# lin-shuyu/ladder-latent-data-distribution-modelling

Measured on AMD Instinct MI355X. Metric: training images/sec (full 4-run LaDDer iteration, CelebA 128x128), higher is better.
Workload: dtype f32; 1 GPU; BASELINE configs[2]: celeba 128x128x3 nh=512 z=64 R=2 K=30 L=100 per-GPU batch=128, 4 runs/iteration (AE step, sigma step, prior step, inner-sigma step), fitted-GM regime; global_batch=128, parallelism=dp1

## Files before the change

### include/ladder_hip.h

```cpp
#ifndef LADDER_HIP_H
#define LADDER_HIP_H

#include <stddef.h>
#include <stdint.h>

#ifdef __cplusplus
extern "C" {
#endif

typedef struct ihipStream_t* ladder_stream_t;

enum { LADDER_OK = 0, LADDER_E_SHAPE = -1, LADDER_E_ALIGN = -2, LADDER_E_WORKSPACE = -3, LADDER_E_LAUNCH = -4 };
enum { LADDER_ACT_NONE = 0, LADDER_ACT_LEAKY = 1 , LADDER_ACT_RELU = 2, LADDER_ACT_TANH = 3 };

#define LADDER_ABI_VERSION 2
int ladder_abi_version(void);
int ladder_igemm_fwd_tile(long M, int Cin, int Cout);
int ladder_conv2d_fwd_kernel_id(int N, int H, int W, int Cin, int Ho, int Wo, int Cout, int KH, int KW, int stride, int ups,
                                int pad_t, int pad_l);
int ladder_dense_fwd_nt(const float* x, const float* wT, const float* bias, float* y, int M, int K, int N, int act, ladder_stream_t stream);
int ladder_dense_bwd_data_nt(const float* dy, const float* w, float* dx, int M, int K, int N, const float* gate_y, int gate_act, ladder_stream_t stream);
int ladder_dense_fwd_is_persistent(long M, int K, int N);
int ladder_dense_bwd_weight_is_persistent(long M, int K, int N);

// ... 31 lines not shown
int ladder_absmax_samples(const float* x, int n_samples, size_t per_sample, float* out, ladder_stream_t stream);
size_t ladder_filter_pack_split_bytes(int ntaps, int Cin, int Cout, int prec);
int ladder_filter_pack_split(const float* w, void* packed, int ntaps, int Cin, int Cout, int transpose_flip, int prec,
                             ladder_stream_t stream);
typedef struct ladder_pack_job_t {
  const float* w;
  void* packed;
  int ntaps, Cin, Cout, transpose_flip;
  int block_begin, reserved;
} ladder_pack_job_t;
int ladder_filter_pack_job_blocks(int ntaps, int Cin, int Cout);
size_t ladder_filter_pack_split_multi_scratch_bytes(int njobs);
int ladder_filter_pack_split_multi(const ladder_pack_job_t* jobs_dev, int njobs, int total_blocks, int prec, void* scratch,
                                   size_t scratch_bytes, ladder_stream_t stream);
int ladder_conv3x3_split_eligible(int N, int H, int W, int Cin, int Cout);
int ladder_conv3x3_f32_eligible(int N, int H, int W, int Cin, int Cout);
int ladder_conv3x3_split(const float* x, const float* x_absmax, const void* packed, const float* bias, float* y, float* y_absmax, int N,
                         int H, int W, int Cin, int Cout, int act, int prec, ladder_stream_t stream);

int ladder_conv3x3_split_proj(const float* x, const float* x_absmax, const void* packed, const float* bias, float* y, const float* proj_w,
                              const float* proj_b, float* proj_out, int proj_cout, int N, int H, int W, int Cin, int Cout, int act,
                              int prec, ladder_stream_t stream);

int ladder_conv3x3_s2_bwd_data_split_eligible(int N, int H, int W, int Cin, int Ho, int Wo, int Cout, int KH, int KW, int stride, int pad_t,
                                              int pad_l);
int ladder_conv3x3_s2_bwd_data_split(const float* dy, const float* dy_absmax, const void* packed_s2, float* dx, float* dx_absmax, int N, int H,
                                     int W, int Cin, int Ho, int Wo, int Cout, int prec, ladder_stream_t stream);
int ladder_conv3x3_s2_bwd_data_f32_eligible(int N, int H, int W, int Cin, int Ho, int Wo, int Cout);
int ladder_conv3x3_s2_fwd_f32_eligible(int N, int H, int W, int Cin, int Ho, int Wo, int Cout);
int ladder_conv3x3_s2_fwd_f32(const float* x, const void* bank_s2f, const float* bias, float* y, int N, int H, int W, int Cin, int Ho, int Wo,
                              int Cout, int act, ladder_stream_t stream);

int ladder_up2proj_eligible(int N, int H, int W, int Cin, int Cout);
int ladder_up2proj_fwd_combine(const float* z, const float* bias, float* y, const float* proj_w, const float* proj_b, float* proj_out, int proj_cout,
                               int N, int H, int W, int C, int act, ladder_stream_t stream);
int ladder_up2proj_bwd_combine(const float* dy, float* d, int N, int H, int W, int C, ladder_stream_t stream);
int ladder_up2proj_wgrad_unpack(const float* dwcat, const float* db9, float* dw, float* db, int Cin, int Cout, ladder_stream_t stream);
int ladder_upfproj_eligible(int factor, int N, int H, int W, int Cin, int Cout);
int ladder_upfproj_fwd_combine(const float* z, const float* bias, float* y, int factor, int N, int H, int W, int C, int act, ladder_stream_t stream);
int ladder_upfproj_bwd_combine(const float* dy, float* d, int factor, int N, int H, int W, int C, ladder_stream_t stream);
int ladder_up2proj_bwd_combine_walk(const float* dy, float* d, int N, int H, int W, int C, int rows_per_thread, ladder_stream_t stream);
int ladder_up2proj_bwd_combine_proj_eligible(int N, int H, int W, int C, int pco);
size_t ladder_up2proj_bwd_combine_proj_workspace_bytes(int N, int H, int W, int C, int pco);
int ladder_up2proj_bwd_combine_proj(const float* y, const float* dyp, const float* pw, float* d, float* dpw, float* dpb, int pco, int N, int H, int W, int C,
                                    int act, void* ws, size_t ws_bytes, ladder_stream_t stream);
int ladder_up2proj_fused_eligible(int N, int H, int W, int Cin, int Cout);
int ladder_up2proj_fused_preferred(int N, int H, int W, int Cin, int Cout);
int ladder_up2proj_fused_wide_tile(int N, int H, int W, int Cin, int Cout);
size_t ladder_up2proj_fused_workspace_bytes(int N, int H, int W, int Cout, int proj_cout);
int ladder_up2proj_fused_fwd(const float* x, const float* wcatT, const float* bias, float* y, const float* proj_w, const float* proj_b, float* proj_out,
                             int proj_cout, int N, int H, int W, int Cin, int Cout, int act, void* ws, size_t ws_bytes, ladder_stream_t stream);

int ladder_conv3x3_up2_split_eligible(int N, int H, int W, int Cin, int Cout, int prec);
int ladder_conv3x3_up2_split(const float* x, const float* x_absmax, const void* packed_up2, const float* bias, float* y, float* y_absmax,
                             int N, int H, int W, int Cin, int Cout, int act, int prec, int x_upsampled, ladder_stream_t stream);
int ladder_conv3x3_up2_split_proj(const float* x, const float* x_absmax, const void* packed_up2, const float* bias, float* y, const float* proj_w,
                                  const float* proj_b, float* proj_out, int proj_cout, int N, int H, int W, int Cin, int Cout, int act, int prec,
                                  int x_upsampled, ladder_stream_t stream);
int ladder_conv3x3_up2_bwd_data_split_eligible(int N, int H, int W, int C, int Cout, int prec);
int ladder_conv3x3_up2_bwd_data_split(const float* dy, const float* dy_absmax, const void* packed_up2t, float* dx, float* dx_absmax, int N, int H,
                                      int W, int C, int Cout, int prec, ladder_stream_t stream);
int ladder_conv3x3_up2_bwd_border(const float* d_up, float* dx, float* dx_absmax, int N, int H, int W, int C, int axis, int first,
                                  ladder_stream_t stream);
size_t ladder_conv3x3_up2_bwd_borders_workspace_bytes(int N, int H, int W, int C, int Cout);
int ladder_conv3x3_up2_bwd_borders(const float* dy, const float* w, float* dx, int N, int H, int W, int C, int Cout, void* ws, size_t ws_bytes,
                                   ladder_stream_t stream);
int ladder_conv3x3_up2_bwd_data_gated_f32_eligible(int N, int H, int W, int C, int Cout);
int ladder_conv3x3_up2_bwd_data_gated_f32(const float* dy, const void* bank_up2t, float* dx, const float* gate, int gate_act, int N, int H, int W, int C,
                                          int Cout, ladder_stream_t stream);
int ladder_conv3x3_up2_bwd_borders_gated(const float* dy, const float* w, float* dx, const float* gate, int gate_act, int N, int H, int W, int C, int Cout,
                                         void* ws, size_t ws_bytes, ladder_stream_t stream);
int ladder_conv3x3_up2_wgrad_eligible(int N, int H, int W, int Cin, int Cout);
size_t ladder_conv3x3_up2_wgrad_workspace_bytes(int N, int H, int W, int Cin, int Cout);
int ladder_conv3x3_up2_wgrad(const float* x, int x_upsampled, const float* dy, float* dw, float* db, int N, int H, int W, int Cin, int Cout,
                             void* ws, size_t ws_bytes, ladder_stream_t stream);
size_t ladder_conv3x3_up2_edges_workspace_bytes(int N, int H, int W, int Cin, int Cout);
int ladder_conv3x3_up2_edges(const float* x, const float* w, const float* bias, float* y, float* y_absmax, const float* proj_w, const float* proj_b,
                             float* proj_out, int proj_cout, int N, int H, int W, int Cin, int Cout, int act, int x_upsampled, void* ws,
                             size_t ws_bytes, ladder_stream_t stream);

size_t ladder_presplit_bytes(size_t n, int prec);
int ladder_presplit(const float* x, const float* x_absmax, void* planes, size_t n, int n_samples, int prec, ladder_stream_t stream);
int ladder_conv2d_fwd_split_eligible(int N, int H, int W, int Cin, int Ho, int Wo, int Cout, int KH, int KW, int stride, int pad_t,
                                     int pad_l);
size_t ladder_conv2d_fwd_split_workspace_bytes(int N, int H, int W, int Cin, int Ho, int Wo, int Cout, int KH, int KW, int stride,
                                               int pad_t, int pad_l);
int ladder_conv2d_fwd_split(const void* x_planes, const float* x_absmax, const void* packed, const float* bias, float* y, int N, int H, int W,
                            int Cin, int Ho, int Wo, int Cout, int KH, int KW, int stride, int pad_t, int pad_l, int act, int prec,
                            void* ws, size_t ws_bytes, ladder_stream_t stream);
size_t ladder_conv2d_fwd_split_bnstats_workspace_bytes(int N, int H, int W, int Cin, int Ho, int Wo, int Cout, int KH, int KW, int stride,
                                                       int pad_t, int pad_l);
int ladder_conv2d_fwd_split_bnstats(const void* x_planes, const float* x_absmax, const void* packed, const float* bias, float* y, int N,
                                    int H, int W, int Cin, int Ho, int Wo, int Cout, int KH, int KW, int stride, int pad_t, int pad_l,
                                    int act, int prec, float* sums4, void* stats_ws, size_t stats_ws_bytes, ladder_stream_t stream);
size_t ladder_conv2d_fwd_bnstats_workspace_bytes(int N, int H, int W, int Cin, int Ho, int Wo, int Cout, int KH, int KW, int stride, int pad_t,
                                                 int pad_l);
int ladder_conv2d_fwd_bnstats(const float* x, const float* w, const float* bias, float* y, int N, int H, int W, int Cin, int Ho, int Wo, int Cout,
                              int KH, int KW, int stride, int pad_t, int pad_l, int act, float* sums4, void* stats_ws, size_t stats_ws_bytes,
                              ladder_stream_t stream);
int ladder_conv2d_bwd_data_split_eligible(int N, int H, int W, int Cin, int Ho, int Wo, int Cout, int KH, int KW, int stride, int pad_t,
                                          int pad_l, int gated);
size_t ladder_conv2d_bwd_data_split_workspace_bytes(int N, int H, int W, int Cin, int Ho, int Wo, int Cout, int KH, int KW, int stride,
                                                    int pad_t, int pad_l);
int ladder_conv2d_bwd_data_split(const void* dy_planes, const float* dy_absmax, const void* packed_T, float* dx, int N, int H, int W, int Cin,
                                 int Ho, int Wo, int Cout, int KH, int KW, int stride, int pad_t, int pad_l, const float* gate_y,
                                 int gate_act, int prec, void* ws, size_t ws_bytes, ladder_stream_t stream);
int ladder_conv3x3_wgrad_split_eligible(int N, int H, int W, int Cin, int Cout, int prec);
size_t ladder_conv3x3_wgrad_split_workspace_bytes(int N, int H, int W, int Cin, int Cout);
int ladder_conv3x3_wgrad_split(const float* x, const float* x_absmax, const float* dy, const float* dy_absmax, float* dw, float* db,
                               int N, int H, int W, int Cin, int Cout, int prec, void* ws, size_t ws_bytes, ladder_stream_t stream);
int ladder_conv2d_bwd_filter_split_eligible(int N, int H, int W, int Cin, int Ho, int Wo, int Cout, int KH, int KW, int stride, int pad_t,
                                            int pad_l);
size_t ladder_conv2d_bwd_filter_split_workspace_bytes(int N, int H, int W, int Cin, int Ho, int Wo, int Cout, int KH, int KW);
int ladder_conv2d_bwd_filter_split(const void* x_planes, const float* x_absmax, const void* dy_planes, const float* dy_absmax, float* dw, float* db,
                                   int N, int H, int W, int Cin, int Ho, int Wo, int Cout, int KH, int KW, int stride, int pad_t, int pad_l,
                                   int prec, void* ws, size_t ws_bytes, ladder_stream_t stream);
int ladder_reduce_splits(const float* ws, float* out, int splits, size_t n, ladder_stream_t stream);

int ladder_dense_fwd(const float* x, const float* w, const float* bias, float* y,
                     int M, int K, int N, int act, void* ws, size_t ws_bytes, ladder_stream_t stream);
int ladder_dense_bwd_data(const float* dy, const float* wT, float* dx, int M, int K, int N,
                          const float* gate_y, int gate_act, void* ws, size_t ws_bytes, ladder_stream_t stream);
size_t ladder_dense_bwd_weight_workspace_bytes(int M, int K, int N);
int ladder_dense_bwd_weight(const float* x, const float* dy, float* dw, float* db,
                            int M, int K, int N, void* ws, size_t ws_bytes, ladder_stream_t stream);
int ladder_dense_small_eligible(int M, int K, int N);
int ladder_dense_fwd_small(const float* x, const float* w, const float* bias, float* y, int M, int K, int N, int act, ladder_stream_t stream);
int ladder_dense_bwd_data_small(const float* dy, const float* w, float* dx, int M, int K, int N, const float* gate_y, int gate_act,
                                ladder_stream_t stream);
int ladder_dense_bwd_weight_small(const float* x, const float* dy, float* dw, float* db, int M, int K, int N, ladder_stream_t stream);
int ladder_dense_bwd_small(const float* x, const float* dy, const float* w, float* dx, float* dw, float* db, int M, int K, int N,
                           const float* gate_y, int gate_act, ladder_stream_t stream);
int ladder_dense_fwd_small_f32(const float* x, const float* w, const float* bias, float* y, int M, int K, int N, int act, ladder_stream_t stream);
int ladder_dense_bwd_data_small_f32(const float* dy, const float* w, float* dx, int M, int K, int N, const float* gate_y, int gate_act,
                                    ladder_stream_t stream);
int ladder_dense_bwd_weight_small_f32(const float* x, const float* dy, float* dw, float* db, int M, int K, int N, ladder_stream_t stream);
int ladder_dense_bwd_small_f32(const float* x, const float* dy, const float* w, float* dx, float* dw, float* db, int M, int K, int N,
                               const float* gate_y, int gate_act, ladder_stream_t stream);


int ladder_conv_rgb_s2_eligible(int N, int H, int W, int Cin, int Cout, int KH, int KW, int stride, int pad_t, int pad_l);
int ladder_conv_rgb_s2_fwd(const float* x, const float* w, const float* bias, float* y, int N, int H, int W, int Cout, int act,
                           ladder_stream_t stream);
size_t ladder_conv_rgb_s2_fwd_bnstats_workspace_bytes(int N, int H, int W, int Cout);
int ladder_conv_rgb_s2_fwd_bnstats(const float* x, const float* w, const float* bias, float* y, int N, int H, int W, int Cout, int act,
                                   float* sums4 , void* ws, size_t ws_bytes,
                                   ladder_stream_t stream);
int ladder_conv_rgb_s2_fwd_f32(const float* x, const float* w, const float* bias, float* y, int N, int H, int W, int Cout, int act,
                               ladder_stream_t stream);
int ladder_conv_rgb_s2_fwd_bnstats_f32(const float* x, const float* w, const float* bias, float* y, int N, int H, int W, int Cout, int act,
                                       float* sums, void* ws, size_t ws_bytes, ladder_stream_t stream);
int ladder_conv_rgb_s2_bwd_filter_f32(const float* x, const float* dy, float* dw, float* db, int N, int H, int W, int Cout, void* ws,
                                      size_t ws_bytes, ladder_stream_t stream);
size_t ladder_conv_rgb_s2_bwd_filter_workspace_bytes(int N, int H, int W, int Cout);
int ladder_conv_rgb_s2_bwd_filter(const float* x, const float* x_absmax, const float* dy, const float* dy_absmax, float* dw, float* db,
                                  int N, int H, int W, int Cout, void* ws, size_t ws_bytes, ladder_stream_t stream);

int ladder_act_bwd(const float* dy, const float* y, float* dx, size_t n, int act, ladder_stream_t stream);

size_t ladder_bn_workspace_bytes(size_t rows, int C);
int ladder_bn_fwd_stats(const float* x, float* sums , size_t rows, int C,
                        void* ws, size_t ws_bytes, ladder_stream_t stream);
int ladder_bn_stats_from_partials(const float* partials, int nblk, float* sums , int C, ladder_stream_t stream);
int ladder_bn_fwd_stats_minmax(const float* x, float* sums4, size_t rows, int C, void* ws, size_t ws_bytes, ladder_stream_t stream);
int ladder_bn_stats_minmax_from_partials(const float* partials , int nblk, float* sums4, int C, ladder_stream_t stream);
int ladder_bn_fwd_apply_planes(const float* x, const float* sums4, double count, const float* gamma, const float* beta, float* y,
                               void* y_planes, float* mean_rstd, size_t rows, int C, float eps, int act, float* y_absmax,
                               ladder_stream_t stream);
int ladder_bn_fwd_apply(const float* x, const float* sums, double count,
                        const float* gamma, const float* beta, float* y, float* mean_rstd,
                        size_t rows, int C, float eps, int act, ladder_stream_t stream);
int ladder_bn_bwd_stats(const float* dy, const float* x, const float* mean_rstd, const float* gamma,
                        const float* beta, float* dsums , size_t rows, int C, int act,
                        void* ws, size_t ws_bytes, ladder_stream_t stream);
int ladder_bn_bwd_apply(const float* dy, const float* x, const float* mean_rstd, const float* gamma,
                        const float* beta, const float* dsums, double count, float* dx,
                        float* dgamma, float* dbeta, size_t rows, int C, int act, ladder_stream_t stream);
int ladder_bn_fwd_apply_absmax(const float* x, const float* sums, double count, const float* gamma, const float* beta, float* y,
                               float* mean_rstd, size_t rows, int C, float eps, int act, float* y_absmax, ladder_stream_t stream);
int ladder_bn_bwd_apply_absmax(const float* dy, const float* x, const float* mean_rstd, const float* gamma, const float* beta,
                               const float* dsums, double count, float* dx, float* dgamma, float* dbeta, size_t rows, int C, int act,
                               float* dx_absmax, ladder_stream_t stream);

size_t ladder_in_style_workspace_bytes(int N, int HW, int C);
int ladder_in_style_fwd(const float* x, const float* style, float* y, float* mean_rstd ,
                        int N, int HW, int C, float eps, int act, void* ws, size_t ws_bytes, ladder_stream_t stream);
int ladder_in_style_bwd(const float* dy, const float* x, const float* style, const float* mean_rstd,
                        float* dx, float* dstyle , int N, int HW, int C, int act,
                        void* ws, size_t ws_bytes, ladder_stream_t stream);
int ladder_in_style_fwd_absmax(const float* x, const float* style, float* y, float* mean_rstd, int N, int HW, int C, float eps, int act,
                               void* ws, size_t ws_bytes, float* y_absmax, ladder_stream_t stream);
int ladder_in_style_bwd_absmax(const float* dy, const float* x, const float* style, const float* mean_rstd, float* dx, float* dstyle,
                               int N, int HW, int C, int act, void* ws, size_t ws_bytes, float* dx_absmax, ladder_stream_t stream);
int ladder_in_style_fwd_resize2x(const float* x, const float* style, float* up, float* mean_rstd, int N, int H, int W, int C, float eps,
                                 int act, void* ws, size_t ws_bytes, float* up_absmax, ladder_stream_t stream);
int ladder_in_style_fwd_resize2x_keep(const float* x, const float* style, float* up, float* y, float* mean_rstd, int N, int H, int W, int C,
                                      float eps, int act, void* ws, size_t ws_bytes, float* up_absmax, ladder_stream_t stream);

int ladder_resize_bilinear_fwd(const float* x, float* y, int N, int H, int W, int C, int OH, int OW, ladder_stream_t stream);
int ladder_resize_bilinear_bwd(const float* dy, float* dx, int N, int H, int W, int C, int OH, int OW, ladder_stream_t stream);
int ladder_resize_bilinear_bwd_gated(const float* dy, float* dx, int N, int H, int W, int C, int OH, int OW, const float* gate_y,
                                     int gate_act, ladder_stream_t stream);

int ladder_depth_to_space(const float* x, float* y, int N, int H, int W, int C, int r, int inverse, ladder_stream_t stream);
int ladder_pad_symmetric(const float* x, float* y, int N, int H, int W, int C, int p, ladder_stream_t stream);
int ladder_pad_symmetric_bwd(const float* dy, float* dx, int N, int H, int W, int C, int p, ladder_stream_t stream);

int ladder_randn(float* out, size_t n, uint64_t seed, uint64_t offset, ladder_stream_t stream);

int ladder_gmm_packed_stride(int R);
int ladder_gmm_prepare(const float* weights, const float* means, const float* covs, int K, int R,
                       float* packed, ladder_stream_t stream);
size_t ladder_gmm_workspace_bytes(int L, int B);
int ladder_gmm_logprob_fwd_bwd(const float* mu, const float* sd, const float* eps, const float* packed,
                               int L, int B, int R, int K, float* sum_logp, float* dmu, float* dsd,
                               void* ws, size_t ws_bytes, ladder_stream_t stream);

int ladder_gmm_logprob_rows(const float* t, const float* packed, int n, int R, int K, float* logp, ladder_stream_t stream);

enum { LADDER_P_PIX_ABS = 0, LADDER_P_PIX_SQ = 1, LADDER_P_LOG_SDZ = 2, LADDER_P_MU2SD2_Z = 3, LADDER_P_CODE_ERR = 4,
       LADDER_P_CODE_SQRT = 5, LADDER_P_CODE_ABS = 6, LADDER_P_LOG_SDT = 7, LADDER_P_MU2SD2_T = 8, LADDER_P_LOGP = 9,
       LADDER_P_FIXED = 16 };
enum { LADDER_S_SIGMA = 0, LADDER_S_MPE = 1, LADDER_S_ENTROPY_Z = 2, LADDER_S_XENT_SG = 3, LADDER_S_XENT_PRIOR = 4,
       LADDER_S_L1 = 5, LADDER_S_L2 = 6, LADDER_S_RECON_LL = 7, LADDER_S_SIGMA_REG = 8, LADDER_S_ELBO = 9,
       LADDER_S_LOSS_AE = 10, LADDER_S_INNER_SIGMA = 11, LADDER_S_MEAN_CODE_ERROR = 12, LADDER_S_CODE_LL = 13,
       LADDER_S_CODE_L1 = 14, LADDER_S_REP_REG = 15, LADDER_S_ENTROPY_T = 16, LADDER_S_XENT_T = 17,
       LADDER_S_ELBO_PRIOR = 18, LADDER_S_LOSS_PRIOR = 19,
       LADDER_S_G_PIX = 20,
       LADDER_S_G_SIGMA_VAR = 21,
       LADDER_S_G_CODE = 22,
       LADDER_S_G_INNER_SIGMA_VAR = 23,
       LADDER_S_INV_B = 24, LADDER_S_INV_LB = 25, LADDER_S_COUNT = 32 };
typedef struct {
  int B_global, D, Z, R, L;
  int sigma_uses_mpe;
  int has_inner;
  int use_sg;
  int clamp_inner_sigma;
  float inner_sigma_lb, inner_sigma_ub;
  int hierarchical;
  int prior_gmm;
} LadderElboCfg;

size_t ladder_pixel_partials_workspace_bytes(size_t n);
int ladder_pixel_partials(const float* x, const float* xhat, size_t n, float* out ,
                          void* ws, size_t ws_bytes, ladder_stream_t stream);
int ladder_pixel_grad(const float* x, const float* xhat, const float* coef, float* dxhat, size_t n, ladder_stream_t stream);
int ladder_latent_fwd(const float* mu, const float* sd_raw, const float* eps, float lvp, float* z, float* sd,
                      float* p_log, float* p_mu2sd2, float* p_sdsum, int B, int Z, ladder_stream_t stream);
int ladder_code_partials(const float* z, const float* zhat, const float* sd_z, int use_mask,
                         float* out , int B, int Z, ladder_stream_t stream);
int ladder_elbo_finalize(const float* partials, const float* sigma_var, const float* inner_sigma_var,
                         LadderElboCfg cfg, float* scalars, ladder_stream_t stream);
int ladder_code_grad(const float* z, const float* zhat, const float* sd_z, int use_mask, const float* scalars,
                     float* dz_accum, float* dzhat, int B, int Z, ladder_stream_t stream);
int ladder_latent_bwd(const float* g_sample, const float* mu, const float* sd, const float* sd_raw, const float* eps,
                      const float* extra_mu, const float* extra_sd, float extra_sign, const float* scalars, int mode,
                      float* dmu, float* dsd_raw, int B, int Z, ladder_stream_t stream);

int ladder_adam_clip(float* theta, const float* g, float* m, float* v, size_t n,
                     float lr_t, float beta1, float beta2, float eps, float clip, ladder_stream_t stream);

int ladder_adam_clip_dev(float* theta, const float* g, float* m, float* v, size_t n, float* state,
                         float beta1, float beta2, float eps, float clip, ladder_stream_t stream);
int ladder_randn_dev(float* out, size_t n, uint64_t seed, const uint64_t* offset_base, uint64_t offset_add, ladder_stream_t stream);
int ladder_u64_add(uint64_t* p, uint64_t inc, ladder_stream_t stream);

size_t ladder_gmm_dense_param_floats(int K, int R);
int ladder_gmm_prepare_dense(const float* weights, const float* means, const float* covs, int K, int R, float* params,
                             ladder_stream_t stream);
size_t ladder_gmm_dense_workspace_bytes(int L, int B, int R, int K);
int ladder_gmm_dense_logprob_fwd_bwd(const float* mu, const float* sd, const float* eps, const float* params, int L, int B, int R,
                                     int K, float* sum_logp, float* dmu, float* dsd, void* ws, size_t ws_bytes,
                                     ladder_stream_t stream);

int ladder_gmm_dense_logprob_rows(const float* t, const float* params, int n, int R, int K, float* logp, void* ws, size_t ws_bytes,
                                  ladder_stream_t stream);

size_t ladder_diag_mixture_workspace_bytes(int B, int Z, int K);
int ladder_diag_mixture_fwd_bwd(const float* mu, const float* sd, const float* eps, const float* comp_mean, const float* comp_sd,
                                int L, int B, int Z, int K, float* sum_logp, float* dmu, float* dsd, float* dcomp_mean,
                                float* dcomp_sd, void* ws, size_t ws_bytes, ladder_stream_t stream);

int ladder_gather_rows(const void* src, int src_is_u8, const int64_t* idx, float* out, int B, int64_t D, float scale,
                       ladder_stream_t stream);

size_t ladder_vbgmm_state_doubles(int K, int R);
size_t ladder_vbgmm_workspace_bytes(int N, int K);
int ladder_vbgmm_fit(const float* X, int N, int K, int R, const int* labels, double* state, int prior_type, double wc_prior,
                     double mean_prec_prior, double reg_covar, double tol, int max_iter, float* weights, float* means,
                     float* covs, void* ws, size_t ws_bytes, ladder_stream_t stream);

size_t ladder_vbgmm_shard_stats_doubles(int K, int R);
size_t ladder_vbgmm_shard_workspace_bytes(int N, int K, int R);
size_t ladder_vbgmm_shard_moments_doubles(int R);
int ladder_vbgmm_shard_moments(const float* X, int N, int R, double* moments, ladder_stream_t stream);
int ladder_vbgmm_shard_estep(const float* X, int N, int K, int R, const int* labels, const double* state, int prior_type, double* stats,
                             void* ws, size_t ws_bytes, ladder_stream_t stream);
int ladder_vbgmm_shard_mstep(const double* stats, const double* moments, int K, int R, double* state, int prior_type, double wc_prior,
                             double mean_prec_prior, double reg_covar, double tol, int max_iter, int it, float* weights, float* means,
                             float* covs, ladder_stream_t stream);

size_t ladder_mixture_sample_param_bytes(int K, int R);
int ladder_mixture_sample_prepare(const float* weights, const float* means, const float* covs, int K, int R, void* params,
                                  ladder_stream_t stream);
int ladder_mixture_sample_prepare_diag(const float* comp_mean, const float* comp_sd, int K, int R, void* params, ladder_stream_t stream);
int ladder_mixture_sample(const void* params, int K, int R, int n, int64_t first, const float* u, const float* eps, uint64_t seed,
                          uint64_t offset, float* out, int* comp, ladder_stream_t stream);
int ladder_images_to_u8(const float* x, uint8_t* out, size_t n, ladder_stream_t stream);

uint32_t ladder_crc32c_extend(uint32_t crc, const void* data, size_t n);
int ladder_axpy(const float* in, float* out, size_t n, float scale, int accumulate, ladder_stream_t stream);

#ifdef __cplusplus
}
#endif
#endif
```

### ladder_latent_data_distribution_modelling_amd/_lib.py

```python
import ctypes as C
import os

_HERE = os.path.dirname(os.path.abspath(__file__))
LIB_PATH = os.path.join(_HERE, "csrc", "libladder_hip.so")

ERRORS = {-1: "LADDER_E_SHAPE", -2: "LADDER_E_ALIGN", -3: "LADDER_E_WORKSPACE", -4: "LADDER_E_LAUNCH"}
ACT = {None: 0, "none": 0, "leaky_relu": 1, "relu": 2, "tanh": 3}

P_PIX_ABS, P_PIX_SQ, P_LOG_SDZ, P_MU2SD2_Z, P_CODE_ERR, P_CODE_SQRT, P_CODE_ABS, P_LOG_SDT, P_MU2SD2_T, P_LOGP = range(10)
P_FIXED = 16
S_NAMES = ["sigma", "mean_pixel_error", "entropy_z", "crossEntropy_prior_sg", "crossEntropy_prior",
           "l1_reconstruction_error", "l2_reconstruction_error", "reconstruction_likelihood", "sigma_regularisor",
           "elbo", "loss_ae", "inner_sigma", "mean_code_error", "code_reconstruction_likelihood",
           "code_l1_reconstruction_error", "representation_regularisor", "entropy_t",
           "crossEntropy_representation", "elbo_prior", "loss_prior",
           "_g_pix", "_g_sigma_var", "_g_code", "_g_inner_sigma_var", "_inv_B", "_inv_LB"]
S_INDEX = {n: i for i, n in enumerate(S_NAMES)}
S_COUNT = 32
ABSMAX_FLOATS = 512
ABI_VERSION = 2


class LadderElboCfg(C.Structure):
    _fields_ = [("B_global", C.c_int), ("D", C.c_int), ("Z", C.c_int), ("R", C.c_int), ("L", C.c_int),
                ("sigma_uses_mpe", C.c_int), ("has_inner", C.c_int), ("use_sg", C.c_int),
                ("clamp_inner_sigma", C.c_int), ("inner_sigma_lb", C.c_float), ("inner_sigma_ub", C.c_float),
                ("hierarchical", C.c_int), ("prior_gmm", C.c_int)]


_p, _i, _f, _d, _z, _u64 = C.c_void_p, C.c_int, C.c_float, C.c_double, C.c_size_t, C.c_uint64

PROTOTYPES = {
    "ladder_abi_version": (_i, []),
    "ladder_igemm_fwd_tile": (_i, [C.c_long, _i, _i]),
    "ladder_dense_fwd_is_persistent": (_i, [C.c_long, _i, _i]),
    "ladder_dense_fwd_nt": (_i, [_p, _p, _p, _p, _i, _i, _i, _i, _p]),
    "ladder_dense_bwd_data_nt": (_i, [_p, _p, _p, _i, _i, _i, _p, _i, _p]),
    "ladder_dense_bwd_weight_is_persistent": (_i, [C.c_long, _i, _i]),
    "ladder_igemm_fwd_splits": (_i, [C.c_long, _i, _i]),
    "ladder_conv2d_fwd_kernel_id": (_i, [_i] * 13),
    "ladder_conv2d_bwd_filter_kernel_id": (_i, [_i] * 12),
    "ladder_conv2d_fwd": (_i, [_p, _p, _p, _p] + [_i] * 13 + [_p, _z, _p]),
    "ladder_igemm_fwd_workspace_bytes": (_z, [C.c_long, _i, _i]),
    "ladder_filter_flip_transpose": (_i, [_p, _p, _i, _i, _i, _i, _p]),
    "ladder_conv2d_bwd_data": (_i, [_p, _p, _p] + [_i] * 12 + [_p, _i, _p, _z, _p]),
    "ladder_conv2d_bwd_filter_workspace_bytes": (_z, [_i] * 9),
    "ladder_conv2d_bwd_filter": (_i, [_p, _p, _p, _p] + [_i] * 12 + [_p, _z, _p]),
    "ladder_dense_fwd": (_i, [_p, _p, _p, _p, _i, _i, _i, _i, _p, _z, _p]),
    "ladder_dense_bwd_data": (_i, [_p, _p, _p, _i, _i, _i, _p, _i, _p, _z, _p]),
    "ladder_dense_bwd_weight_workspace_bytes": (_z, [_i, _i, _i]),
    "ladder_dense_bwd_weight": (_i, [_p, _p, _p, _p, _i, _i, _i, _p, _z, _p]),
    "ladder_act_bwd": (_i, [_p, _p, _p, _z, _i, _p]),
    "ladder_bn_workspace_bytes": (_z, [_z, _i]),
    "ladder_bn_fwd_stats": (_i, [_p, _p, _z, _i, _p, _z, _p]),
    "ladder_bn_fwd_apply": (_i, [_p, _p, _d, _p, _p, _p, _p, _z, _i, _f, _i, _p]),
    "ladder_bn_bwd_stats": (_i, [_p, _p, _p, _p, _p, _p, _z, _i, _i, _p, _z, _p]),
    "ladder_bn_bwd_apply": (_i, [_p, _p, _p, _p, _p, _p, _d, _p, _p, _p, _z, _i, _i, _p]),
    "ladder_in_style_workspace_bytes": (_z, [_i, _i, _i]),
    "ladder_in_style_fwd": (_i, [_p, _p, _p, _p, _i, _i, _i, _f, _i, _p, _z, _p]),
    "ladder_in_style_bwd": (_i, [_p, _p, _p, _p, _p, _p, _i, _i, _i, _i, _p, _z, _p]),
    "ladder_resize_bilinear_fwd": (_i, [_p, _p] + [_i] * 6 + [_p]),
    "ladder_resize_bilinear_bwd": (_i, [_p, _p] + [_i] * 6 + [_p]),
    "ladder_resize_bilinear_bwd_gated": (_i, [_p, _p, _i, _i, _i, _i, _i, _i, _p, _i, _p]),
    "ladder_depth_to_space": (_i, [_p, _p] + [_i] * 6 + [_p]),
    "ladder_pad_symmetric": (_i, [_p, _p] + [_i] * 5 + [_p]),
    "ladder_randn": (_i, [_p, _z, _u64, _u64, _p]),
    "ladder_gmm_packed_stride": (_i, [_i]),
    "ladder_gmm_prepare": (_i, [_p, _p, _p, _i, _i, _p, _p]),
    "ladder_gmm_workspace_bytes": (_z, [_i, _i]),
    "ladder_gmm_logprob_fwd_bwd": (_i, [_p, _p, _p, _p, _i, _i, _i, _i, _p, _p, _p, _p, _z, _p]),
    "ladder_gmm_logprob_rows": (_i, [_p, _p, _i, _i, _i, _p, _p]),
    "ladder_gmm_dense_logprob_rows": (_i, [_p, _p, _i, _i, _i, _p, _p, _z, _p]),
    "ladder_pixel_partials_workspace_bytes": (_z, [_z]),
    "ladder_pixel_partials": (_i, [_p, _p, _z, _p, _p, _z, _p]),
    "ladder_pixel_grad": (_i, [_p, _p, _p, _p, _z, _p]),
    "ladder_latent_fwd": (_i, [_p, _p, _p, _f, _p, _p, _p, _p, _p, _i, _i, _p]),
    "ladder_code_partials": (_i, [_p, _p, _p, _i, _p, _i, _i, _p]),
    "ladder_elbo_finalize": (_i, [_p, _p, _p, LadderElboCfg, _p, _p]),
    "ladder_code_grad": (_i, [_p, _p, _p, _i, _p, _p, _p, _i, _i, _p]),
    "ladder_latent_bwd": (_i, [_p, _p, _p, _p, _p, _p, _p, _f, _p, _i, _p, _p, _i, _i, _p]),
    "ladder_adam_clip": (_i, [_p, _p, _p, _p, _z, _f, _f, _f, _f, _f, _p]),
    "ladder_adam_clip_dev": (_i, [_p, _p, _p, _p, _z, _p, _f, _f, _f, _f, _p]),
    "ladder_randn_dev": (_i, [_p, _z, _u64, _p, _u64, _p]),
    "ladder_u64_add": (_i, [_p, _u64, _p]),
    "ladder_crc32c_extend": (C.c_uint32, [C.c_uint32, _p, _z]),
    "ladder_gmm_dense_param_floats": (_z, [_i, _i]),
    "ladder_gmm_prepare_dense": (_i, [_p, _p, _p, _i, _i, _p, _p]),
    "ladder_gmm_dense_workspace_bytes": (_z, [_i, _i, _i, _i]),
    "ladder_gmm_dense_logprob_fwd_bwd": (_i, [_p, _p, _p, _p, _i, _i, _i, _i, _p, _p, _p, _p, _z, _p]),
    "ladder_diag_mixture_workspace_bytes": (_z, [_i, _i, _i]),
    "ladder_diag_mixture_fwd_bwd": (_i, [_p, _p, _p, _p, _p, _i, _i, _i, _i, _p, _p, _p, _p, _p, _p, _z, _p]),
    "ladder_pad_symmetric_bwd": (_i, [_p, _p, _i, _i, _i, _i, _i, _p]),
    "ladder_conv1x1_smallcout_eligible": (_i, [C.c_long, _i, _i]),
    "ladder_conv1x1_smallcout_bwd_workspace_bytes": (_z, [C.c_long, _i, _i]),
    "ladder_conv1x1_smallcout_bwd": (_i, [_p, _p, _p, _p, _p, _p, C.c_long, _i, _i, _i, _p, _z, _p]),
    "ladder_gather_rows": (_i, [_p, _i, _p, _p, _i, C.c_int64, _f, _p]),
    "ladder_vbgmm_state_doubles": (_z, [_i, _i]),
    "ladder_vbgmm_workspace_bytes": (_z, [_i, _i]),
    "ladder_vbgmm_fit": (_i, [_p, _i, _i, _i, _p, _p, _i, _d, _d, _d, _d, _i, _p, _p, _p, _p, _z, _p]),
    "ladder_vbgmm_shard_stats_doubles": (_z, [_i, _i]),
    "ladder_vbgmm_shard_workspace_bytes": (_z, [_i, _i, _i]),
    "ladder_vbgmm_shard_moments_doubles": (_z, [_i]),
    "ladder_vbgmm_shard_moments": (_i, [_p, _i, _i, _p, _p]),
    "ladder_vbgmm_shard_estep": (_i, [_p, _i, _i, _i, _p, _p, _i, _p, _p, _z, _p]),
    "ladder_vbgmm_shard_mstep": (_i, [_p, _p, _i, _i, _p, _i, _d, _d, _d, _d, _i, _i, _p, _p, _p, _p]),
    "ladder_axpy": (_i, [_p, _p, _z, _f, _i, _p]),
    "ladder_filter_pack_split_bytes": (_z, [_i, _i, _i, _i]),
    "ladder_filter_pack_split": (_i, [_p, _p, _i, _i, _i, _i, _i, _p]),
    "ladder_filter_pack_job_blocks": (_i, [_i, _i, _i]),
    "ladder_filter_pack_split_multi_scratch_bytes": (_z, [_i]),
    "ladder_filter_pack_split_multi": (_i, [_p, _i, _i, _i, _p, _z, _p]),
    "ladder_conv2d_fwd_split_eligible": (_i, [_i] * 12),
    "ladder_conv2d_fwd_split_workspace_bytes": (_z, [_i] * 12),
    "ladder_conv2d_fwd_split": (_i, [_p, _p, _p, _p, _p] + [_i] * 14 + [_p, _z, _p]),
    "ladder_conv2d_fwd_split_bnstats_workspace_bytes": (_z, [_i] * 12),
    "ladder_conv2d_fwd_split_bnstats": (_i, [_p] * 5 + [_i] * 14 + [_p, _p, _z, _p]),
    "ladder_conv2d_fwd_bnstats_workspace_bytes": (_z, [_i] * 12),
    "ladder_conv2d_fwd_bnstats": (_i, [_p, _p, _p, _p] + [_i] * 13 + [_p, _p, _z, _p]),
    "ladder_conv2d_bwd_data_split_eligible": (_i, [_i] * 13),
    "ladder_conv2d_bwd_data_split_workspace_bytes": (_z, [_i] * 12),
    "ladder_conv2d_bwd_data_split": (_i, [_p, _p, _p, _p] + [_i] * 12 + [_p, _i, _i, _p, _z, _p]),
    "ladder_conv3x3_split_eligible": (_i, [_i] * 5),
    "ladder_conv3x3_split": (_i, [_p, _p, _p, _p, _p, _p] + [_i] * 7 + [_p]),
    "ladder_conv3x3_s2_bwd_data_split_eligible": (_i, [_i] * 12),
    "ladder_conv3x3_up2_split_eligible": (_i, [_i] * 6),
    "ladder_conv3x3_up2_split": (_i, [_p, _p, _p, _p, _p, _p] + [_i] * 8 + [_p]),
    "ladder_conv3x3_up2_split_proj": (_i, [_p] * 8 + [_i] * 9 + [_p]),
    "ladder_conv3x3_up2_bwd_data_split_eligible": (_i, [_i] * 6),
    "ladder_conv3x3_up2_bwd_data_split": (_i, [_p] * 5 + [_i] * 6 + [_p]),
    "ladder_conv3x3_up2_bwd_border": (_i, [_p, _p, _p] + [_i] * 6 + [_p]),
    "ladder_conv3x3_up2_bwd_borders_workspace_bytes": (_z, [_i] * 5),
    "ladder_conv3x3_up2_bwd_borders": (_i, [_p, _p, _p] + [_i] * 5 + [_p, _z, _p]),
    "ladder_conv3x3_up2_wgrad_eligible": (_i, [_i] * 5),
    "ladder_conv3x3_up2_wgrad_workspace_bytes": (_z, [_i] * 5),
    "ladder_conv3x3_up2_wgrad": (_i, [_p, _i, _p, _p, _p] + [_i] * 5 + [_p, _z, _p]),
    "ladder_conv3x3_up2_edges_workspace_bytes": (_z, [_i] * 5),
    "ladder_conv3x3_up2_edges": (_i, [_p] * 8 + [_i] * 8 + [_p, _z, _p]),
    "ladder_conv3x3_s2_bwd_data_split": (_i, [_p, _p, _p, _p, _p] + [_i] * 8 + [_p]),
    "ladder_conv3x3_f32_eligible": (_i, [_i] * 5),
    "ladder_conv3x3_up2_bwd_data_gated_f32_eligible": (_i, [_i] * 5),
    "ladder_conv3x3_up2_bwd_data_gated_f32": (_i, [_p, _p, _p, _p] + [_i] * 6 + [_p]),
    "ladder_conv3x3_up2_bwd_borders_gated": (_i, [_p, _p, _p, _p] + [_i] * 6 + [_p, _z, _p]),
    "ladder_conv3x3_s2_bwd_data_f32_eligible": (_i, [_i] * 7),
    "ladder_conv3x3_s2_fwd_f32_eligible": (_i, [_i] * 7),
    "ladder_conv3x3_s2_fwd_f32": (_i, [_p, _p, _p, _p] + [_i] * 8 + [_p]),
    "ladder_up2proj_eligible": (_i, [_i] * 5),
    "ladder_up2proj_fwd_combine": (_i, [_p] * 6 + [_i] * 6 + [_p]),
    "ladder_up2proj_bwd_combine": (_i, [_p, _p] + [_i] * 4 + [_p]),
    "ladder_up2proj_wgrad_unpack": (_i, [_p] * 4 + [_i, _i, _p]),
    "ladder_upfproj_eligible": (_i, [_i] * 6),
    "ladder_upfproj_fwd_combine": (_i, [_p] * 3 + [_i] * 6 + [_p]),
    "ladder_upfproj_bwd_combine": (_i, [_p, _p] + [_i] * 5 + [_p]),
    "ladder_up2proj_bwd_combine_walk": (_i, [_p, _p] + [_i] * 5 + [_p]),
    "ladder_up2proj_bwd_combine_proj_eligible": (_i, [_i] * 5),
    "ladder_up2proj_bwd_combine_proj_workspace_bytes": (_z, [_i] * 5),
    "ladder_up2proj_bwd_combine_proj": (_i, [_p] * 6 + [_i] * 6 + [_p, _z, _p]),
    "ladder_up2proj_fused_eligible": (_i, [_i] * 5),
    "ladder_up2proj_fused_preferred": (_i, [_i] * 5),
    "ladder_up2proj_fused_wide_tile": (_i, [_i] * 5),
    "ladder_up2proj_fused_workspace_bytes": (_z, [_i] * 5),
    "ladder_up2proj_fused_fwd": (_i, [_p] * 7 + [_i] * 7 + [_p, _z, _p]),
    "ladder_dense_small_eligible": (_i, [_i, _i, _i]),
    "ladder_dense_fwd_small": (_i, [_p, _p, _p, _p, _i, _i, _i, _i, _p]),
    "ladder_dense_bwd_data_small": (_i, [_p, _p, _p, _i, _i, _i, _p, _i, _p]),
    "ladder_dense_bwd_weight_small": (_i, [_p, _p, _p, _p, _i, _i, _i, _p]),
    "ladder_dense_bwd_small": (_i, [_p, _p, _p, _p, _p, _p, _i, _i, _i, _p, _i, _p]),
    "ladder_dense_fwd_small_f32": (_i, [_p, _p, _p, _p, _i, _i, _i, _i, _p]),
    "ladder_dense_bwd_data_small_f32": (_i, [_p, _p, _p, _i, _i, _i, _p, _i, _p]),
    "ladder_dense_bwd_weight_small_f32": (_i, [_p, _p, _p, _p, _i, _i, _i, _p]),
    "ladder_dense_bwd_small_f32": (_i, [_p, _p, _p, _p, _p, _p, _i, _i, _i, _p, _i, _p]),
    "ladder_presplit_bytes": (_z, [_z, _i]),
    "ladder_presplit": (_i, [_p, _p, _p, _z, _i, _i, _p]),
    "ladder_absmax_samples": (_i, [_p, _i, _z, _p, _p]),
    "ladder_conv3x3_split_proj": (_i, [_p, _p, _p, _p, _p, _p, _p, _p] + [_i] * 8 + [_p]),
    "ladder_conv_rgb_s2_eligible": (_i, [_i] * 10),
    "ladder_conv_rgb_s2_fwd": (_i, [_p, _p, _p, _p, _i, _i, _i, _i, _i, _p]),
    "ladder_conv_rgb_s2_fwd_bnstats_workspace_bytes": (_z, [_i] * 4),
    "ladder_conv_rgb_s2_fwd_bnstats": (_i, [_p, _p, _p, _p, _i, _i, _i, _i, _i, _p, _p, _z, _p]),
    "ladder_conv_rgb_s2_fwd_f32": (_i, [_p, _p, _p, _p, _i, _i, _i, _i, _i, _p]),
    "ladder_conv_rgb_s2_fwd_bnstats_f32": (_i, [_p, _p, _p, _p, _i, _i, _i, _i, _i, _p, _p, _z, _p]),
    "ladder_bn_stats_from_partials": (_i, [_p, _i, _p, _i, _p]),
    "ladder_bn_stats_minmax_from_partials": (_i, [_p, _i, _p, _i, _p]),
    "ladder_bn_fwd_stats_minmax": (_i, [_p, _p, _z, _i, _p, _z, _p]),
    "ladder_bn_fwd_apply_planes": (_i, [_p, _p, _d, _p, _p, _p, _p, _p, _z, _i, _f, _i, _p, _p]),
    "ladder_conv_rgb_s2_bwd_filter_workspace_bytes": (_z, [_i] * 4),
    "ladder_conv_rgb_s2_bwd_filter": (_i, [_p] * 6 + [_i] * 4 + [_p, _z, _p]),
    "ladder_conv_rgb_s2_bwd_filter_f32": (_i, [_p] * 4 + [_i] * 4 + [_p, _z, _p]),
    "ladder_bn_fwd_apply_absmax": (_i, [_p, _p, _d, _p, _p, _p, _p, _z, _i, _f, _i, _p, _p]),
    "ladder_bn_bwd_apply_absmax": (_i, [_p, _p, _p, _p, _p, _p, _d, _p, _p, _p, _z, _i, _i, _p, _p]),
    "ladder_in_style_fwd_absmax": (_i, [_p, _p, _p, _p, _i, _i, _i, _f, _i, _p, _z, _p, _p]),
    "ladder_in_style_fwd_resize2x": (_i, [_p, _p, _p, _p, _i, _i, _i, _i, _f, _i, _p, _z, _p, _p]),
    "ladder_in_style_fwd_resize2x_keep": (_i, [_p, _p, _p, _p, _p, _i, _i, _i, _i, _f, _i, _p, _z, _p, _p]),
    "ladder_in_style_bwd_absmax": (_i, [_p, _p, _p, _p, _p, _p, _i, _i, _i, _i, _p, _z, _p, _p]),
    "ladder_conv1x1_smallcout_bwd_absmax": (_i, [_p, _p, _p, _p, _p, _p, C.c_long, _i, _i, _i, _p, _z, _p, C.c_long, _p]),
    "ladder_absmax": (_i, [_p, _z, _p, _p]),
    "ladder_conv3x3_wgrad_split_eligible": (_i, [_i] * 6),
    "ladder_conv3x3_wgrad_split_workspace_bytes": (_z, [_i] * 5),
    "ladder_conv3x3_wgrad_split": (_i, [_p, _p, _p, _p, _p, _p] + [_i] * 6 + [_p, _z, _p]),
    "ladder_reduce_splits": (_i, [_p, _p, _i, _z, _p]),
    "ladder_conv2d_bwd_filter_split_eligible": (_i, [_i] * 12),
    "ladder_conv2d_bwd_filter_split_workspace_bytes": (_z, [_i] * 9),
    "ladder_conv2d_bwd_filter_split": (_i, [_p, _p, _p, _p, _p, _p] + [_i] * 13 + [_p, _z, _p]),
    "ladder_mixture_sample_param_bytes": (_z, [_i, _i]),
    "ladder_mixture_sample_prepare": (_i, [_p, _p, _p, _i, _i, _p, _p]),
    "ladder_mixture_sample_prepare_diag": (_i, [_p, _p, _i, _i, _p, _p]),
    "ladder_mixture_sample": (_i, [_p, _i, _i, _i, C.c_int64, _p, _p, _u64, _u64, _p, _p, _p]),
    "ladder_images_to_u8": (_i, [_p, _p, _z, _p]),
}

_lib = None


class LadderHipError(RuntimeError):
    pass


def load(path=None):
    global _lib
    if _lib is not None:
        return _lib
    path = path or os.environ.get("LADDER_HIP_LIB", LIB_PATH)
    import torch
    if not os.path.exists(path):
        raise LadderHipError(
            "libladder_hip.so not found at %s: build it with `python -m "
            "ladder_latent_data_distribution_modelling_amd.csrc.build` (there is no CPU fallback)" % path)
    lib = C.CDLL(path)
    for name, (res, args) in PROTOTYPES.items():
        fn = getattr(lib, name)
        fn.restype = res
        fn.argtypes = args
    got = lib.ladder_abi_version()
    if got != ABI_VERSION:
        raise LadderHipError("%s reports ABI version %d, this binding needs %d (stale build? re-run `python -m "
                             "ladder_latent_data_distribution_modelling_amd.csrc.build`)" % (path, got, ABI_VERSION))
    _lib = lib
    return lib


def call(name, *args):
    rc = getattr(load(), name)(*args)
    if rc != 0:
        raise LadderHipError("%s failed: %s (%d)" % (name, ERRORS.get(rc, "?"), rc))


def query(name, *args):
    return getattr(load(), name)(*args)
```

### ladder_latent_data_distribution_modelling_amd/csrc/convrgb.hip

```cpp
#include "split16.h"

namespace {

constexpr int RGB_TH = 8, RGB_TW = 32, RGB_PIX = RGB_TH * RGB_TW;
constexpr int RGB_PH = 2 * RGB_TH + 1, RGB_PW = 2 * RGB_TW + 1;
constexpr int RGB_PATCH = RGB_PH * RGB_PW * 3;
constexpr int RGB_THREADS = 512;
constexpr int RGB_A_PLANE = 2 * 2 * RGB_PIX * 16;
constexpr int RGB_B_PLANE = 2 * 2 * 128 * 16;

__device__ __forceinline__ float block_max_512(float m, float* red) {
  m = wave_max(m);
  __syncthreads();
  if ((threadIdx.x & 63) == 0) red[threadIdx.x >> 6] = m;
  __syncthreads();
  float b = red[0];
#pragma unroll
  for (int w = 1; w < 8; ++w) b = fmaxf(b, red[w]);
  return b;
}

__device__ __forceinline__ float rgb_tap(const float* __restrict__ patch, int pr, int pc, int k) {
  const int tap = k / 3, ci = k - tap * 3, r = tap / 3, s = tap - r * 3;
  return patch[((2 * pr + r) * RGB_PW + 2 * pc + s) * 3 + ci];
// ... 162 lines not shown
    __syncthreads();
#pragma unroll
    for (int ni = 0; ni < 2; ++ni) {
      const float a0 = st0[ni] + __shfl_xor(st0[ni], 32, 64), a1 = st1[ni] + __shfl_xor(st1[ni], 32, 64);
      const float a2 = fminf(smn[ni], __shfl_xor(smn[ni], 32, 64)), a3 = fmaxf(smx[ni], __shfl_xor(smx[ni], 32, 64));
      if (lh == 0) {
        const int cc = wn * 64 + ni * 32 + l31;
        sred[(0 * 4 + wm) * 128 + cc] = a0;
        sred[(1 * 4 + wm) * 128 + cc] = a1;
        sred[(2 * 4 + wm) * 128 + cc] = a2;
        sred[(3 * 4 + wm) * 128 + cc] = a3;
      }
    }
    __syncthreads();
    {
      const int which = tid >> 7, c = tid & 127;
      const float v0 = sred[(which * 4 + 0) * 128 + c], v1 = sred[(which * 4 + 1) * 128 + c], v2 = sred[(which * 4 + 2) * 128 + c],
                  v3 = sred[(which * 4 + 3) * 128 + c];
      const float t = which < 2 ? (v0 + v1) + (v2 + v3) : (which == 2 ? fminf(fminf(v0, v1), fminf(v2, v3)) : fmaxf(fmaxf(v0, v1), fmaxf(v2, v3)));
      if (n0 + c < Cout) stats_part[((size_t)mt * 4 + which) * Cout + n0 + c] = t;
    }
  }
}

constexpr int RW_PH = 2, RW_PW = 32, RW_PIX = RW_PH * RW_PW;
constexpr int RW_XH = 2 * RW_PH + 1, RW_XW = 2 * RW_PW + 1, RW_PATCH = RW_XH * RW_XW * 3;
constexpr int RW_THREADS = 256;
constexpr int RW_ABLK = RW_PIX * 64 + 64, RW_DBLK = RW_PIX * 64 + 64;
constexpr int RW_APLANE = RW_ABLK, RW_DPLANE = 4 * RW_DBLK;
constexpr int RW_XU = (RW_PATCH + RW_THREADS - 1) / RW_THREADS;
constexpr int RW_DU = RW_PIX * 32 / RW_THREADS;

typedef short rgb_s16x4 __attribute__((ext_vector_type(4)));
__device__ __forceinline__ uint4 rgb_tr_frag(const unsigned char* p) {
  const rgb_s16x4 lo = __builtin_amdgcn_ds_read_tr16_b64_v4i16((__attribute__((address_space(3))) rgb_s16x4*)(p));
  const rgb_s16x4 hi = __builtin_amdgcn_ds_read_tr16_b64_v4i16((__attribute__((address_space(3))) rgb_s16x4*)(p + 4 * 64));
  const uint2 a = __builtin_bit_cast(uint2, lo), b = __builtin_bit_cast(uint2, hi);
  return make_uint4(a.x, a.y, b.x, b.y);
}
__device__ __forceinline__ float rgb_frag_sum(const uint4 f) {
  const uint32_t w[4] = {f.x, f.y, f.z, f.w};
  float s = 0.f;
#pragma unroll
  for (int i = 0; i < 4; ++i) {
    const f32x2 v = __builtin_convertvector(__builtin_bit_cast(f16x2, w[i]), f32x2);
    s += v.x + v.y;
  }
  return s;
}

__global__ __launch_bounds__(RW_THREADS, 3) void conv_rgb_s2_wgrad_kernel(const float* __restrict__ x, const float* __restrict__ dy,
                                                                         float* __restrict__ part, float* __restrict__ bias_part,
                                                                         const int N, const int H, const int W, const int Cout,
                                                                         const int tiles_co, const int patches_per_split,
                                                                         const float* __restrict__ xamax, const float* __restrict__ damax) {
  __shared__ __attribute__((aligned(16))) unsigned char lds[2 * RW_APLANE + 2 * RW_DPLANE];
  __shared__ __attribute__((aligned(16))) float patch[RW_PATCH + 1];
  unsigned char* const Ab = lds;
  unsigned char* const Db = lds + 2 * RW_APLANE;

  const int tid = threadIdx.x, lane = tid & 63, wv = tid >> 6;
  const int l31 = lane & 31, lh = lane >> 5, l15 = lane & 15;
  const int split = blockIdx.x / tiles_co, co0 = (blockIdx.x - split * tiles_co) * 128;
  const int Ho = H / 2, Wo = W / 2, WP = Wo / RW_PW, HP = Ho / RW_PH;
  const int q_total = N * HP * WP;
  const int q0 = split * patches_per_split, q1 = min(q_total, q0 + patches_per_split);
  const float cx = scale_from_absmax(amax_load(xamax)), cd = scale_from_absmax(amax_load(damax));
  const int frag_lane = (8 * lh + (l15 >> 2)) * 64 + (16 * ((lane >> 4) & 1) + 4 * (l15 & 3)) * 2;

  f32x16 acc;
#pragma unroll
  for (int e = 0; e < 16; ++e) acc[e] = 0.f;
  float bsum = 0.f;

  float xr[RW_XU];
  float4 d0, d1, d2, d3, d4, d5, d6, d7;
  auto load_patch = [&](int q) {
    const int img = q / (HP * WP), rem = q - img * (HP * WP), hp = rem / WP;
    const int h0 = hp * RW_PH, w0 = (rem - hp * WP) * RW_PW;
#pragma unroll
    for (int i = 0; i < RW_XU; ++i) {
      const int v = tid + i * RW_THREADS;
      const int r = v / (RW_XW * 3), c3 = v - r * (RW_XW * 3);
      const int hi = 2 * h0 + r, wi3 = 2 * w0 * 3 + c3;
      xr[i] = (v < RW_PATCH && hi < H && wi3 < W * 3) ? x[((long)img * H + hi) * W * 3 + wi3] : 0.f;
    }
    const float* dbase = dy + (((long)img * Ho + h0) * Wo + w0) * Cout + co0;
#define RW_DSRC(i_) [&]() -> float4 {                                                                                       \
      const int u = tid + (i_) * RW_THREADS, px = u >> 5, q4 = u & 31;                                                        \
      if (co0 + q4 * 4 >= Cout) return make_float4(0.f, 0.f, 0.f, 0.f);                                                       \
      return *reinterpret_cast<const float4*>(dbase + ((long)(px >> 5) * Wo + (px & 31)) * Cout + q4 * 4); }()
    d0 = RW_DSRC(0); d1 = RW_DSRC(1); d2 = RW_DSRC(2); d3 = RW_DSRC(3); d4 = RW_DSRC(4); d5 = RW_DSRC(5); d6 = RW_DSRC(6); d7 = RW_DSRC(7);
#undef RW_DSRC
  };
  auto store_d = [&](int i, float4 v) {
    const int u = tid + i * RW_THREADS, px = u >> 5, q4 = u & 31;
    uint2 pl[2];
    split4<2, true>(make_float4(v.x * cd, v.y * cd, v.z * cd, v.w * cd), pl);
#pragma unroll
    for (int p = 0; p < 2; ++p) *reinterpret_cast<uint2*>(Db + p * RW_DPLANE + (q4 >> 3) * RW_DBLK + px * 64 + (q4 & 7) * 8) = pl[p];
  };

  if (q0 < q1) load_patch(q0);
  for (int q = q0; q < q1; ++q) {
#pragma unroll
    for (int i = 0; i < RW_XU; ++i)
      if (tid + i * RW_THREADS < RW_PATCH) patch[tid + i * RW_THREADS] = xr[i];
    store_d(0, d0); store_d(1, d1); store_d(2, d2); store_d(3, d3); store_d(4, d4); store_d(5, d5); store_d(6, d6); store_d(7, d7);
    __syncthreads();
    if (tid < 2 * RW_PIX) {
      const int p = tid & (RW_PIX - 1), kh = tid >> 6, pr = p >> 5, pc = p & 31;
      float av[16];
#pragma unroll
      for (int j = 0; j < 16; ++j) {
        const int k = kh * 16 + j;
        const int tap = k / 3, ci = k - tap * 3, r = tap / 3, s = tap - r * 3;
        av[j] = k < 27 ? patch[((2 * pr + r) * RW_XW + 2 * pc + s) * 3 + ci] * cx : 0.f;
      }
#pragma unroll
      for (int o = 0; o < 4; ++o) {
        uint2 pl[2];
        split4<2, true>(make_float4(av[4 * o], av[4 * o + 1], av[4 * o + 2], av[4 * o + 3]), pl);
#pragma unroll
        for (int pp = 0; pp < 2; ++pp) *reinterpret_cast<uint2*>(Ab + pp * RW_APLANE + p * 64 + kh * 32 + o * 8) = pl[pp];
      }
    }
    __syncthreads();
    if (q + 1 < q1) load_patch(q + 1);
#pragma unroll
    for (int ks = 0; ks < RW_PIX / 16; ++ks) {
      const int pb = ks * 16;
      const uint4 a0 = rgb_tr_frag(Ab + pb * 64 + frag_lane), a1 = rgb_tr_frag(Ab + RW_APLANE + pb * 64 + frag_lane);
      const uint4 b0 = rgb_tr_frag(Db + wv * RW_DBLK + pb * 64 + frag_lane), b1 = rgb_tr_frag(Db + RW_DPLANE + wv * RW_DBLK + pb * 64 + frag_lane);
      acc = mfma16<true>(a1, b0, acc);
      acc = mfma16<true>(a0, b1, acc);
      acc = mfma16<true>(a0, b0, acc);
      bsum += rgb_frag_sum(b1) + rgb_frag_sum(b0);
    }
    __syncthreads();
  }

  const float unscale = 1.f / (cx * cd);
  float* o = part + (size_t)split * 27 * Cout;
  const int n = co0 + wv * 32 + l31;
#pragma unroll
  for (int e = 0; e < 16; ++e) {
    const int k = (e & 3) + 8 * (e >> 2) + 4 * lh;
    if (k < 27 && n < Cout) o[(size_t)k * Cout + n] = acc[e] * unscale;
  }
  bsum += __shfl_down(bsum, 32, 64);
  if (bias_part != nullptr && lh == 0 && n < Cout) bias_part[(size_t)split * Cout + n] = bsum * (1.f / cd);
}

constexpr int RW_LDA32 = 33;
__global__ __launch_bounds__(RW_THREADS, 4) void conv_rgb_s2_wgrad_f32_kernel(const float* __restrict__ x, const float* __restrict__ dy,
                                                                             float* __restrict__ part, float* __restrict__ bias_part,
                                                                             const int N, const int H, const int W, const int Cout,
                                                                             const int tiles_co, const int patches_per_split) {
  __shared__ float A32[RW_PIX * RW_LDA32];
  __shared__ float patch[RW_PATCH + 1];
  const int tid = threadIdx.x, lane = tid & 63, wv = tid >> 6;
  const int l31 = lane & 31, lh = lane >> 5;
  const int split = blockIdx.x / tiles_co, co0 = (blockIdx.x - split * tiles_co) * 128;
  const int Ho = H / 2, Wo = W / 2, WP = Wo / RW_PW, HP = Ho / RW_PH;
  const int q_total = N * HP * WP;
  const int q0 = split * patches_per_split, q1 = min(q_total, q0 + patches_per_split);
  const int co = co0 + wv * 32 + l31;
  const bool co_ok = co < Cout;

  f32x16 acc;
#pragma unroll
  for (int e = 0; e < 16; ++e) acc[e] = 0.f;
  float bsum = 0.f;
  float xr[RW_XU];
  auto decode = [&](int q, int& img, int& h0, int& w0) {
    img = q / (HP * WP);
    const int rem = q - img * (HP * WP), hp = rem / WP;
    h0 = hp * RW_PH;
    w0 = (rem - hp * WP) * RW_PW;
  };
  auto load_x = [&](int q) {
    int img, h0, w0;
    decode(q, img, h0, w0);
#pragma unroll
    for (int i = 0; i < RW_XU; ++i) {
      const int v = tid + i * RW_THREADS;
      const int r = v / (RW_XW * 3), c3 = v - r * (RW_XW * 3);
      const int hi = 2 * h0 + r, wi3 = 2 * w0 * 3 + c3;
      xr[i] = (v < RW_PATCH && hi < H && wi3 < W * 3) ? x[((long)img * H + hi) * W * 3 + wi3] : 0.f;
    }
  };

  if (q0 < q1) load_x(q0);
  for (int q = q0; q < q1; ++q) {
    float b[RW_PIX / 2];
    {
      int img, h0, w0;
      decode(q, img, h0, w0);
      const float* du = dy + (((long)img * Ho + h0) * Wo + w0) * Cout;
      const unsigned loff = (unsigned)(co + lh * Cout);
#pragma unroll
      for (int ks = 0; ks < RW_PIX / 2; ++ks) {
        const float* pk = du + ((long)(ks >> 4) * Wo + 2 * (ks & 15)) * Cout;
        b[ks] = co_ok ? pk[loff] : 0.f;
      }
    }
#pragma unroll
    for (int i = 0; i < RW_XU; ++i)
      if (tid + i * RW_THREADS < RW_PATCH) patch[tid + i * RW_THREADS] = xr[i];
    __syncthreads();
    if (q + 1 < q1) load_x(q + 1);
    {
      const int p = tid & (RW_PIX - 1), kq = tid >> 6, pr = p >> 5, pc = p & 31;
#pragma unroll
      for (int j = 0; j < 8; ++j) {
        const int k = kq * 8 + j;
        const int tap = k / 3, ci = k - tap * 3, r = tap / 3, sx = tap - r * 3;
        A32[p * RW_LDA32 + k] = k < 27 ? patch[((2 * pr + r) * RW_XW + 2 * pc + sx) * 3 + ci] : 0.f;
      }
    }
    __syncthreads();
#pragma unroll
    for (int ks = 0; ks < RW_PIX / 2; ++ks) {
      const float a = A32[(2 * ks + lh) * RW_LDA32 + l31];
      acc = __builtin_amdgcn_mfma_f32_32x32x2f32(a, b[ks], acc, 0, 0, 0);
      bsum += b[ks];
    }
    __syncthreads();
  }

  float* o = part + (size_t)split * 27 * Cout;
#pragma unroll
  for (int e = 0; e < 16; ++e) {
    const int k = (e & 3) + 8 * (e >> 2) + 4 * lh;
    if (k < 27 && co_ok) o[(size_t)k * Cout + co] = acc[e];
  }
  if (bias_part != nullptr) {
    const float v = bsum + __shfl_down(bsum, 32, 64);
    if (lh == 0 && co_ok) bias_part[(size_t)split * Cout + co] = v;
  }
}

struct RgbWgradPlan { int tiles_co, splits, pps; };
RgbWgradPlan plan_rgb_wgrad(int N, int H, int W, int Cout) {
  RgbWgradPlan p;
  p.tiles_co = (Cout + 127) / 128;
  const long q_total = (long)N * (H / 2 / RW_PH) * (W / 2 / RW_PW);
  long s = (3 * 256L) / p.tiles_co;
  if (s > q_total / 4) s = q_total / 4;
  if (s < 1) s = 1;
  p.pps = (int)((q_total + s - 1) / s);
  p.splits = (int)((q_total + p.pps - 1) / p.pps);
  return p;
}

bool rgb_s2_ok(int N, int H, int W, int Cin, int Cout, int KH, int KW, int stride, int pad_t, int pad_l) {
  return N > 0 && Cin == 3 && KH == 3 && KW == 3 && stride == 2 && pad_t == 0 && pad_l == 0 && (H % 2) == 0 && (W % 2) == 0 &&
         ((H / 2) % RGB_TH) == 0 && ((W / 2) % RGB_TW) == 0 && Cout >= 32 && (Cout % 4) == 0;
}

}

extern "C" {

int ladder_conv_rgb_s2_eligible(int N, int H, int W, int Cin, int Cout, int KH, int KW, int stride, int pad_t, int pad_l) {
  return rgb_s2_ok(N, H, W, Cin, Cout, KH, KW, stride, pad_t, pad_l) ? 1 : 0;
}

static int rgb_fwd_launch(const float* x, const float* w, const float* bias, float* y, int N, int H, int W, int Cout, int act, float* stats_part,
                          ladder_stream_t stream, bool f32 = false) {
  if (!rgb_s2_ok(N, H, W, 3, Cout, 3, 3, 2, 0, 0)) return LADDER_E_SHAPE;
  if (!ladder_aligned16(y) || (bias != nullptr && !ladder_aligned16(bias))) return LADDER_E_ALIGN;
  const int tiles_n = (Cout + 127) / 128;
  const long tiles = (long)N * (H / 2 / RGB_TH) * (W / 2 / RGB_TW) * tiles_n;
  if (tiles >= (1L << 31)) return LADDER_E_SHAPE;
  if (f32)
    hipLaunchKernelGGL(conv_rgb_s2_fwd_kernel<true>, dim3((unsigned)tiles), dim3(RGB_THREADS), 0, stream, x, w, bias, y, N, H, W, Cout, act, tiles_n,
                       stats_part);
  else
    hipLaunchKernelGGL(conv_rgb_s2_fwd_kernel<false>, dim3((unsigned)tiles), dim3(RGB_THREADS), 0, stream, x, w, bias, y, N, H, W, Cout, act, tiles_n,
                       stats_part);
  LADDER_CHECK_LAUNCH();
  return LADDER_OK;
}

int ladder_conv_rgb_s2_fwd(const float* x, const float* w, const float* bias, float* y, int N, int H, int W, int Cout, int act,
                           ladder_stream_t stream) {
  return rgb_fwd_launch(x, w, bias, y, N, H, W, Cout, act, nullptr, stream);
}

size_t ladder_conv_rgb_s2_fwd_bnstats_workspace_bytes(int N, int H, int W, int Cout) {
  if (!rgb_s2_ok(N, H, W, 3, Cout, 3, 3, 2, 0, 0)) return 0;
  return (size_t)N * (H / 2 / RGB_TH) * (W / 2 / RGB_TW) * 4 * Cout * sizeof(float);
}

int ladder_conv_rgb_s2_fwd_bnstats(const float* x, const float* w, const float* bias, float* y, int N, int H, int W, int Cout, int act,
                                   float* sums, void* ws, size_t ws_bytes, ladder_stream_t stream) {
  const size_t need = ladder_conv_rgb_s2_fwd_bnstats_workspace_bytes(N, H, W, Cout);
  if (need == 0 || sums == nullptr) return LADDER_E_SHAPE;
  if (ws == nullptr || ws_bytes < need) return LADDER_E_WORKSPACE;
  const int rc = rgb_fwd_launch(x, w, bias, y, N, H, W, Cout, act, (float*)ws, stream);
  if (rc != LADDER_OK) return rc;
  return ladder_bn_stats_minmax_from_partials((const float*)ws, N * (H / 2 / RGB_TH) * (W / 2 / RGB_TW), sums, Cout, stream);
}

int ladder_conv_rgb_s2_fwd_f32(const float* x, const float* w, const float* bias, float* y, int N, int H, int W, int Cout, int act,
                               ladder_stream_t stream) {
  return rgb_fwd_launch(x, w, bias, y, N, H, W, Cout, act, nullptr, stream, true);
}

int ladder_conv_rgb_s2_fwd_bnstats_f32(const float* x, const float* w, const float* bias, float* y, int N, int H, int W, int Cout, int act,
                                       float* sums, void* ws, size_t ws_bytes, ladder_stream_t stream) {
  const size_t need = ladder_conv_rgb_s2_fwd_bnstats_workspace_bytes(N, H, W, Cout);
  if (need == 0 || sums == nullptr) return LADDER_E_SHAPE;
  if (ws == nullptr || ws_bytes < need) return LADDER_E_WORKSPACE;
  const int rc = rgb_fwd_launch(x, w, bias, y, N, H, W, Cout, act, (float*)ws, stream, true);
  if (rc != LADDER_OK) return rc;
  return ladder_bn_stats_minmax_from_partials((const float*)ws, N * (H / 2 / RGB_TH) * (W / 2 / RGB_TW), sums, Cout, stream);
}

int ladder_conv_rgb_s2_bwd_filter_f32(const float* x, const float* dy, float* dw, float* db, int N, int H, int W, int Cout, void* ws,
                                      size_t ws_bytes, ladder_stream_t stream) {
  if (!rgb_s2_ok(N, H, W, 3, Cout, 3, 3, 2, 0, 0)) return LADDER_E_SHAPE;
  if (!ladder_aligned16(dw)) return LADDER_E_ALIGN;
  const RgbWgradPlan p = plan_rgb_wgrad(N, H, W, Cout);
  if (ws == nullptr || ws_bytes < (size_t)p.splits * (27 * (size_t)Cout + Cout) * sizeof(float)) return LADDER_E_WORKSPACE;
  float* part = (float*)ws;
  float* bias_part = db != nullptr ? part + (size_t)p.splits * 27 * Cout : nullptr;
  hipLaunchKernelGGL(conv_rgb_s2_wgrad_f32_kernel, dim3(p.tiles_co * p.splits), dim3(RW_THREADS), 0, stream, x, dy, part, bias_part, N, H, W, Cout,
                     p.tiles_co, p.pps);
  LADDER_CHECK_LAUNCH();
  int rc = ladder_reduce_splits(part, dw, p.splits, (size_t)27 * Cout, stream);
  if (rc != LADDER_OK) return rc;
  if (db != nullptr) rc = ladder_reduce_splits(bias_part, db, p.splits, (size_t)Cout, stream);
  return rc;
}

size_t ladder_conv_rgb_s2_bwd_filter_workspace_bytes(int N, int H, int W, int Cout) {
  if (!rgb_s2_ok(N, H, W, 3, Cout, 3, 3, 2, 0, 0)) return 0;
  const RgbWgradPlan p = plan_rgb_wgrad(N, H, W, Cout);
  return (size_t)p.splits * (27 * (size_t)Cout + Cout) * sizeof(float);
}

int ladder_conv_rgb_s2_bwd_filter(const float* x, const float* x_absmax, const float* dy, const float* dy_absmax, float* dw, float* db, int N,
                                  int H, int W, int Cout, void* ws, size_t ws_bytes, ladder_stream_t stream) {
  if (!rgb_s2_ok(N, H, W, 3, Cout, 3, 3, 2, 0, 0) || x_absmax == nullptr || dy_absmax == nullptr) return LADDER_E_SHAPE;
  if (!ladder_aligned16(dy) || !ladder_aligned16(dw)) return LADDER_E_ALIGN;
  if (ws == nullptr || ws_bytes < ladder_conv_rgb_s2_bwd_filter_workspace_bytes(N, H, W, Cout)) return LADDER_E_WORKSPACE;
  const RgbWgradPlan p = plan_rgb_wgrad(N, H, W, Cout);
  float* part = (float*)ws;
  float* bias_part = db != nullptr ? part + (size_t)p.splits * 27 * Cout : nullptr;
  hipLaunchKernelGGL(conv_rgb_s2_wgrad_kernel, dim3(p.tiles_co * p.splits), dim3(RW_THREADS), 0, stream, x, dy, part, bias_part, N, H, W, Cout,
                     p.tiles_co, p.pps, x_absmax, dy_absmax);
  LADDER_CHECK_LAUNCH();
  int rc = ladder_reduce_splits(part, dw, p.splits, (size_t)27 * Cout, stream);
  if (rc != LADDER_OK) return rc;
  if (db != nullptr) rc = ladder_reduce_splits(bias_part, db, p.splits, (size_t)Cout, stream);
  return rc;
}

}
```

### ladder_latent_data_distribution_modelling_amd/csrc/norm.hip

```cpp
#include "split16.h"

namespace {

template <int MODE>
__global__ __launch_bounds__(256) void colstats_stage1(const float* __restrict__ a, const float* __restrict__ b,
                                                       const float* __restrict__ mean_rstd, const float* __restrict__ gamma,
                                                       const float* __restrict__ beta, float* __restrict__ ws, size_t rows,
                                                       int C, size_t rows_per_blk, int act) {
  const int cl = threadIdx.x & 63, rl = threadIdx.x >> 6;
  const int c = blockIdx.x * 64 + cl;
  const size_t r0 = (size_t)blockIdx.y * rows_per_blk, r1 = min(rows, r0 + rows_per_blk);
  float s0 = 0.f, s1 = 0.f;
  if (c < C) {
    if (MODE == 1) {
      for (size_t r = r0 + rl; r < r1; r += 4) {
        const float v = a[r * C + c];
        s0 += v;
        s1 += v * v;
      }
    } else {
      const float mu = mean_rstd[c], rs = mean_rstd[C + c], g = gamma[c], be = beta[c];
      for (size_t r = r0 + rl; r < r1; r += 4) {
        const float xh = (b[r * C + c] - mu) * rs;
        const float dp = a[r * C + c] * ladder_act_grad_from_out(g * xh + be, act);
// ... 593 lines not shown
  __syncthreads();
  if (rl < 2 && c < C) {
    float4 t = make_float4(0.f, 0.f, 0.f, 0.f);
#pragma unroll
    for (int k = 0; k < 16; ++k) t = f4add(t, sm[rl][k][cq]);
    *reinterpret_cast<float4*>(part + (((size_t)n * split + sp) * 2 + rl) * C + c) = t;
  }
}

__global__ void in_finalize_kernel(const float* __restrict__ x, const float* __restrict__ part, float* __restrict__ mean_rstd,
                                   int N, int HW, int C, int split, float eps, float* __restrict__ clear_rec) {
  amax_clear_by_block0(clear_rec);
  const int i = blockIdx.x * blockDim.x + threadIdx.x;
  if (i >= N * C) return;
  const int n = i / C, c = i - n * C;
  double s0 = 0.0, s1 = 0.0;
  for (int sp = 0; sp < split; ++sp) {
    s0 += (double)part[(((size_t)n * split + sp) * 2 + 0) * C + c];
    s1 += (double)part[(((size_t)n * split + sp) * 2 + 1) * C + c];
  }
  const double pv = (double)in_pivot(x + (size_t)n * HW * C, HW, C, c);
  const double md = s0 / HW;
  double var = s1 / HW - md * md;
  if (var < 0.0) var = 0.0;
  mean_rstd[(size_t)n * 2 * C + c] = (float)(pv + md);
  mean_rstd[(size_t)n * 2 * C + C + c] = (float)(1.0 / sqrt(var + (double)eps));
}

__global__ __launch_bounds__(256) void in_apply_kernel(const float* __restrict__ x, const float* __restrict__ style,
                                                       const float* __restrict__ mean_rstd, float* __restrict__ y, int HW, int C,
                                                       int act, int split, float* __restrict__ yamax) {
  const int cq = threadIdx.x & 15, rl = threadIdx.x >> 4;
  const int n = blockIdx.y, sp = blockIdx.z;
  int c = blockIdx.x * 64 + cq * 4;
  const bool live = c < C;
  if (!live) {
    if (yamax == nullptr) return;
    c = 0;
  }
  float ymax = 0.f;
  const size_t base = (size_t)n * HW * C;
  const int per = (HW + split - 1) / split, r0 = sp * per, r1 = live ? min(HW, r0 + per) : r0;
  const float4 mu = *reinterpret_cast<const float4*>(mean_rstd + (size_t)n * 2 * C + c);
  const float4 rs = *reinterpret_cast<const float4*>(mean_rstd + (size_t)n * 2 * C + C + c);
  float4 s0 = *reinterpret_cast<const float4*>(style + (size_t)n * 2 * C + c);
  const float4 s1 = *reinterpret_cast<const float4*>(style + (size_t)n * 2 * C + C + c);
  s0.x += 1.f; s0.y += 1.f; s0.z += 1.f; s0.w += 1.f;
  for (int r = r0 + rl; r < r1; r += 16) {
    const size_t i = base + (size_t)r * C + c;
    const float4 v = *reinterpret_cast<const float4*>(x + i);
    float4 o;
    o.x = ladder_act_fn((v.x - mu.x) * rs.x * s0.x + s1.x, act);
    o.y = ladder_act_fn((v.y - mu.y) * rs.y * s0.y + s1.y, act);
    o.z = ladder_act_fn((v.z - mu.z) * rs.z * s0.z + s1.z, act);
    o.w = ladder_act_fn((v.w - mu.w) * rs.w * s0.w + s1.w, act);
    *reinterpret_cast<float4*>(y + i) = o;
    ymax = fmaxf(fmaxf(ymax, fmaxf(fabsf(o.x), fabsf(o.y))), fmaxf(fabsf(o.z), fabsf(o.w)));
  }
  if (yamax != nullptr) amax_commit_block_sample(ymax, yamax, n);
}

__global__ __launch_bounds__(256) void in_bwd_stats_kernel(const float* __restrict__ dy, const float* __restrict__ x,
                                                           const float* __restrict__ style, const float* __restrict__ mean_rstd,
                                                           float* __restrict__ part, int HW, int C, int act, int split) {
  const int cq = threadIdx.x & 15, rl = threadIdx.x >> 4;
  const int n = blockIdx.y, c = blockIdx.x * 64 + cq * 4, sp = blockIdx.z;
  const size_t base = (size_t)n * HW * C;
  const int per = (HW + split - 1) / split, r0 = sp * per, r1 = min(HW, r0 + per);
  float4 a0 = make_float4(0.f, 0.f, 0.f, 0.f), a1 = a0;
  if (c < C) {
    const float4 mu = *reinterpret_cast<const float4*>(mean_rstd + (size_t)n * 2 * C + c);
    const float4 rs = *reinterpret_cast<const float4*>(mean_rstd + (size_t)n * 2 * C + C + c);
    float4 s0 = *reinterpret_cast<const float4*>(style + (size_t)n * 2 * C + c);
    const float4 s1 = *reinterpret_cast<const float4*>(style + (size_t)n * 2 * C + C + c);
    s0.x += 1.f; s0.y += 1.f; s0.z += 1.f; s0.w += 1.f;
    for (int r = r0 + rl; r < r1; r += 16) {
      const size_t i = base + (size_t)r * C + c;
      const float4 xv = *reinterpret_cast<const float4*>(x + i), dv = *reinterpret_cast<const float4*>(dy + i);
      float xh, dp;
      xh = (xv.x - mu.x) * rs.x; dp = dv.x * ladder_act_grad_from_out(xh * s0.x + s1.x, act); a0.x += dp * xh; a1.x += dp;
      xh = (xv.y - mu.y) * rs.y; dp = dv.y * ladder_act_grad_from_out(xh * s0.y + s1.y, act); a0.y += dp * xh; a1.y += dp;
      xh = (xv.z - mu.z) * rs.z; dp = dv.z * ladder_act_grad_from_out(xh * s0.z + s1.z, act); a0.z += dp * xh; a1.z += dp;
      xh = (xv.w - mu.w) * rs.w; dp = dv.w * ladder_act_grad_from_out(xh * s0.w + s1.w, act); a0.w += dp * xh; a1.w += dp;
    }
  }
  __shared__ float4 sm[2][16][16];
  sm[0][rl][cq] = a0;
  sm[1][rl][cq] = a1;
  __syncthreads();
  if (rl < 2 && c < C) {
    float4 t = make_float4(0.f, 0.f, 0.f, 0.f);
#pragma unroll
    for (int k = 0; k < 16; ++k) t = f4add(t, sm[rl][k][cq]);
    *reinterpret_cast<float4*>(part + (((size_t)n * split + sp) * 2 + rl) * C + c) = t;
  }
}
__global__ void in_bwd_finalize_kernel(const float* __restrict__ part, float* __restrict__ dstyle, int N, int C, int split,
                                       float* __restrict__ clear_rec) {
  amax_clear_by_block0(clear_rec);
  const int i = blockIdx.x * blockDim.x + threadIdx.x;
  if (i >= N * C) return;
  const int n = i / C, c = i - n * C;
  double s0 = 0.0, s1 = 0.0;
  for (int sp = 0; sp < split; ++sp) {
    s0 += (double)part[(((size_t)n * split + sp) * 2 + 0) * C + c];
    s1 += (double)part[(((size_t)n * split + sp) * 2 + 1) * C + c];
  }
  dstyle[(size_t)n * 2 * C + c] = (float)s0;
  dstyle[(size_t)n * 2 * C + C + c] = (float)s1;
}
__global__ __launch_bounds__(256) void in_bwd_apply_kernel(const float* __restrict__ dy, const float* __restrict__ x,
                                                           const float* __restrict__ style, const float* __restrict__ mean_rstd,
                                                           const float* __restrict__ dstyle, float* __restrict__ dx, int HW, int C,
                                                           int act, int split, float* __restrict__ dxamax) {
  const int cq = threadIdx.x & 15, rl = threadIdx.x >> 4;
  const int n = blockIdx.y, sp = blockIdx.z;
  int c = blockIdx.x * 64 + cq * 4;
  const bool live = c < C;
  if (!live) {
    if (dxamax == nullptr) return;
    c = 0;
  }
  float omax = 0.f;
  const size_t base = (size_t)n * HW * C;
  const int per = (HW + split - 1) / split, r0 = sp * per, r1 = live ? min(HW, r0 + per) : r0;
  const float inv = 1.f / (float)HW;
  float mu[4], rs[4], s0[4], s1[4], d0[4], d1[4];
#pragma unroll
  for (int j = 0; j < 4; ++j) {
    mu[j] = mean_rstd[(size_t)n * 2 * C + c + j];
    rs[j] = mean_rstd[(size_t)n * 2 * C + C + c + j];
    s0[j] = style[(size_t)n * 2 * C + c + j] + 1.f;
    s1[j] = style[(size_t)n * 2 * C + C + c + j];
    d0[j] = dstyle[(size_t)n * 2 * C + c + j] * inv;
    d1[j] = dstyle[(size_t)n * 2 * C + C + c + j] * inv;
  }
  for (int r = r0 + rl; r < r1; r += 16) {
    const size_t i = base + (size_t)r * C + c;
    const float4 xv = *reinterpret_cast<const float4*>(x + i), dv = *reinterpret_cast<const float4*>(dy + i);
    const float xs[4] = {xv.x, xv.y, xv.z, xv.w}, ds[4] = {dv.x, dv.y, dv.z, dv.w};
    float o[4];
#pragma unroll
    for (int j = 0; j < 4; ++j) {
      const float xh = (xs[j] - mu[j]) * rs[j];
      const float dp = ds[j] * ladder_act_grad_from_out(xh * s0[j] + s1[j], act);
      o[j] = rs[j] * s0[j] * (dp - d1[j] - xh * d0[j]);
    }
    *reinterpret_cast<float4*>(dx + i) = make_float4(o[0], o[1], o[2], o[3]);
    omax = fmaxf(fmaxf(omax, fmaxf(fabsf(o[0]), fabsf(o[1]))), fmaxf(fabsf(o[2]), fabsf(o[3])));
  }
  if (dxamax != nullptr) amax_commit_block_sample(omax, dxamax, n);
}

inline int in_split(int N, int HW, int C) {
  const long groups = (long)N * ((C + 63) / 64);
  int sp = (int)((2048 + groups - 1) / groups);
  const int max_sp = (HW + 63) / 64;
  if (sp > max_sp) sp = max_sp;
  if (sp < 1) sp = 1;
  return sp;
}

template <int V> struct ResizeVec;
template <> struct ResizeVec<4> { using T = float4; };
template <> struct ResizeVec<1> { using T = float; };
__device__ __forceinline__ float4 rz_lerp(const float4& a, const float4& b, float t) {
  return make_float4(a.x + (b.x - a.x) * t, a.y + (b.y - a.y) * t, a.z + (b.z - a.z) * t, a.w + (b.w - a.w) * t);
}
__device__ __forceinline__ float rz_lerp(float a, float b, float t) { return a + (b - a) * t; }
__device__ __forceinline__ void rz_fma(float4& acc, float w, const float4& q) {
  acc.x += w * q.x; acc.y += w * q.y; acc.z += w * q.z; acc.w += w * q.w;
}
__device__ __forceinline__ void rz_fma(float& acc, float w, float q) { acc += w * q; }
__device__ __forceinline__ void rz_zero(float4& a) { a = make_float4(0.f, 0.f, 0.f, 0.f); }
__device__ __forceinline__ void rz_zero(float& a) { a = 0.f; }
__device__ __forceinline__ void rz_gate(float4& a, const float4& y, int act) {
  a.x *= ladder_act_grad_from_out(y.x, act); a.y *= ladder_act_grad_from_out(y.y, act);
  a.z *= ladder_act_grad_from_out(y.z, act); a.w *= ladder_act_grad_from_out(y.w, act);
}
__device__ __forceinline__ void rz_gate(float& a, float y, int act) { a *= ladder_act_grad_from_out(y, act); }

template <int V>
__global__ __launch_bounds__(256) void resize_fwd_kernel(const float* __restrict__ x, float* __restrict__ y, int H, int W, int CV,
                                                         int fy, int fx, int bpr) {
  using T = typename ResizeVec<V>::T;
  const int row = blockIdx.x / bpr;
  const int j = (blockIdx.x - row * bpr) * blockDim.x + threadIdx.x;
  if (j >= W * CV) return;
  const int n = row / H, iy = row - n * H;
  const int ix = j / CV, cv = j - ix * CV;
  const int yhi = min(iy + 1, H - 1), xhi = min(ix + 1, W - 1);
  const T* r0 = reinterpret_cast<const T*>(x) + (size_t)row * W * CV;
  const T* r1 = reinterpret_cast<const T*>(x) + ((size_t)n * H + yhi) * W * CV;
  const T tl = r0[ix * CV + cv], tr = r0[xhi * CV + cv], bl = r1[ix * CV + cv], br = r1[xhi * CV + cv];
  const int OW = W * fx;
  T* out = reinterpret_cast<T*>(y) + (((size_t)row * fy) * OW + (size_t)ix * fx) * CV + cv;
  for (int dy = 0; dy < fy; ++dy) {
    const float yl = (float)dy / (float)fy;
    for (int dx = 0; dx < fx; ++dx) {
      const float xl = (float)dx / (float)fx;
      const T top = rz_lerp(tl, tr, xl), bot = rz_lerp(bl, br, xl);
      out[((size_t)dy * OW + dx) * CV] = rz_lerp(top, bot, yl);
    }
  }
}

__global__ __launch_bounds__(256) void in_apply_resize2x_kernel(const float* __restrict__ x, const float* __restrict__ style,
                                                                const float* __restrict__ mean_rstd, float* __restrict__ up, int H, int W,
                                                                int C, int act, float* __restrict__ yamax, float* __restrict__ lo) {
  const int CV = C >> 2;
  const int n = blockIdx.y;
  const long j = (long)blockIdx.x * blockDim.x + threadIdx.x;
  float ymax = 0.f;
  if (j < (long)H * W * CV) {
    const int cv = (int)(j % CV);
    const int pix = (int)(j / CV), iy = pix / W, ix = pix - iy * W;
    const int c = cv * 4;
    const float4 mu = *reinterpret_cast<const float4*>(mean_rstd + (size_t)n * 2 * C + c);
    const float4 rs = *reinterpret_cast<const float4*>(mean_rstd + (size_t)n * 2 * C + C + c);
    float4 s0 = *reinterpret_cast<const float4*>(style + (size_t)n * 2 * C + c);
    const float4 s1 = *reinterpret_cast<const float4*>(style + (size_t)n * 2 * C + C + c);
    s0.x += 1.f; s0.y += 1.f; s0.z += 1.f; s0.w += 1.f;
    const int yh = min(iy + 1, H - 1), xh = min(ix + 1, W - 1);
    const float* xb = x + (size_t)n * H * W * C + c;
    auto norm = [&](int r, int q) -> float4 {
      const float4 v = *reinterpret_cast<const float4*>(xb + ((size_t)r * W + q) * C);
      float4 o;
      o.x = ladder_act_fn((v.x - mu.x) * rs.x * s0.x + s1.x, act);
      o.y = ladder_act_fn((v.y - mu.y) * rs.y * s0.y + s1.y, act);
      o.z = ladder_act_fn((v.z - mu.z) * rs.z * s0.z + s1.z, act);
      o.w = ladder_act_fn((v.w - mu.w) * rs.w * s0.w + s1.w, act);
      return o;
    };
    const float4 tl = norm(iy, ix), tr = norm(iy, xh), bl = norm(yh, ix), br = norm(yh, xh);
    ymax = fmaxf(fmaxf(fabsf(tl.x), fabsf(tl.y)), fmaxf(fabsf(tl.z), fabsf(tl.w)));
    const float4 top = rz_lerp(tl, tr, 0.5f), bot = rz_lerp(bl, br, 0.5f);
    const int OW = 2 * W;
    float* o = up + (((size_t)n * 2 * H + 2 * iy) * OW + 2 * ix) * C + c;
    *reinterpret_cast<float4*>(o) = tl;
    if (lo != nullptr) *reinterpret_cast<float4*>(lo + (((size_t)n * H + iy) * W + ix) * C + c) = tl;
    *reinterpret_cast<float4*>(o + C) = top;
    *reinterpret_cast<float4*>(o + (size_t)OW * C) = rz_lerp(tl, bl, 0.5f);
    *reinterpret_cast<float4*>(o + (size_t)OW * C + C) = rz_lerp(top, bot, 0.5f);
  }
  if (yamax != nullptr) amax_commit_block_sample(ymax, yamax, n);
}

template <int V>
__global__ __launch_bounds__(256) void resize_bwd_kernel(const float* __restrict__ dy, float* __restrict__ dx, int H, int W, int CV,
                                                         int fy, int fx, int bpr) {
  using T = typename ResizeVec<V>::T;
  const int row = blockIdx.x / bpr;
  const int j = (blockIdx.x - row * bpr) * blockDim.x + threadIdx.x;
  if (j >= W * CV) return;
  const int n = row / H, iy = row - n * H;
  const int ix = j / CV, cv = j - ix * CV;
  const int OH = H * fy, OW = W * fx;
  T acc;
  rz_zero(acc);
  const int oy0 = max(0, (iy - 1) * fy), oy1 = min(OH, (iy + 1) * fy);
  const int ox0 = max(0, (ix - 1) * fx), ox1 = min(OW, (ix + 1) * fx);
  const T* base = reinterpret_cast<const T*>(dy) + (size_t)n * OH * OW * CV + cv;
  for (int oy = oy0; oy < oy1; ++oy) {
    const int ylo = oy / fy, yhi = min(ylo + 1, H - 1);
    const float yl = (float)(oy - ylo * fy) / (float)fy;
    const float wy = (ylo == iy ? 1.f - yl : 0.f) + (yhi == iy ? yl : 0.f);
    if (wy == 0.f) continue;
    for (int ox = ox0; ox < ox1; ++ox) {
      const int xlo = ox / fx, xhi = min(xlo + 1, W - 1);
      const float xl = (float)(ox - xlo * fx) / (float)fx;
      const float wx = (xlo == ix ? 1.f - xl : 0.f) + (xhi == ix ? xl : 0.f);
      if (wx == 0.f) continue;
      rz_fma(acc, wy * wx, base[((size_t)oy * OW + ox) * CV]);
    }
  }
  reinterpret_cast<T*>(dx)[((size_t)row * W + ix) * CV + cv] = acc;
}

template <int V>
__global__ __launch_bounds__(256) void resize_bwd_x2_kernel(const float* __restrict__ dy, float* __restrict__ dx, int H, int W, int CV,
                                                            int bpr, const float* __restrict__ gate_y, int gate_act) {
  using T = typename ResizeVec<V>::T;
  const int row = blockIdx.x / bpr;
  const int j = (blockIdx.x - row * bpr) * blockDim.x + threadIdx.x;
  if (j >= W * CV) return;
  const int n = row / H, iy = row - n * H;
  const int ix = j / CV, cv = j - ix * CV;
  const int OW = 2 * W;
  const T* base = reinterpret_cast<const T*>(dy) + (size_t)n * (2 * H) * OW * CV + cv;
  const float wy[3] = {iy > 0 ? 0.5f : 0.f, 1.f, iy == H - 1 ? 1.f : 0.5f};
  const float wx[3] = {ix > 0 ? 0.5f : 0.f, 1.f, ix == W - 1 ? 1.f : 0.5f};
  T v[3][3];
#pragma unroll
  for (int a = 0; a < 3; ++a)
#pragma unroll
    for (int b = 0; b < 3; ++b) {
      const int oy = max(2 * iy - 1 + a, 0), ox = max(2 * ix - 1 + b, 0);
      v[a][b] = base[((size_t)oy * OW + ox) * CV];
    }
  T acc;
  rz_zero(acc);
#pragma unroll
  for (int a = 0; a < 3; ++a)
#pragma unroll
    for (int b = 0; b < 3; ++b)
      if (wy[a] != 0.f && wx[b] != 0.f) rz_fma(acc, wy[a] * wx[b], v[a][b]);
  const size_t o = ((size_t)row * W + ix) * CV + cv;
  if (gate_y != nullptr) rz_gate(acc, reinterpret_cast<const T*>(gate_y)[o], gate_act);
  reinterpret_cast<T*>(dx)[o] = acc;
}

__global__ __launch_bounds__(256) void gather_rows_u8_kernel(const unsigned char* __restrict__ src, const long long* __restrict__ idx,
                                                             float* __restrict__ out, int B, long long D, float scale) {
// ... 105 lines not shown
    out[i] = accumulate == 2 ? scale : (accumulate ? out[i] + scale * in[i] : scale * in[i]);
}

inline unsigned ew_grid(size_t work_items) {
  size_t g = (work_items + 255) / 256;
  if (g > 256 * 8) g = 256 * 8;
  if (g < 1) g = 1;
  return (unsigned)g;
}

}

extern "C" {

int ladder_bn_fwd_stats(const float* x, float* sums, size_t rows, int C, void* ws, size_t ws_bytes, ladder_stream_t stream) {
  if (rows == 0 || C <= 0) return LADDER_E_SHAPE;
  const size_t nblk = stats_nblk(rows);
  if (ws_bytes < nblk * 2 * (size_t)C * sizeof(double)) return LADDER_E_WORKSPACE;
  if ((reinterpret_cast<uintptr_t>(sums) & 7u) != 0 || (reinterpret_cast<uintptr_t>(ws) & 7u) != 0) return LADDER_E_ALIGN;
  const size_t rpb = (rows + nblk - 1) / nblk;
  if (C % 4 == 0 && ladder_aligned16(x))
    hipLaunchKernelGGL(colstats64_stage1_v4<false>, dim3((C + 63) / 64, (unsigned)nblk), dim3(256), 0, stream, x, (double*)ws, (float*)nullptr, rows, C, rpb);
  else
    hipLaunchKernelGGL(colstats64_stage1, dim3((C + 63) / 64, (unsigned)nblk), dim3(256), 0, stream, x, (double*)ws, rows, C, rpb);
  hipLaunchKernelGGL(colstats64_stage2, dim3((2 * C + 63) / 64), dim3(1024), 0, stream, (const double*)ws, (const float*)nullptr, sums, (int)nblk, C);
  LADDER_CHECK_LAUNCH();
  return LADDER_OK;
}

int ladder_bn_stats_from_partials(const float* partials, int nblk, float* sums, int C, ladder_stream_t stream) {
  if (nblk <= 0 || C <= 0) return LADDER_E_SHAPE;
  hipLaunchKernelGGL(colstats_stage2_wide, dim3((2 * C + 15) / 16), dim3(256), 0, stream, partials, sums, nblk, C);
  LADDER_CHECK_LAUNCH();
  return LADDER_OK;
}

int ladder_bn_fwd_apply(const float* x, const float* sums, double count, const float* gamma, const float* beta, float* y,
                        float* mean_rstd, size_t rows, int C, float eps, int act, ladder_stream_t stream) {
  return ladder_bn_fwd_apply_absmax(x, sums, count, gamma, beta, y, mean_rstd, rows, C, eps, act, nullptr, stream);
}

int ladder_bn_fwd_apply_absmax(const float* x, const float* sums, double count, const float* gamma, const float* beta, float* y,
                               float* mean_rstd, size_t rows, int C, float eps, int act, float* y_absmax, ladder_stream_t stream) {
  if (rows == 0 || C <= 0 || count <= 0) return LADDER_E_SHAPE;
  if (y_absmax != nullptr) {
    if (!(C % 4 == 0 && ladder_aligned16(x) && ladder_aligned16(y))) return LADDER_E_SHAPE;
  }
  const size_t n = rows * (size_t)C;
  static const bool fold = getenv("LADDER_DISABLE_BN_FOLD") == nullptr;
  if (fold && y_absmax == nullptr && C % 4 == 0 && ladder_aligned16(x) && ladder_aligned16(y) && ladder_aligned16(gamma) && ladder_aligned16(beta) &&
      ((size_t)ew_grid(n / 4) * 256 * 4) % (size_t)C == 0) {
    hipLaunchKernelGGL(bn_apply_fin_kernel, dim3(ew_grid(n / 4)), dim3(256), 0, stream, x, sums, count, eps, mean_rstd, gamma, beta, y, n, C, act);
    LADDER_CHECK_LAUNCH();
    return LADDER_OK;
  }
  hipLaunchKernelGGL(bn_finalize_kernel, dim3((C + 255) / 256), dim3(256), 0, stream, sums, count, eps, mean_rstd, C, y_absmax);
  if (C % 4 == 0 && ladder_aligned16(x) && ladder_aligned16(y))
    hipLaunchKernelGGL(bn_apply_kernel, dim3(ew_grid(n / 4)), dim3(256), 0, stream, x, mean_rstd, gamma, beta, y, n, C, act, y_absmax);
  else
    hipLaunchKernelGGL(bn_apply_scalar_kernel, dim3(ew_grid(n)), dim3(256), 0, stream, x, mean_rstd, gamma, beta, y, n, C, act);
  LADDER_CHECK_LAUNCH();
  return LADDER_OK;
}

int ladder_bn_fwd_stats_minmax(const float* x, float* sums4, size_t rows, int C, void* ws, size_t ws_bytes, ladder_stream_t stream) {
  if (rows == 0 || C <= 0 || (C % 4) != 0) return LADDER_E_SHAPE;
  if (!ladder_aligned16(x)) return LADDER_E_ALIGN;
  const size_t nblk = stats_nblk(rows);
  if (ws_bytes < nblk * (2 * (size_t)C * sizeof(double) + 2 * (size_t)C * sizeof(float))) return LADDER_E_WORKSPACE;
  if ((reinterpret_cast<uintptr_t>(sums4) & 7u) != 0 || (reinterpret_cast<uintptr_t>(ws) & 7u) != 0) return LADDER_E_ALIGN;
  const size_t rpb = (rows + nblk - 1) / nblk;
  float* wsmm = reinterpret_cast<float*>(reinterpret_cast<double*>(ws) + nblk * 2 * (size_t)C);
  hipLaunchKernelGGL(colstats64_stage1_v4<true>, dim3((C + 63) / 64, (unsigned)nblk), dim3(256), 0, stream, x, (double*)ws, wsmm, rows, C, rpb);
  hipLaunchKernelGGL(colstats64_stage2, dim3((4 * C + 63) / 64), dim3(1024), 0, stream, (const double*)ws, (const float*)wsmm, sums4, (int)nblk, C);
  LADDER_CHECK_LAUNCH();
  return LADDER_OK;
}

int ladder_bn_stats_minmax_from_partials(const float* partials, int nblk, float* sums4, int C, ladder_stream_t stream) {
  if (nblk <= 0 || C <= 0) return LADDER_E_SHAPE;
  hipLaunchKernelGGL(colstats_minmax_stage2, dim3((4 * C + 15) / 16), dim3(1024), 0, stream, partials, sums4, nblk, C);
  LADDER_CHECK_LAUNCH();
  return LADDER_OK;
}

int ladder_bn_fwd_apply_planes(const float* x, const float* sums4, double count, const float* gamma, const float* beta, float* y, void* y_planes,
                               float* mean_rstd, size_t rows, int C, float eps, int act, float* y_absmax, ladder_stream_t stream) {
  if (rows == 0 || C <= 0 || count <= 0 || (C % 4) != 0 || y_planes == nullptr || y_absmax == nullptr) return LADDER_E_SHAPE;
  const size_t n = rows * (size_t)C;
  if ((n % 8) != 0) return LADDER_E_SHAPE;
  if (!ladder_aligned16(x) || !ladder_aligned16(y_planes) || (y != nullptr && !ladder_aligned16(y))) return LADDER_E_ALIGN;
  hipLaunchKernelGGL(bn_finalize_minmax_kernel, dim3(1), dim3(256), 0, stream, sums4, count, eps, mean_rstd, gamma, beta, C, act, y_absmax);
  hipLaunchKernelGGL(bn_apply_planes_kernel, dim3(ew_grid(n / 4)), dim3(256), 0, stream, x, (const float*)mean_rstd, gamma, beta, y,
                     (uint16_t*)y_planes, n, C, act, (const float*)y_absmax);
  LADDER_CHECK_LAUNCH();
  return LADDER_OK;
}

int ladder_bn_bwd_stats(const float* dy, const float* x, const float* mean_rstd, const float* gamma, const float* beta,
                        float* dsums, size_t rows, int C, int act, void* ws, size_t ws_bytes, ladder_stream_t stream) {
  if (rows == 0 || C <= 0) return LADDER_E_SHAPE;
  const size_t nblk = stats_nblk(rows);
  if (ws_bytes < nblk * 2 * (size_t)C * sizeof(float)) return LADDER_E_WORKSPACE;
  const size_t rpb = (rows + nblk - 1) / nblk;
  if (C % 4 == 0 && ladder_aligned16(x) && ladder_aligned16(dy))
    hipLaunchKernelGGL(colstats_stage1_v4<2>, dim3((C + 63) / 64, (unsigned)nblk), dim3(256), 0, stream, dy, x, mean_rstd, gamma, beta,
                       (float*)ws, rows, C, rpb, act);
  else
    hipLaunchKernelGGL(colstats_stage1<2>, dim3((C + 63) / 64, (unsigned)nblk), dim3(256), 0, stream, dy, x, mean_rstd, gamma, beta,
                       (float*)ws, rows, C, rpb, act);
  hipLaunchKernelGGL(colstats_stage2, dim3((2 * C + 63) / 64), dim3(1024), 0, stream, (const float*)ws, dsums, (int)nblk, C);
  LADDER_CHECK_LAUNCH();
  return LADDER_OK;
}

int ladder_bn_bwd_apply(const float* dy, const float* x, const float* mean_rstd, const float* gamma, const float* beta,
                        const float* dsums, double count, float* dx, float* dgamma, float* dbeta, size_t rows, int C, int act,
                        ladder_stream_t stream) {
  return ladder_bn_bwd_apply_absmax(dy, x, mean_rstd, gamma, beta, dsums, count, dx, dgamma, dbeta, rows, C, act, nullptr, stream);
}

int ladder_bn_bwd_apply_absmax(const float* dy, const float* x, const float* mean_rstd, const float* gamma, const float* beta,
                               const float* dsums, double count, float* dx, float* dgamma, float* dbeta, size_t rows, int C, int act,
                               float* dx_absmax, ladder_stream_t stream) {
  if (rows == 0 || C <= 0 || count <= 0) return LADDER_E_SHAPE;
  const size_t n = rows * (size_t)C;
  if (dx_absmax != nullptr) {
    if (!(dx != nullptr && C % 4 == 0 && ladder_aligned16(x) && ladder_aligned16(dy) && ladder_aligned16(dx))) return LADDER_E_SHAPE;
  }
  const bool pgrad = dgamma != nullptr && dbeta != nullptr;
  const bool v4 = dx != nullptr && C % 4 == 0 && ladder_aligned16(x) && ladder_aligned16(dy) && ladder_aligned16(dx);
  static const bool fold = getenv("LADDER_DISABLE_BN_FOLD") == nullptr;
  const bool pgrad_rides = fold && pgrad && v4 && dx_absmax == nullptr;
  if (pgrad && !pgrad_rides)
    hipLaunchKernelGGL(bn_param_grad_kernel, dim3((C + 255) / 256), dim3(256), 0, stream, dsums, dgamma, dbeta, C, dx_absmax);
  else if (!pgrad && dx_absmax != nullptr && hipMemsetAsync(dx_absmax, 0, LADDER_ABSMAX_FLOATS * sizeof(float), stream) != hipSuccess)
    return LADDER_E_LAUNCH;
  if (dx != nullptr) {
    if (v4)
      hipLaunchKernelGGL(bn_bwd_apply_v4_kernel, dim3(ew_grid(n / 4)), dim3(256), 0, stream, dy, x, mean_rstd, gamma, beta, dsums,
                         (float)(1.0 / count), dx, n, C, act, dx_absmax, pgrad_rides ? dgamma : (float*)nullptr, pgrad_rides ? dbeta : (float*)nullptr);
    else
      hipLaunchKernelGGL(bn_bwd_apply_kernel, dim3(ew_grid(n)), dim3(256), 0, stream, dy, x, mean_rstd, gamma, beta, dsums,
                         (float)(1.0 / count), dx, n, C, act);
  }
  LADDER_CHECK_LAUNCH();
  return LADDER_OK;
}

size_t ladder_bn_workspace_bytes(size_t rows, int C) { return stats_nblk(rows) * 2 * (size_t)C * sizeof(double); }

size_t ladder_in_style_workspace_bytes(int N, int HW, int C) { return (size_t)N * in_split(N, HW, C) * 2 * C * sizeof(float); }

int ladder_in_style_fwd(const float* x, const float* style, float* y, float* mean_rstd, int N, int HW, int C, float eps, int act,
                        void* ws, size_t ws_bytes, ladder_stream_t stream) {
  return ladder_in_style_fwd_absmax(x, style, y, mean_rstd, N, HW, C, eps, act, ws, ws_bytes, nullptr, stream);
}

int ladder_in_style_fwd_absmax(const float* x, const float* style, float* y, float* mean_rstd, int N, int HW, int C, float eps, int act,
                               void* ws, size_t ws_bytes, float* y_absmax, ladder_stream_t stream) {
  if (N <= 0 || HW <= 0 || C <= 0) return LADDER_E_SHAPE;
  if (y_absmax != nullptr) {
    if (!(C % 4 == 0 && ws != nullptr && ws_bytes >= ladder_in_style_workspace_bytes(N, HW, C) && ladder_aligned16(x) && ladder_aligned16(y)))
      return LADDER_E_SHAPE;
  }
  if (C % 4 == 0 && ws != nullptr && ws_bytes >= ladder_in_style_workspace_bytes(N, HW, C) && ladder_aligned16(x) && ladder_aligned16(y)) {
    const int sp = in_split(N, HW, C);
    dim3 grid((C + 63) / 64, N, sp);
    hipLaunchKernelGGL(in_stats_kernel, grid, dim3(256), 0, stream, x, (float*)ws, HW, C, sp);
    hipLaunchKernelGGL(in_finalize_kernel, dim3((N * C + 255) / 256), dim3(256), 0, stream, x, (const float*)ws, mean_rstd, N, HW, C, sp, eps, y_absmax);
    hipLaunchKernelGGL(in_apply_kernel, grid, dim3(256), 0, stream, x, style, (const float*)mean_rstd, y, HW, C, act, sp, y_absmax);
    LADDER_CHECK_LAUNCH();
    return LADDER_OK;
  }
  hipLaunchKernelGGL(in_style_fwd_kernel, dim3((C + 63) / 64, N), dim3(256), 0, stream, x, style, y, mean_rstd, HW, C, eps, act);
  LADDER_CHECK_LAUNCH();
  return LADDER_OK;
}

int ladder_in_style_fwd_resize2x(const float* x, const float* style, float* up, float* mean_rstd, int N, int H, int W, int C, float eps,
                                 int act, void* ws, size_t ws_bytes, float* up_absmax, ladder_stream_t stream) {
  return ladder_in_style_fwd_resize2x_keep(x, style, up, nullptr, mean_rstd, N, H, W, C, eps, act, ws, ws_bytes, up_absmax, stream);
}

int ladder_in_style_fwd_resize2x_keep(const float* x, const float* style, float* up, float* y, float* mean_rstd, int N, int H, int W, int C,
                                      float eps, int act, void* ws, size_t ws_bytes, float* up_absmax, ladder_stream_t stream) {
  if (N <= 0 || H <= 0 || W <= 0 || C <= 0) return LADDER_E_SHAPE;
  if (y != nullptr && !ladder_aligned16(y)) return LADDER_E_ALIGN;
  const int HW = H * W;
  if (!(C % 4 == 0 && ws != nullptr && ws_bytes >= ladder_in_style_workspace_bytes(N, HW, C) && ladder_aligned16(x) && ladder_aligned16(up)))
    return LADDER_E_SHAPE;
  const int sp = in_split(N, HW, C);
  dim3 grid((C + 63) / 64, N, sp);
  hipLaunchKernelGGL(in_stats_kernel, grid, dim3(256), 0, stream, x, (float*)ws, HW, C, sp);
  hipLaunchKernelGGL(in_finalize_kernel, dim3((N * C + 255) / 256), dim3(256), 0, stream, x, (const float*)ws, mean_rstd, N, HW, C, sp, eps, up_absmax);
  const long units = (long)HW * (C / 4);
  hipLaunchKernelGGL(in_apply_resize2x_kernel, dim3((unsigned)((units + 255) / 256), N), dim3(256), 0, stream, x, style,
                     (const float*)mean_rstd, up, H, W, C, act, up_absmax, y);
  LADDER_CHECK_LAUNCH();
  return LADDER_OK;
}

int ladder_in_style_bwd(const float* dy, const float* x, const float* style, const float* mean_rstd, float* dx, float* dstyle,
                        int N, int HW, int C, int act, void* ws, size_t ws_bytes, ladder_stream_t stream) {
  return ladder_in_style_bwd_absmax(dy, x, style, mean_rstd, dx, dstyle, N, HW, C, act, ws, ws_bytes, nullptr, stream);
}

int ladder_in_style_bwd_absmax(const float* dy, const float* x, const float* style, const float* mean_rstd, float* dx, float* dstyle,
                               int N, int HW, int C, int act, void* ws, size_t ws_bytes, float* dx_absmax, ladder_stream_t stream) {
  if (N <= 0 || HW <= 0 || C <= 0) return LADDER_E_SHAPE;
  if (dx_absmax != nullptr) {
    if (!(C % 4 == 0 && ws != nullptr && ws_bytes >= ladder_in_style_workspace_bytes(N, HW, C) && ladder_aligned16(x) && ladder_aligned16(dy) &&
          ladder_aligned16(dx)))
      return LADDER_E_SHAPE;
  }
  if (C % 4 == 0 && ws != nullptr && ws_bytes >= ladder_in_style_workspace_bytes(N, HW, C) && ladder_aligned16(x) && ladder_aligned16(dy) &&
      ladder_aligned16(dx)) {
    const int sp = in_split(N, HW, C);
    dim3 grid((C + 63) / 64, N, sp);
    hipLaunchKernelGGL(in_bwd_stats_kernel, grid, dim3(256), 0, stream, dy, x, style, mean_rstd, (float*)ws, HW, C, act, sp);
    hipLaunchKernelGGL(in_bwd_finalize_kernel, dim3((N * C + 255) / 256), dim3(256), 0, stream, (const float*)ws, dstyle, N, C, sp, dx_absmax);
    hipLaunchKernelGGL(in_bwd_apply_kernel, grid, dim3(256), 0, stream, dy, x, style, mean_rstd, (const float*)dstyle, dx, HW, C, act, sp, dx_absmax);
    LADDER_CHECK_LAUNCH();
    return LADDER_OK;
  }
  hipLaunchKernelGGL(in_style_bwd_kernel, dim3((C + 63) / 64, N), dim3(256), 0, stream, dy, x, style, mean_rstd, dx, dstyle, HW, C, act);
  LADDER_CHECK_LAUNCH();
  return LADDER_OK;
}

static int resize_launch(bool fwd, const float* a, float* b, int N, int H, int W, int C, int OH, int OW, hipStream_t stream,
                         const float* gate_y = nullptr, int gate_act = 0) {
  if (N <= 0 || H <= 0 || W <= 0 || C <= 0 || OH < H || OW < W || OH % H || OW % W) return LADDER_E_SHAPE;
  if (gate_y != nullptr && (fwd || OH != 2 * H || OW != 2 * W)) return LADDER_E_SHAPE;
  const bool v4 = (C % 4 == 0) && ladder_aligned16(a) && ladder_aligned16(b) && (gate_y == nullptr || ladder_aligned16(gate_y));
  const int CV = v4 ? C / 4 : C;
  const long bprl = ((long)W * CV + 255) / 256;
  if (bprl * N * H >= (1L << 31)) return LADDER_E_SHAPE;
  const int bpr = (int)bprl;
  const dim3 grid((unsigned)(bprl * N * H)), block(256);
  const int fy = OH / H, fx = OW / W;
  if (fwd) {
    if (v4) hipLaunchKernelGGL(resize_fwd_kernel<4>, grid, block, 0, stream, a, b, H, W, CV, fy, fx, bpr);
    else hipLaunchKernelGGL(resize_fwd_kernel<1>, grid, block, 0, stream, a, b, H, W, CV, fy, fx, bpr);
  } else {
    if (fy == 2 && fx == 2) {
      if (v4) hipLaunchKernelGGL(resize_bwd_x2_kernel<4>, grid, block, 0, stream, a, b, H, W, CV, bpr, gate_y, gate_act);
      else hipLaunchKernelGGL(resize_bwd_x2_kernel<1>, grid, block, 0, stream, a, b, H, W, CV, bpr, gate_y, gate_act);
    } else if (v4) hipLaunchKernelGGL(resize_bwd_kernel<4>, grid, block, 0, stream, a, b, H, W, CV, fy, fx, bpr);
    else hipLaunchKernelGGL(resize_bwd_kernel<1>, grid, block, 0, stream, a, b, H, W, CV, fy, fx, bpr);
  }
  LADDER_CHECK_LAUNCH();
  return LADDER_OK;
}

int ladder_resize_bilinear_fwd(const float* x, float* y, int N, int H, int W, int C, int OH, int OW, ladder_stream_t stream) {
  return resize_launch(true, x, y, N, H, W, C, OH, OW, stream);
}

int ladder_resize_bilinear_bwd(const float* dy, float* dx, int N, int H, int W, int C, int OH, int OW, ladder_stream_t stream) {
  return resize_launch(false, dy, dx, N, H, W, C, OH, OW, stream);
}

int ladder_resize_bilinear_bwd_gated(const float* dy, float* dx, int N, int H, int W, int C, int OH, int OW, const float* gate_y, int gate_act,
                                     ladder_stream_t stream) {
  if (gate_y == nullptr) return LADDER_E_SHAPE;
  return resize_launch(false, dy, dx, N, H, W, C, OH, OW, stream, gate_y, gate_act);
}

int ladder_gather_rows(const void* src, int src_is_u8, const int64_t* idx, float* out, int B, int64_t D, float scale,
                       ladder_stream_t stream) {
  if (B <= 0 || D <= 0) return LADDER_E_SHAPE;
  const long long total = (long long)B * D;
  if (src_is_u8 && (D % 16) == 0 && ladder_aligned16(src) && ladder_aligned16(out)) {
    hipLaunchKernelGGL(gather_rows_u8_kernel, dim3(ew_grid((size_t)(total / 16))), dim3(256), 0, stream, (const unsigned char*)src,
                       (const long long*)idx, out, B, (long long)D, scale);
  } else if (src_is_u8) {
    hipLaunchKernelGGL(gather_rows_scalar_kernel<unsigned char>, dim3(ew_grid((size_t)total)), dim3(256), 0, stream,
                       (const unsigned char*)src, (const long long*)idx, out, B, (long long)D, scale);
  } else {
    hipLaunchKernelGGL(gather_rows_scalar_kernel<float>, dim3(ew_grid((size_t)total)), dim3(256), 0, stream, (const float*)src,
                       (const long long*)idx, out, B, (long long)D, scale);
  }
  LADDER_CHECK_LAUNCH();
  return LADDER_OK;
}

int ladder_depth_to_space(const float* x, float* y, int N, int H, int W, int C, int r, int inverse, ladder_stream_t stream) {
  if (N <= 0 || H <= 0 || W <= 0 || C <= 0 || r <= 0 || C % (r * r)) return LADDER_E_SHAPE;
  const int seg = C / r;
  const bool v4 = (seg % 4 == 0) && ladder_aligned16(x) && ladder_aligned16(y);
  const long per_row = (long)W * seg / (v4 ? 4 : 1);
  const long bpr = (per_row + 255) / 256, rows = (long)N * H * r;
  if (bpr * rows >= (1L << 31) || (long)W * seg >= (1L << 31)) return LADDER_E_SHAPE;
  if (v4) hipLaunchKernelGGL(d2s_kernel<4>, dim3((unsigned)(bpr * rows)), dim3(256), 0, stream, x, y, H, W, C, r, inverse, (int)bpr);
  else hipLaunchKernelGGL(d2s_kernel<1>, dim3((unsigned)(bpr * rows)), dim3(256), 0, stream, x, y, H, W, C, r, inverse, (int)bpr);
  LADDER_CHECK_LAUNCH();
  return LADDER_OK;
}

int ladder_pad_symmetric(const float* x, float* y, int N, int H, int W, int C, int p, ladder_stream_t stream) {
  if (N <= 0 || H <= 0 || W <= 0 || C <= 0 || p < 0 || p > H || p > W) return LADDER_E_SHAPE;
  hipLaunchKernelGGL(pad_sym_kernel, dim3(ew_grid((size_t)N * (H + 2 * p) * (W + 2 * p) * C)), dim3(256), 0, stream, x, y, N, H, W, C, p);
  LADDER_CHECK_LAUNCH();
  return LADDER_OK;
}

int ladder_pad_symmetric_bwd(const float* dy, float* dx, int N, int H, int W, int C, int p, ladder_stream_t stream) {
  if (N <= 0 || H <= 0 || W <= 0 || C <= 0 || p < 0 || p > H || p > W) return LADDER_E_SHAPE;
  hipLaunchKernelGGL(pad_sym_bwd_kernel, dim3(ew_grid((size_t)N * H * W * C)), dim3(256), 0, stream, dy, dx, N, H, W, C, p);
  LADDER_CHECK_LAUNCH();
  return LADDER_OK;
}

int ladder_act_bwd(const float* dy, const float* y, float* dx, size_t n, int act, ladder_stream_t stream) {
  if (n == 0) return LADDER_OK;
  hipLaunchKernelGGL(act_bwd_kernel, dim3(ew_grid(n / 4 + 1)), dim3(256), 0, stream, dy, y, dx, n, act);
  LADDER_CHECK_LAUNCH();
  return LADDER_OK;
}

int ladder_axpy(const float* in, float* out, size_t n, float scale, int accumulate, ladder_stream_t stream) {
  if (n == 0) return LADDER_OK;
  hipLaunchKernelGGL(axpy_kernel, dim3(ew_grid(n)), dim3(256), 0, stream, in, out, n, scale, accumulate);
  LADDER_CHECK_LAUNCH();
  return LADDER_OK;
}

}
```

### ladder_latent_data_distribution_modelling_amd/engine.py

```python
import os

import numpy as np
import torch

from . import _lib as L
from . import arch
from . import layers as _layers
from .comm import Comm, VirtualComm, VirtualGroup, run_virtual_ranks, _NoComm, _DoneWork, _TracedWork
from .layers import (ADAM_B1, ADAM_B2, ADAM_EPS, BN_EPS, DEFAULT_PRECISION, IN_EPS, PRECISION_NOTES, PRECISIONS, BatchNormAct, Conv2D, Ctx, Dense,
                     DepthToSpace, InstanceNormStyleAct, ParamStore, PlanesOnly, Resize, _p, _timed, add_, pad_symmetric, plan_decoder)
from .profiler import KernelProfiler


def set_profiler(prof):
    _layers.PROF = prof


class Encoder:
    def __init__(self, ctx, ps, cfg):
        self.ctx, self.cfg = ctx, cfg
        self.exp = cfg["exp_name"]
        self.convs, self.bns = [], []
        for i, (cin, cout, k, s, pad, act, bn) in enumerate(arch.encoder_convs(cfg)):
            self.convs.append(Conv2D(ctx, ps, "encoder/" + arch.tfname("conv2d", i), k, cin, cout, s, pad, act, bias_grad=not bn, want_bn_sums=bool(bn)))
            self.bns.append(BatchNormAct(ctx, ps, "encoder/" + arch.tfname("batch_normalization", i), cout, "leaky_relu") if bn else None)
        feat, hid = arch.encoder_flat_dim(cfg), arch.encoder_hidden(cfg)
        self.hidden = Dense(ctx, ps, "encoder/dense", feat, hid, "leaky_relu") if hid is not None else None
        feat = hid if hid is not None else feat
        Z = int(cfg["code_size"])
        self.head_mu = Dense(ctx, ps, "encoder/code_mean", feat, Z, None)
        self.head_sd = Dense(ctx, ps, "encoder/code_std_dev", feat, Z, "relu")

    def forward(self, x):
        h = pad_symmetric(self.ctx, x, 2) if self.exp != "celeba" else x
        for i, (conv, bn) in enumerate(zip(self.convs, self.bns)):
            h = conv.forward(h)
            if bn is not None:
                nxt = self.convs[i + 1] if i + 1 < len(self.convs) else None
                h = bn.forward(h, sums=conv.bn_sums, planes=nxt.planes_demand(h.shape) if nxt is not None else (False, True))
            conv.bn_sums = None
        self.conv_shape = h.shape
        h = h.reshape(h.shape[0], -1)
        if self.hidden is not None:
            h = self.hidden.forward(h)
        return self.head_mu.forward(h), self.head_sd.forward(h)

    def backward(self, dmu, dsd_raw, wgrad=True, need_input_dx=False):
        dh = self.head_mu.backward(dmu, wgrad=wgrad)
        add_(self.ctx, dh, self.head_sd.backward(dsd_raw, wgrad=wgrad, act_done=True))
        if self.hidden is not None:
            dh = self.hidden.backward(dh, wgrad=wgrad)
        dh = dh.reshape(self.conv_shape)
        for i in range(len(self.convs) - 1, -1, -1):
            if self.bns[i] is not None:
                dh = self.bns[i].backward(dh, wgrad=wgrad)
            dh = self.convs[i].backward(dh, need_dx=(i > 0 or need_input_dx), wgrad=wgrad)
        if need_input_dx and self.exp != "celeba":
            N, Hp, Wp, C = dh.shape
            dx = self.ctx.empty(N, Hp - 4, Wp - 4, C)
            L.call("ladder_pad_symmetric_bwd", _p(dh), _p(dx), N, Hp - 4, Wp - 4, C, 2, self.ctx.stream)
            dh = dx
        return dh if need_input_dx else None


class MnistDecoder:
    def __init__(self, ctx, ps, cfg):
        self.ctx = ctx
        width, r0, convs = arch.mnist_decoder_convs(cfg)
        self.dense = Dense(ctx, ps, "decoder/dense", int(cfg["code_size"]), width, "leaky_relu")
        self.d2s0 = DepthToSpace(ctx, r0)
        self.convs, self.d2s = [], []
        for i, (k, ci, co, pad, act, d) in enumerate(convs):
            self.convs.append(Conv2D(ctx, ps, "decoder/" + arch.tfname("conv2d", i), k, ci, co, 1, pad, act))
            self.d2s.append(DepthToSpace(ctx, d) if d else None)

    def forward(self, z):
        h = self.dense.forward(z)
        h = self.d2s0.forward(h.view(h.shape[0], 1, 1, -1))
        for conv, d in zip(self.convs, self.d2s):
            h = conv.forward(h)
            if d is not None:
                h = d.forward(h)
        return h

    def backward(self, dxhat, need_dz=True):
        dh = dxhat
        for conv, d in zip(reversed(self.convs), reversed(self.d2s)):
            if d is not None:
                dh = d.backward(dh)
            dh = conv.backward(dh)
        dh = self.d2s0.backward(dh)
        return self.dense.backward(dh.reshape(dh.shape[0], -1), need_dx=need_dz)


class CelebADecoder:

    def __init__(self, ctx, ps, cfg):
        self.ctx = ctx
        nh, Z = int(cfg["num_hidden_units"]), int(cfg["code_size"])
        self.nh = nh
        self.dense0 = Dense(ctx, ps, "decoder/dense", Z, nh, "leaky_relu")
        self.mapping = [Dense(ctx, ps, "decoder/dense_%d" % i, nh, nh, "leaky_relu") for i in range(1, 9)]
        self.conv0 = Conv2D(ctx, ps, "decoder/conv2d", 1, nh, nh, 1, "same", None)
        self.up0 = Resize(ctx, 2, 2)
        self.blocks = []
        si = 0
        for i, (k, ci, co, styled, act, rs) in enumerate(arch.celeba_decoder_convs(cfg)):
            conv = Conv2D(ctx, ps, "decoder/conv2d_%d" % (i + 1), k, ci, co, 1, "same", act, bias_grad=not styled)
            sty = norm = None
            if styled:
                sty = Dense(ctx, ps, "decoder/StyleMod_%d/dense" % si, nh, 2 * co, None)
                norm = InstanceNormStyleAct(ctx, co, "leaky_relu")
                si += 1
            self.blocks.append((conv, sty, norm, Resize(ctx, rs, rs) if rs else None))
        self.conv_out = Conv2D(ctx, ps, "decoder/conv2d_8", 1, nh // 4, int(cfg["dim_input_channel"]), 1, "same", None)
        self._plans, self.plan = {}, None

    def forward(self, z):
        B = z.shape[0]
        encoded = self.dense0.forward(z)
        d = encoded
        for lyr in self.mapping:
            d = lyr.forward(d)
        dlatent = d
        keep = self.ctx.keep_activations
        h = self.conv0.forward(encoded.view(B, 1, 1, self.nh))
        plan = plan_decoder(self._plans, self.ctx, self.up0, self.blocks, self.conv_out, tuple(h.shape[:3]))
        if keep:
            self.plan = plan
        h, lo = (None, h) if plan[0].resize in ("virtual", "fold_forward_only") else (self.up0.forward(h), None)
        for e, (conv, sty, norm, rs) in zip(plan, self.blocks):
            proj = self.conv_out if e.proj else None
            if e.form != "plain":
                h = conv.forward_up2(lo, e, proj, keep_y=keep, upsampled=h)
            elif proj is not None:
                h = conv.forward_fused_proj(h, proj, keep_y=keep)
            else:
                h = conv.forward(h)
            if proj is not None:
                return h
            lo = None
            if norm is not None:
                style = sty.forward(dlatent)
                h, lo = (norm.forward(h, style), None) if e.norm_out == "lowres" else norm.forward_resized(h, style, rs, e.norm_out == "both")
            if e.behind in ("virtual", "fold_forward_only"):
                h, lo = None, h
            elif e.behind is not None and e.norm_out in (None, "lowres"):
                h, lo = rs.forward(h), (h if e.behind == "keep_both" else None)
        return self.conv_out.forward(h)

    def backward(self, dxhat, need_dz=True):
        ctx, plan = self.ctx, self.plan
        last = plan[-1]
        dh = None if last.proj_grad else self.conv_out.backward(dxhat, gate_prev=self.blocks[-1][0].act if last.fuse_last else None)
        ddlat = None
        for i in range(len(self.blocks) - 1, -1, -1):
            e, (conv, sty, norm, rs) = plan[i], self.blocks[i]
            if e.gated:
                dh, _ = rs.backward(dh, gate=(conv.kept.y, conv.act))
            elif e.rs_bwd:
                dh = rs.backward(dh)
            if norm is not None:
                dh, dstyle = norm.backward(dh)
                g = sty.backward(dstyle)
                ddlat = g if ddlat is None else add_(ctx, ddlat, g)
            below = self.blocks[i - 1][0]
            dh = conv.backward(dh, act_done=e.fuse_last or e.gated or e.pre_gated, lowres_dx=e.lowres_dx,
                               lowres_gate=(below.kept.y, below.act) if e.lgate else None, proj_grad=(dxhat, self.conv_out) if e.proj_grad else None)
        dh = self.conv0.backward(dh if plan[0].lowres_dx else self.up0.backward(dh))
        denc = dh.reshape(dh.shape[0], self.nh)
        for i in range(len(self.mapping) - 1, -1, -1):
            ddlat = self.mapping[i].backward(ddlat, act_done=(i < len(self.mapping) - 1), gate_prev="leaky_relu" if i > 0 else None)
        add_(ctx, denc, ddlat)
        return self.dense0.backward(denc, need_dx=need_dz)


class InnerVAE:

    def __init__(self, ctx, ps, cfg):
        self.ctx = ctx
        Z, H = int(cfg["code_size"]), int(cfg["num_hidden_units_inner_VAE"])
        R, nl = int(cfg["representation_size"]), int(cfg["n_layers_inner_VAE"])
        a = cfg["inner_activation"]
        dims = [(Z, H)] + [(H, H)] * (nl - 1)
        self.enc = [Dense(ctx, ps, "prior/" + arch.tfname("dense", i), ci, co, a) for i, (ci, co) in enumerate(dims)]
        self.head_mu = Dense(ctx, ps, "prior/" + arch.tfname("dense", nl), H, R, None)
        self.head_sd = Dense(ctx, ps, "prior/" + arch.tfname("dense", nl + 1), H, R, "relu")
        dims = [(R, H)] + [(H, H)] * (nl - 1)
        self.dec = [Dense(ctx, ps, "prior/" + arch.tfname("dense", nl + 2 + i), ci, co, a) for i, (ci, co) in enumerate(dims)]
        self.dec_out = Dense(ctx, ps, "prior/" + arch.tfname("dense", 2 * nl + 2), H, Z, None)

    def encode(self, z):
        h = z
        for lyr in self.enc:
            h = lyr.forward(h)
        return self.head_mu.forward(h), self.head_sd.forward(h)

    def decode(self, t):
        h = t
        for lyr in self.dec:
            h = lyr.forward(h)
        return self.dec_out.forward(h)

    def decode_backward(self, dzhat, wgrad):
        a = self.dec[0].act
        dh = self.dec_out.backward(dzhat, wgrad=wgrad, gate_prev=a)
        for i in range(len(self.dec) - 1, -1, -1):
            dh = self.dec[i].backward(dh, wgrad=wgrad, act_done=True, gate_prev=a if i > 0 else None)
        return dh

    def encode_backward(self, dmu, dsd_raw, wgrad, need_dz):
        dh = self.head_mu.backward(dmu, wgrad=wgrad)
        add_(self.ctx, dh, self.head_sd.backward(dsd_raw, wgrad=wgrad, act_done=True))
        a = self.enc[0].act
        for i in range(len(self.enc) - 1, -1, -1):
            dh = self.enc[i].backward(dh, need_dx=(need_dz or i > 0), wgrad=wgrad, act_done=(i < len(self.enc) - 1),
                                      gate_prev=a if i > 0 else None)
        return dh


class _AsyncFetch:

    def __init__(self, host, event, names, pool, undefined=()):
        self._host, self._event, self._names, self._pool, self._val = host, event, names, pool, None
        self._undefined = frozenset(undefined)

    def ready(self):
        return self._val is not None or self._event.query()

    def get(self):
        if self._val is None:
            self._event.synchronize()
            s = self._host.numpy()
            self._val = {n: (float("nan") if n in self._undefined else float(s[L.S_INDEX[n]])) for n in self._names}
            self._pool.append(self._host)
            self._host = None
        return self._val


DEC_SCALARS = frozenset(("sigma", "mean_pixel_error", "l1_reconstruction_error", "l2_reconstruction_error", "reconstruction_likelihood",
                         "sigma_regularisor", "elbo", "loss_ae"))


PRIOR_METHODS = arch.PRIOR_METHODS


class PriorSampler:

    def __init__(self, eng, method, K, R, params, seed=0, offset=0):
        self.eng, self.method, self.K, self.R, self.params = eng, method, int(K), int(R), params
        self.seed, self.offset = int(seed), int(offset)
        self.to_code = method in ("ours", "hierarchical")

    def sample(self, n, first=0, noise=None, seed=None):
        eng, n = self.eng, int(n)
        ctx = eng.ctx
        latent = ctx.empty(n, self.R)
        comp = torch.empty(n, dtype=torch.int32, device=ctx.device)
        u = eps = None
        if noise is not None:
            u, eps = eng._dev(noise["u"]).reshape(-1), eng._dev(noise["eps"])
            if tuple(u.shape) != (n,) or tuple(eps.shape) != (n, self.R):
                raise ValueError("noise: u %s, eps %s; expected (%d,) and (%d, %d)" % (tuple(u.shape), tuple(eps.shape), n, n, self.R))
        L.call("ladder_mixture_sample", _p(self.params), self.K, self.R, n, int(first), _p(u), _p(eps),
               self.seed if seed is None else int(seed), self.offset, _p(latent), _p(comp), ctx.stream)
        code = eng.decode_representation(latent) if self.to_code else latent
        return code, latent, comp


class LadderEngine:

    def __init__(self, cfg, device="cuda:0", values=None, seed=1, comm=None, noise_seed=1234):
        self.cfg = cfg
        if comm is None and bool(int(cfg.get("deterministic_allreduce", 0))):
            comm = Comm(deterministic=True)
        self.ctx = Ctx(device, comm)
        prec = str(cfg.get("matmul_precision", DEFAULT_PRECISION))
        if prec not in PRECISIONS:
            raise ValueError("matmul_precision %r: expected one of %s" % (prec, sorted(PRECISIONS)))
        self.ctx.ns = PRECISIONS[prec]
        self.ctx.up2 = int(cfg.get("upsample_fused_convs", 4 if prec == "f32" else 2))
        self.ctx.fuse_fwd = int(cfg.get("fused_projected_forward", 2))
        self.ctx.fuse_bwd_proj = int(cfg.get("fused_projection_backward", 1))
        self.precision = prec
        if self.ctx.comm.rank == 0:
            print("Contraction precision (config key matmul_precision): {} -- {}".format(prec, PRECISION_NOTES[prec]))
        self.ps = ParamStore(cfg, self.ctx, values, seed)
        self.encoder = Encoder(self.ctx, self.ps, cfg)
        self.decoder = (CelebADecoder if cfg["exp_name"] == "celeba" else MnistDecoder)(self.ctx, self.ps, cfg)
        self.has_inner = cfg["prior"] in ("ours", "hierarchical")
        self.hier = cfg["prior"] == "hierarchical"
        self.gmm_z = cfg["prior"] == "GMM"
        self.vamp = cfg["prior"] == "vampPrior"
        if cfg["prior"] not in ("ours", "hierarchical", "GMM", "vampPrior", "standard_gaussian"):
            raise ValueError("unknown prior %r" % cfg["prior"])
        if self.vamp:
            self.encoder_p = Encoder(self.ctx.local(), self.ps, cfg)
            self._enc_range = self.ps.prefix_range("ae", "encoder/")
        self.inner = InnerVAE(self.ctx, self.ps, cfg) if self.has_inner else None
        self.Z = int(cfg["code_size"])
        self.R = int(cfg["code_size"]) if cfg["prior"] in ("GMM", "vampPrior") else int(cfg.get("representation_size", 1))
        self.K = int(cfg.get("n_mixtures", 1))
        self.Lmc = int(cfg.get("n_MC_samples", 1))
        self.D = int(cfg["dim_input_x"]) * int(cfg["dim_input_y"]) * int(cfg["dim_input_channel"])
        self.lvp = float(cfg["latent_variance_precision"])
        self.partials = self.ctx.zeros(L.P_FIXED + self.Z + self.R)
        self.scalars = self.ctx.zeros(L.S_COUNT)
        self.noise_seed = int(noise_seed) + 7919 * self.ctx.comm.rank
        self.rng_counter = torch.zeros(1, dtype=torch.int64, device=self.ctx.device)
        self._run_calls = 0
        self._gm_packed = None
        self.use_graphs = False
        if bool(int(cfg.get("overlap_filter_gradients", os.environ.get("LADDER_OVERLAP_FILTER_GRADIENTS", 0)))):
            self.ctx.side = torch.cuda.Stream(device=self.ctx.device)
        self._graphs, self._warm = {}, {}
        self._dec_range = self.ps.prefix_range("ae", "decoder/")
        self.ps.before_read = self._join_aux
        self._aux_on = False
        self._enc_event, self._aux_event = None, None
        self._main_calls, self._aux_calls = 0, 0
        self._on_aux = False
        self._fetch_src = None
        self._sigma_one = torch.ones(1, dtype=torch.float32, device=self.ctx.device)

    def enable_prior_overlap(self, on=True):
        on = bool(on) and not self.ctx.comm.on
        self._aux_on = on
        if on and self.ctx.aux is None:
            self.ctx.aux = torch.cuda.Stream(device=self.ctx.device, priority=int(os.environ.get("LADDER_AUX_PRIORITY", -1)))
            self.partials_aux, self.scalars_aux = torch.zeros_like(self.partials), torch.zeros_like(self.scalars)
            self.rng_counter_aux = torch.zeros_like(self.rng_counter)

    def _join_aux(self):
        if self._aux_event is not None:
            torch.cuda.current_stream(self.ctx.device).wait_event(self._aux_event)
            self._aux_event = None
            self._aux_calls = 0

    def _dev(self, a):
        if a is None:
            return None
        if isinstance(a, torch.Tensor):
            return a.to(device=self.ctx.device, dtype=torch.float32).contiguous()
        return torch.as_tensor(np.ascontiguousarray(a, dtype=np.float32)).to(self.ctx.device)

    @staticmethod
    def _batch_token(x):
        if isinstance(x, torch.Tensor):
            return ("t", x.data_ptr(), tuple(x.shape))
        a = np.asarray(x)
        return ("n", a.__array_interface__["data"][0], tuple(a.shape))

    def _randn(self, *shape):
        t = self.ctx.empty(*shape)
        if self._on_aux:
            L.call("ladder_randn_dev", _p(t), t.numel(), self.noise_seed, _p(self.rng_counter_aux),
                   self._main_calls + self._aux_calls + self._run_calls, self.ctx.stream)
        else:
            L.call("ladder_randn_dev", _p(t), t.numel(), self.noise_seed, _p(self.rng_counter), self._run_calls, self.ctx.stream)
        self._run_calls += 1
        return t

    def _noise(self, noise, key, shape):
        if noise is not None and noise.get(key) is not None:
            t = self._dev(noise[key])
            assert tuple(t.shape) == tuple(shape), (key, t.shape, shape)
            return t
        return self._randn(*shape)

    def set_mixture(self, weights, means, covs):
        K, R = self.K, self.R
        w, m, c = self._dev(weights), self._dev(means), self._dev(covs)
        assert tuple(w.shape) == (K,) and tuple(m.shape) == (K, R) and tuple(c.shape) == (K, R, R)
        self._gm_dense = R > 8
        if getattr(self, "_gm_buf", None) is None:
            self._gm_buf = self.ctx.empty(L.query("ladder_gmm_dense_param_floats", K, R) if self._gm_dense
                                          else K * L.query("ladder_gmm_packed_stride", R))
        L.call("ladder_gmm_prepare_dense" if self._gm_dense else "ladder_gmm_prepare", _p(w), _p(m), _p(c), K, R, _p(self._gm_buf),
               self.ctx.stream)
        torch.cuda.current_stream(self.ctx.device).synchronize()
        self._gm_packed = self._gm_buf

    def set_sg_mixture(self):
        K, R = self.K, self.R
        self.set_mixture(np.full(K, 1.0 / K), np.zeros((K, R)), np.tile(np.eye(R), (K, 1, 1)))

    def forward(self, x, noise=None, use_sg=True, use_mask=False, parts=("dec", "inner", "gmm"), reuse_encoder=False, keep_acts=True):
        ctx, st = self.ctx, self.ctx.stream
        if not self._on_aux:
            self._join_aux()
            self._fetch_src = (self.scalars, torch.cuda.current_stream(ctx.device))
        ctx.keep_activations = bool(keep_acts)
        Z, R = self.Z, self.R
        P = self.partials
        L.call("ladder_axpy", None, _p(P), P.numel(), 0.0, 2, st)
        self._run_calls = 0
        use_mask = bool(use_mask) and not self.hier
        tok = self.__dict__.pop("_x_token", None) or self._batch_token(x)
        cache = getattr(self, "_enc_cache", None)
        if (reuse_encoder and cache is not None and cache[0] == self.ps.step["ae"] and cache[4] == tok
                and not self._enc_needs_grad(parts)):
            _, x, mu, sd_raw, _ = cache
        else:
            x = self._dev(x)
            mu, sd_raw = self.encoder.forward(x)
            self._enc_cache = (self.ps.step["ae"], x, mu, sd_raw, tok)
        B = x.shape[0]
        self.x, self.B = x, B
        self.Bg = B * ctx.comm.world
        eps_z = self._noise(noise, "eps_z", (B, Z))
        z, sd = ctx.empty(B, Z), ctx.empty(B, Z)
        L.call("ladder_latent_fwd", _p(mu), _p(sd_raw), _p(eps_z), self.lvp, _p(z), _p(sd), _p(P[L.P_LOG_SDZ:]),
               _p(P[L.P_MU2SD2_Z:]), _p(P[L.P_FIXED:]), B, Z, st)
        self.lat_z = (mu, sd, sd_raw, eps_z, z)
        early_aux = "inner" not in parts and "gmm" not in parts
        if early_aux:
            self._mark_for_aux()
        self.xhat = None
        if "dec" in parts:
            xhat = self.decoder.forward(z)
            nb = L.query("ladder_pixel_partials_workspace_bytes", x.numel())
            wsp, wsn = ctx.ws(nb)
            L.call("ladder_pixel_partials", _p(x), _p(xhat), x.numel(), _p(P[L.P_PIX_ABS:]), wsp, wsn, st)
            self.xhat = xhat
        if self.gmm_z and "gmm" in parts:
            self.gmm_grads = self._mixture_term(mu, sd, noise, B, need_grad="gmm_grad" in parts)
        vamp_on = self.vamp and "gmm" in parts and not use_sg
        if vamp_on:
            self.gmm_grads = self._vamp_term(mu, sd, noise, B)
        inner_on = self.has_inner and "inner" in parts
        if inner_on:
            mu_t, sdraw_t = self.inner.encode(z)
            eps_t = self._noise(noise, "eps_t", (B, R))
            t, sd_t = ctx.empty(B, R), ctx.empty(B, R)
            L.call("ladder_latent_fwd", _p(mu_t), _p(sdraw_t), _p(eps_t), self.lvp, _p(t), _p(sd_t), _p(P[L.P_LOG_SDT:]),
                   _p(P[L.P_MU2SD2_T:]), _p(P[L.P_FIXED + Z:]), B, R, st)
# ... 443 lines not shown
```

### ladder_latent_data_distribution_modelling_amd/layers.py

```python
import functools
import os
from collections import namedtuple

import numpy as np
import torch

from . import _lib as L
from . import arch
from .comm import Comm, _NoComm

BN_EPS = 1e-3
IN_EPS = 1e-6
ADAM_B1, ADAM_B2, ADAM_EPS = 0.9, 0.95, 1e-8


def _p(t):
    return None if t is None else t.data_ptr()


PRECISIONS = {"f32": 0, "bf16x3": 2, "bf16x6": 3, "f16x3": 4}
DEFAULT_PRECISION = "f32"

PRECISION_NOTES = {
    "f32": "native fp32 MFMA (v_mfma_f32_32x32x2_f32), bit-exact fp32 FMA chains",
    "f16x3": "fp32-class EMULATION: fp32 operands as 2 scaled fp16 planes (22 significand bits, power-of-two scales per sample / "
             "per tensor, see DESIGN 4a), 3 fp16 MFMAs per product, fp32 accumulation; set \"matmul_precision\": \"f32\" for strict fp32",
    "bf16x6": "fp32-class EMULATION: 3 bf16 planes (24 bits), 6 bf16 MFMAs per product, fp32 accumulation",
    "bf16x3": "REDUCED precision: 2 bf16 planes (16 bits), 3 bf16 MFMAs per product (between TF32 and fp32)"}

PROF = None


def _igemm_plan(M, Cin, Cout, Kdim, conv=None):
    nb = L.query("ladder_igemm_fwd_workspace_bytes", M, Kdim, Cout)
    kid = L.query("ladder_conv2d_fwd_kernel_id", *conv) if conv else L.query("ladder_igemm_fwd_tile", M, Cin, Cout)
    if kid != 256128 and nb and L.query("ladder_igemm_fwd_splits", M, Kdim, Cout) > 1:
        kid = 0
    return nb or None, kid if kid in (256128, 128128) else 0


def _timed(kid, flops, name, args, executed=None):
    if PROF is None or not kid:
        L.call(name, *args)
        return
    s, e = torch.cuda.Event(enable_timing=True), torch.cuda.Event(enable_timing=True)
    s.record()
    L.call(name, *args)
    e.record()
    PROF.add(kid, s, e, flops, executed)


class PlanesOnly:

    def __init__(self, shape):
        self.shape = torch.Size(shape)

    def numel(self):
        n = 1
        for d in self.shape:
            n *= int(d)
        return n

    def data_ptr(self):
        raise RuntimeError("this activation exists only as fp16 planes (PlanesOnly): an fp32 kernel was routed to it")


class Ctx:

    def __init__(self, device, comm=None):
        self.device = torch.device(device)
        if self.device.type != "cuda":
            raise L.LadderHipError("the LaDDer HIP path needs a GPU device (got %s); there is no CPU fallback" % device)
        L.load()
        self.comm = comm or Comm()
        self._ws = torch.empty(1 << 20, dtype=torch.uint8, device=self.device)
        self._ws_retired, self.ws_generation = [], 0
        self._amax = {}
        self._planes = {}
        self.pack_banks, self._pack_table = [], None
        self.side, self._side_active, self._side_refs = None, False, []
        self._ws_side = torch.empty(1 << 20, dtype=torch.uint8, device=self.device)
        self._ws_side_retired = []
        self.aux = None
        self._ws_aux = None
        self.keep_activations = True
        self.ns = 0
        self.up2_used = {}
        self.up2_skipped = {}
        self.fuse_bwd_proj = 1
        self.fuse_fwd = 2
        self.up2 = True

    @property
    def sfx(self):
        return "" if self.ns else "_f32"

    @property
    def stream(self):
        return torch.cuda.current_stream(self.device).cuda_stream

    def fork_side(self, *keep):
        ev = torch.cuda.Event()
        ev.record()
        self.side.wait_event(ev)
        self._side_refs.extend(k for k in keep if k is not None)
        self._side_active = True
        return torch.cuda.stream(self.side)

    def side_or_main(self, *keep):
        if self.side is None or torch.cuda.is_current_stream_capturing():
            import contextlib
            return contextlib.nullcontext()
        return self.fork_side(*keep)

    def join_side(self):
        if self._side_active:
            torch.cuda.current_stream(self.device).wait_stream(self.side)
            self._side_active = False
            self._side_refs.clear()
            self._ws_side_retired.clear()

    def ws(self, nbytes):
        if nbytes is None:
            return None, 0
        if self.aux is not None and torch.cuda.current_stream(self.device) == self.aux:
            if self._ws_aux is None or self._ws_aux.numel() < nbytes:
                self._ws_aux = torch.empty(int(nbytes * 1.25) + 256, dtype=torch.uint8, device=self.device)
            return self._ws_aux.data_ptr(), self._ws_aux.numel()
        if self.side is not None and torch.cuda.current_stream(self.device) == self.side:
            if self._ws_side.numel() < nbytes:
                self._ws_side_retired.append(self._ws_side)
                self._ws_side = torch.empty(int(nbytes * 1.25) + 256, dtype=torch.uint8, device=self.device)
            return self._ws_side.data_ptr(), self._ws_side.numel()
        if self._ws.numel() < nbytes:
            self._ws_retired.append(self._ws)
            self._ws = torch.empty(int(nbytes * 1.25) + 256, dtype=torch.uint8, device=self.device)
            self.ws_generation += 1
        return self._ws.data_ptr(), self._ws.numel()

    def empty(self, *shape):
        return torch.empty(*shape, dtype=torch.float32, device=self.device)

    def new_amax(self):
        return torch.empty(L.ABSMAX_FLOATS, dtype=torch.float32, device=self.device)

    def set_amax(self, t, rec):
        if self.ns == 4 and rec is not None:
            import weakref
            k, reg = id(t), self._amax
            reg[k] = (weakref.ref(t, lambda _r, k=k, reg=reg: reg.pop(k, None)), rec)

    def known_amax(self, t):
        e = self._amax.get(id(t))
        return e[1] if e is not None and e[0]() is t else None

    def drop_amax(self, t):
        self._amax.pop(id(t), None)
        self._planes.pop(id(t), None)

    def absmax(self, t):
        if self.ns != 4:
            return None
        rec = self.known_amax(t)
        if rec is None:
            rec = self.new_amax()
            per = t.numel() // int(t.shape[0]) if t.dim() >= 2 else 0
            if per and per % 4 == 0 and int(t.shape[0]) > 1:
                L.call("ladder_absmax_samples", _p(t), int(t.shape[0]), per, _p(rec), self.stream)
            else:
                L.call("ladder_absmax", _p(t), t.numel(), _p(rec), self.stream)
            self.set_amax(t, rec)
        return rec

    def set_planes(self, t, buf):
        import weakref
        k, reg = id(t), self._planes
        reg[k] = (weakref.ref(t, lambda _r, k=k, reg=reg: reg.pop(k, None)), buf)

    def planes(self, t, per_sample=False):
        e = self._planes.get(id(t))
        if e is not None and e[0]() is t:
            return e[1]
        import weakref
        buf = torch.empty(L.query("ladder_presplit_bytes", t.numel(), self.ns), dtype=torch.uint8, device=self.device)
        ns = int(t.shape[0]) if (per_sample and t.dim() == 4 and (t.numel() // int(t.shape[0])) % 8 == 0) else 0
        L.call("ladder_presplit", _p(t), _p(self.absmax(t)), _p(buf), t.numel(), ns, self.ns, self.stream)
        k, reg = id(t), self._planes
        reg[k] = (weakref.ref(t, lambda _r, k=k, reg=reg: reg.pop(k, None)), buf)
        return buf

    def zeros(self, *shape):
        return torch.zeros(*shape, dtype=torch.float32, device=self.device)

    def local(self):
        import copy
        c = copy.copy(self)
        c.comm = _NoComm()
        return c


class ParamStore:

    ALIGN = 64

    def __init__(self, cfg, ctx, values=None, seed=1):
        self.cfg, self.ctx = cfg, ctx
        self.specs = arch.param_specs(cfg)
        values = values if values is not None else arch.init_values(cfg, seed)
        self.offsets, sizes = {}, {}
        for name, shp in self.specs.items():
            g = arch.group_of(name)
            off = sizes.get(g, 0)
            n = int(np.prod(shp)) if len(shp) else 1
            self.offsets[name] = (g, off, n)
            sizes[g] = off + (n + self.ALIGN - 1) // self.ALIGN * self.ALIGN
        self.theta = {g: ctx.zeros(n) for g, n in sizes.items()}
        self.grad = {g: ctx.zeros(n) for g, n in sizes.items()}
        self.m = {g: ctx.zeros(n) for g, n in sizes.items()}
        self.v = {g: ctx.zeros(n) for g, n in sizes.items()}
        self.step = {g: 0 for g in sizes}
        self.version = {g: 0 for g in sizes}
        self.adam_state = {g: ctx.zeros(4) for g in sizes}
        self._lr_host = {g: None for g in sizes}
        self.w, self.g = {}, {}
        for name, shp in self.specs.items():
            g, off, n = self.offsets[name]
            self.w[name] = self.theta[g][off:off + n].view(*shp) if len(shp) else self.theta[g][off:off + 1]
            self.g[name] = self.grad[g][off:off + n].view(*shp) if len(shp) else self.grad[g][off:off + 1]
        self.load_dict(values)

    def prefix_range(self, group, prefix):
        runs = [(off, off + (n + self.ALIGN - 1) // self.ALIGN * self.ALIGN, name.startswith(prefix))
                for name, (g, off, n) in self.offsets.items() if g == group]
        runs.sort()
        inside = [r for r in runs if r[2]]
        if not inside:
            return None
        lo, hi = inside[0][0], inside[-1][1]
        if any(lo <= r[0] < hi and not r[2] for r in runs):
            return None
        return lo, hi
# ... 337 lines not shown

    def _fwd_s2(self, r, x, y):
        _timed(r.fwd.kid, r.flops, r.fwd.fn, (_p(x), _p(self._packed_filter(BANK_S2_FWD)), self._wb()[1], _p(y), r.N, r.H, r.W, self.cin, r.Ho, r.Wo,
                                              self.cout, L.ACT[self.act], self.ctx.stream))

    def _fwd_gather(self, r, x, y):
        wsp, wsn = self.ctx.ws(r.fwd.ws)
        _timed(r.fwd.kid, r.flops, r.fwd.fn, (_p(x), *self._wb(), _p(y), *r.geo, L.ACT[self.act], *self._sums(r), wsp, wsn, self.ctx.stream))

    def _backward_proj(self, dy, need_dx, wgrad, gate, proj_grad=None):
        ctx, st = self.ctx, self.ctx.stream
        x, f = self.kept.x, self.kept.factor
        N, H, W, _ = x.shape
        M, n9 = N * H * W, 9 * self.cout
        flops = 2.0 * N * f * f * H * W * 9 * self.cin * self.cout
        executed = 2.0 * M * self.cin * n9
        d = ctx.empty(M, n9)
        if proj_grad is not None:
            dyp, proj = proj_grad
            wsp, wsn = ctx.ws(L.query("ladder_up2proj_bwd_combine_proj_workspace_bytes", N, H, W, self.cout, proj.cout))
            L.call("ladder_up2proj_bwd_combine_proj", _p(self.kept.y), _p(dyp), _p(proj.ps.w[proj.name + "/kernel"]), _p(d), _p(proj.ps.g[proj.name + "/kernel"]),
                   _p(proj.ps.g[proj.name + "/bias"]) if proj.bias_grad else None, proj.cout, N, H, W, self.cout, L.ACT[self.act] if self.act else 0,
                   wsp, wsn, st)
            proj.kept = None
        else:
            L.call("ladder_upfproj_bwd_combine", _p(dy), _p(d), f, N, H, W, self.cout, st)
        if wgrad:
            self._count_up2(":wgrad", 1.0 - 1.0 / (f * f))
            dwcat, db9 = ctx.empty(self.cin, n9), (ctx.empty(n9) if self.bias_grad else None)
            wsp, wsn = ctx.ws(L.query("ladder_dense_bwd_weight_workspace_bytes", M, self.cin, n9))
            _timed(9132 if L.query("ladder_dense_bwd_weight_is_persistent", M, self.cin, n9) else 9130, flops, "ladder_dense_bwd_weight",
                   (_p(x), _p(d), _p(dwcat), _p(db9), M, self.cin, n9, wsp, wsn, st), executed)
            L.call("ladder_up2proj_wgrad_unpack", _p(dwcat), _p(db9), _p(self.ps.g[self.name + "/kernel"]),
                   _p(self.ps.g[self.name + "/bias"]) if self.bias_grad else None, self.cin, self.cout, st)
        dx = None
        if need_dx:
            self._count_up2(":bwd", 1.0 - 1.0 / (f * f))
            dx = ctx.empty(N, H, W, self.cin)
            wsp, wsn = ctx.ws(L.query("ladder_igemm_fwd_workspace_bytes", M, n9, self.cin))
            gy, gact = gate if gate is not None else (None, None)
            if L.query("ladder_dense_fwd_is_persistent", M, n9, self.cin):
                _timed(128134, flops, "ladder_dense_bwd_data_nt",
                       (_p(d), _p(self._packed_filter(BANK_PROJ)), _p(dx), M, self.cin, n9, _p(gy), L.ACT[gact] if gact else 0, st), executed)
            else:
                _timed(abs(L.query("ladder_igemm_fwd_tile", M, n9, self.cin)), flops, "ladder_dense_bwd_data",
                       (_p(d), _p(self._packed_filter(BANK_PROJ_T)), _p(dx), M, self.cin, n9, _p(gy), L.ACT[gact] if gact else 0, wsp, wsn, st), executed)
        return dx

    def _dx_lowres(self, dy, dy_amax, kid, gate=None):
        ctx, st = self.ctx, self.ctx.stream
        N, OH, OW, _ = dy.shape
        H, W = OH // 2, OW // 2
        dx = ctx.empty(N, H, W, self.cin)
        dx_amax = ctx.new_amax() if ctx.ns == 4 else None
        flops = 2.0 * N * OH * OW * 9 * self.cin * self.cout
        self._count_up2(":bwd", 11.0 / 36.0)
        pk4 = self._packed_filter(BANK_UP2_BWD)
        if ctx.ns == 0:
            wsp, wsn = ctx.ws(L.query("ladder_conv3x3_up2_bwd_borders_workspace_bytes", N, H, W, self.cout, self.cin))
            if gate is not None:
                gy, gact = gate
                _timed(kid, flops, "ladder_conv3x3_up2_bwd_data_gated_f32",
                       (_p(dy), _p(pk4), _p(dx), _p(gy), L.ACT[gact], N, H, W, self.cout, self.cin, st), flops * 25.0 / 36.0)
                L.call("ladder_conv3x3_up2_bwd_borders_gated", _p(dy), _p(self.ps.w[self.name + "/kernel"]), _p(dx), _p(gy), L.ACT[gact], N, H, W, self.cout,
                       self.cin, wsp, wsn, st)
                return dx
            _timed(kid, flops, "ladder_conv3x3_up2_bwd_data_split",
                   (_p(dy), None, _p(pk4), _p(dx), None, N, H, W, self.cout, self.cin, 0, st), flops * 25.0 / 36.0)
            L.call("ladder_conv3x3_up2_bwd_borders", _p(dy), _p(self.ps.w[self.name + "/kernel"]), _p(dx), N, H, W, self.cout, self.cin, wsp, wsn, st)
            return dx
        pk = self._packed_filter(BANK_BWD)
        strips = []
        for axis, first in ((1, True), (1, False), (2, True), (2, False)):
            n_dy, n_up = (3, 2) if first else (4, 3)
            O_ = OH if axis == 1 else OW
            sl = slice(0, n_dy) if first else slice(O_ - n_dy, O_)
            pad = 1 if first else 2
            if axis == 1:
                geo = (N, n_up, OW, self.cin, n_dy, OW, self.cout, 3, 3, 1, pad, 1)
                view, s, dup = dy[:, sl], ctx.empty(N, n_dy, OW, self.cout), ctx.empty(N, n_up, OW, self.cin)
            else:
                geo = (N, OH, n_up, self.cin, OH, n_dy, self.cout, 3, 3, 1, 1, pad)
                view, s, dup = dy[:, :, sl], ctx.empty(N, OH, n_dy, self.cout), ctx.empty(N, OH, n_up, self.cin)
            strips.append((axis, first, geo, view, s, dup))
        _timed(256120 + ctx.ns, flops, "ladder_conv3x3_up2_bwd_data_split",
               (_p(dy), _p(dy_amax), _p(pk4), _p(dx), _p(dx_amax), N, H, W, self.cout, self.cin, ctx.ns, st), flops * 25.0 / 36.0)
        for axis, first, geo, view, s, dup in strips:
            s.copy_(view)
            ctx.set_amax(s, dy_amax)
            s_amax = ctx.absmax(s)
            wsp, wsn = ctx.ws(L.query("ladder_conv2d_bwd_data_split_workspace_bytes", *geo))
            L.call("ladder_conv2d_bwd_data_split", _p(ctx.planes(s, self._ps(geo[1], geo[2]))), _p(s_amax), _p(pk), _p(dup), *geo, None, 0, ctx.ns, wsp, wsn, st)
            L.call("ladder_conv3x3_up2_bwd_border", _p(dup), _p(dx), _p(dx_amax), N, H, W, self.cin, axis, 1 if first else 0, st)
        ctx.set_amax(dx, dx_amax)
        return dx

    def backward(self, dy, need_dx=True, wgrad=True, act_done=False, gate_prev=None, lowres_dx=False, lowres_gate=None, proj_grad=None):
        try:
            return self._backward(self.kept, dy, need_dx, wgrad, act_done, gate_prev, lowres_dx, lowres_gate, proj_grad)
        finally:
            self.kept = None

    def _backward(self, k, dy, need_dx, wgrad, act_done, gate_prev, lowres_dx, lowres_gate, proj_grad):
        r, x, x_amax, ctx = k.route, k.x, k.x_amax, self.ctx
        lo = k.x_kind == "lowres"
        if proj_grad is not None:
            if not (wgrad and lo and k.form == "projected" and k.factor == 2):
                raise RuntimeError("%s: the projection-gradient form of the backward combination does not apply" % self.name)
            return self._backward_proj(None, need_dx, wgrad, lowres_gate, proj_grad)
        if self.act is not None and not act_done:
            L.call("ladder_act_bwd", _p(dy), _p(k.y), _p(dy), dy.numel(), L.ACT[self.act], ctx.stream)
        if lo and k.form == "projected":
            return self._backward_proj(dy, need_dx, wgrad, lowres_gate)
        if wgrad and r.fused_bwd is not None:
            return r.fused_bwd.run(r, x, dy, need_dx, gate_prev)
        wg, dl = r.wgrad if wgrad else None, (r.dx_gated if gate_prev else r.dx) if need_dx else None
        halo_w, halo_d = bool(wg and wg.fn == "ladder_conv3x3_wgrad_split"), bool(dl and dl.fn == "ladder_conv3x3_split")
        if halo_w and x_amax is None:
            x_amax = ctx.absmax(x)
        dy_amax = ctx.absmax(dy) if (halo_w or halo_d) else None
        if wg is not None:
            wg.run(r, x, dy, x_amax, dy_amax, lo)
        if lowres_dx:
            if not halo_d:
                raise RuntimeError("%s: the low-resolution backward-data was requested for a call the split halo kernels do not take" % self.name)
            return self._dx_lowres(dy, dy_amax, r.up2_kids[1], lowres_gate)
        if dl is None:
            return None
        dx = ctx.empty(r.N, r.H, r.W, self.cin)
        dl.run(r, dl, x, dy, dx, dy_amax, gate_prev)
        return dx

    def _bwd_smallcout(self, r, x, dy, need_dx, gate):
        ctx, M = self.ctx, r.N * r.H * r.W
        wsp, wsn = ctx.ws(r.fused_bwd.ws)
        dx = ctx.empty(r.N, r.H, r.W, self.cin) if need_dx else None
        dx_amax = ctx.new_amax() if (need_dx and ctx.ns == 4) else None
        L.call(r.fused_bwd.fn, _p(x), _p(dy), self._wb()[0], _p(dx), *self._grads(), M, self.cin, self.cout, L.ACT[gate] if gate else 0, wsp, wsn,
               _p(dx_amax), r.H * r.W, ctx.stream)
        if dx is not None:
            ctx.set_amax(dx, dx_amax)
        return dx

    def _wg_dense(self, r, x, dy, x_amax, dy_amax, lo):
        L.call(r.wgrad.fn, _p(x), _p(dy), *self._grads(), r.N * r.H * r.W, self.cin, self.cout, self.ctx.stream)

    def _wg_rgb(self, r, x, dy, x_amax, dy_amax, lo):
        ctx = self.ctx
        xa, da = (ctx.absmax(x), ctx.absmax(dy)) if ctx.ns else (None, None)
        with ctx.side_or_main(x, dy, xa, da):
            wsp, wsn = ctx.ws(r.wgrad.ws)
            ops = (_p(x), _p(xa), _p(dy), _p(da)) if ctx.ns else (_p(x), _p(dy))
            L.call(r.wgrad.fn, *ops, *self._grads(), r.N, r.H, r.W, self.cout, wsp, wsn, ctx.stream)

    def _wg_halo_split(self, r, x, dy, x_amax, dy_amax, lo):
        ctx = self.ctx
        with ctx.side_or_main(x, dy, x_amax, dy_amax):
            wsp, wsn = ctx.ws(r.wgrad.ws)
            _timed(r.wgrad.kid, r.flops, r.wgrad.fn, (_p(x), _p(x_amax), _p(dy), _p(dy_amax), *self._grads(), r.N, r.H, r.W, self.cin, self.cout,
                                                            ctx.ns, wsp, wsn, ctx.stream))

    def _wg_gather_split(self, r, x, dy, x_amax, dy_amax, lo):
        ctx = self.ctx
        x_amax, dy_amax = ctx.absmax(x) if x_amax is None else x_amax, ctx.absmax(dy)
        ps_ = self._ps(r.Ho, r.Wo)
        xpl, dpl = ctx.planes(x, ps_), ctx.planes(dy, ps_)
        with ctx.side_or_main(x, dy, xpl, dpl, x_amax, dy_amax):
            wsp, wsn = ctx.ws(r.wgrad.ws)
            L.call(r.wgrad.fn, _p(xpl), _p(x_amax), _p(dpl), _p(dy_amax), *self._grads(), *r.geo, ctx.ns, wsp, wsn, ctx.stream)

    def _wg_up2(self, r, x, dy, x_amax, dy_amax, lo):
        ctx, fl = self.ctx, r.flops
        wsp, wsn = ctx.ws(r.wgrad.ws)
        self._count_up2(":wgrad", 11.0 / 36.0)
        _timed(r.wgrad.kid, fl, r.wgrad.fn, (_p(x), 0 if lo else 1, _p(dy), *self._grads(), r.N, r.H // 2, r.W // 2, self.cin, self.cout, wsp, wsn,
                                            ctx.stream), fl * 25.0 / 36.0)

    def _wg_gather(self, r, x, dy, x_amax, dy_amax, lo):
        assert not lo, "%s: virtual upsample without the low-resolution filter gradient" % self.name
        wsp, wsn = self.ctx.ws(r.wgrad.ws)
        _timed(r.wgrad.kid, r.flops, r.wgrad.fn, (_p(x), _p(dy), *self._grads(), *r.geo, wsp, wsn, self.ctx.stream))

    def _dx_dense(self, r, dl, x, dy, dx, dy_amax, gate):
        gate_args = (_p(x), L.ACT[gate]) if gate else (None, 0)
        L.call(dl.fn, _p(dy), self._wb()[0], _p(dx), r.N * r.H * r.W, self.cin, self.cout, *gate_args, self.ctx.stream)

    def _dx_halo(self, r, dl, x, dy, dx, dy_amax, gate):
        ctx = self.ctx
        dx_amax = ctx.new_amax() if ctx.ns == 4 else None
        ctx.set_amax(dx, dx_amax)
        _timed(dl.kid, r.flops, dl.fn,
               (_p(dy), _p(dy_amax), _p(self._packed_filter(BANK_BWD)), None, _p(dx), _p(dx_amax), r.N, r.H, r.W, self.cout, self.cin, 0, ctx.ns, ctx.stream))

    def _dx_s2(self, r, dl, x, dy, dx, dy_amax, gate):
        ctx = self.ctx
        dy_amax = ctx.absmax(dy)
        dx_amax = ctx.new_amax() if ctx.ns == 4 else None
        ctx.set_amax(dx, dx_amax)
        _timed(dl.kid, 2.0 * r.N * r.Ho * r.Wo * 9 * self.cin * self.cout, dl.fn,
               (_p(dy), _p(dy_amax), _p(self._packed_filter(BANK_S2_BWD)), _p(dx), _p(dx_amax), r.N, r.H, r.W, self.cin, r.Ho, r.Wo, self.cout, ctx.ns, ctx.stream))

    def _dx_gather_split(self, r, dl, x, dy, dx, dy_amax, gate):
        ctx = self.ctx
        dy_amax = ctx.absmax(dy)
        wsp, wsn = ctx.ws(dl.ws)
        L.call(dl.fn, _p(ctx.planes(dy, self._ps(r.Ho, r.Wo))), _p(dy_amax), _p(self._packed_filter(BANK_BWD)), _p(dx), *r.geo,
               _p(x) if gate else None, L.ACT[gate] if gate else 0, ctx.ns, wsp, wsn, ctx.stream)

    def _dx_gather(self, r, dl, x, dy, dx, dy_amax, gate):
        ctx = self.ctx
        wT = self._packed_filter(dl.bank) if dl.bank is not None else ctx.empty(self.k * self.k * self.cin * self.cout)
        if dl.bank is None:
            L.call("ladder_filter_flip_transpose", self._wb()[0], _p(wT), self.k, self.k, self.cin, self.cout, ctx.stream)
        wsp, wsn = ctx.ws(dl.ws)
        _timed(dl.kid, 2.0 * r.N * r.H * r.W * self.k * self.k * self.cin * self.cout, dl.fn,
               (_p(dy), _p(wT), _p(dx), *r.geo, _p(x) if gate else None, L.ACT[gate] if gate else 0, wsp, wsn, ctx.stream))


PairPlan = namedtuple("PairPlan", "resize factor form one_launch proj norm_out behind lowres_dx lgate pre_gated gated rs_bwd fuse_last proj_grad")


def plan_decoder(cache, ctx, up0, blocks, conv_out, shape):
    keep, ns, up2 = ctx.keep_activations, ctx.ns, ctx.up2
    halo_sw, gate_sw = halo_disabled(), switch("LADDER_ENABLE_LOWRES_GATE") == "1"
    key = (tuple(shape), keep, ns, up2, ctx.fuse_fwd, ctx.fuse_bwd_proj, halo_sw, gate_sw)
    if key in cache:
        return cache[key]
    N = shape[0]
    halo_off = ns == 0 and halo_sw

    def c3(c):
        return c.k == 3 and c.stride == 1 and c.padding == "same"

    def factor(rs, H, W):
        return next((f for f in (2, 4) if rs is not None and (rs.oh, rs.ow) == (f * H, f * W)), 0)

    def proj_ok(c, H, W, f):
        return bool(ns == 0 and up2 >= 4 and c3(c) and not halo_sw and 36 * N * H * W * c.cout <= PROJ_MAX_BYTES
                    and L.query("ladder_upfproj_eligible", f, N, H, W, c.cin, c.cout))

    def fold_ok(c, H, W, f):
        if proj_ok(c, H, W, f):
            return True
        return bool(f == 2 and not halo_off and up2 and ns in (0, 2, 4) and c3(c) and L.query("ladder_conv3x3_up2_split_eligible", N, H, W, c.cin, c.cout, ns))

    def tap_bwd_ok(c, H, W):
        if halo_off:
            return False
        if ns == 0 and H * W < UP2T_MIN_PIXELS:
            return False
        return bool(up2 >= 2 and ns in (0, 2, 4) and c3(c) and L.query("ladder_conv3x3_up2_bwd_data_split_eligible", N, H, W, c.cout, c.cin, ns)
                    and (ns == 0 or all(L.query("ladder_conv2d_bwd_data_split_eligible", *g, 0) for g in (
                        (N, 2, 2 * W, c.cin, 3, 2 * W, c.cout, 3, 3, 1, 1, 1), (N, 3, 2 * W, c.cin, 4, 2 * W, c.cout, 3, 3, 1, 2, 1),
                        (N, 2 * H, 2, c.cin, 2 * H, 3, c.cout, 3, 3, 1, 1, 1), (N, 2 * H, 3, c.cin, 2 * H, 4, c.cout, 3, 3, 1, 1, 2)))))

    def virtual_ok(c, H, W, f):
        if proj_ok(c, H, W, f):
            return True
        return bool(f == 2 and ns == 0 and up2 >= 3 and fold_ok(c, H, W, 2) and tap_bwd_ok(c, H, W) and H * W >= UP2W_MIN_PIXELS
                    and L.query("ladder_conv3x3_up2_wgrad_eligible", N, H, W, c.cin, c.cout))

    n, fwd, front, (h, w) = len(blocks), [], up0, shape[1:3]
    for i, (conv, _, norm, rs) in enumerate(blocks):
        f, resize = factor(front, h, w), None
        if front is not None and (front.oh, front.ow) != (h, w):
            if not (f and fold_ok(conv, h, w, f)):
                resize = "materialise"
            elif not keep:
                resize = "fold_forward_only"
            elif virtual_ok(conv, h, w, f):
                resize = "virtual"
            elif i and up2 >= 2 and f == 2 and (blocks[i - 1][2] is None or blocks[i - 1][0].cout % 4 == 0):
                resize = "keep_both"
            else:
                resize = "materialise"
        lo_hw, (h, w) = (h, w), ((front.oh, front.ow) if front is not None else (h, w))
        last = i == n - 1 and norm is None and (rs is None or (rs.oh, rs.ow) == (h, w))
        if resize in (None, "materialise"):
            form, one_launch = "plain", False
            proj = "rides" if (last and conv.cout <= 128 and conv._is_projection(conv_out) and conv.route((N, h, w, conv.cin)).halo) else None
        else:
            form = "projected" if proj_ok(conv, lo_hw[0], lo_hw[1], f) else "tapfold"
            one_launch = bool(form == "projected" and f == 2 and ctx.fuse_fwd and L.query(
                "ladder_up2proj_fused_eligible" if ctx.fuse_fwd >= 2 else "ladder_up2proj_fused_preferred", N, lo_hw[0], lo_hw[1], conv.cin, conv.cout))
            proj = None if not (last and f == 2) else "rides" if (conv.cout == 128 and conv._is_projection(conv_out)) else "follows"
        fwd.append((resize, f, form, one_launch, proj, lo_hw, (h, w), last))
        front = rs
    plan, above_lowres, above_lgate = [None] * n, False, False
    for i in range(n - 1, -1, -1):
        conv, _, norm, rs = blocks[i]
        resize, f, form, one_launch, proj, (lh, lw), (ho, wo), last = fwd[i]
        if i + 1 < n:
            behind, fb = fwd[i + 1][0], fwd[i + 1][1]
        else:
            behind, fb = ("materialise" if rs is not None and (rs.oh, rs.ow) != (ho, wo) else None), factor(rs, ho, wo)
        norm_out = None if norm is None else "both" if behind == "keep_both" else \
            "resized" if (behind == "materialise" and fb == 2 and conv.cout % 4 == 0) else "lowres"
        lowres_dx = bool(keep and (resize == "virtual" or (
            resize in ("materialise", "keep_both") and i and f == 2 and (i == n - 1 or up2 >= 3) and tap_bwd_ok(conv, lh, lw))))
        below = blocks[i - 1] if i else None
        lgate = bool(lowres_dx and below is not None and below[2] is None and below[0].act is not None and gate_sw and (
            (resize == "virtual" and form == "projected")
            or (ns == 0 and L.query("ladder_conv3x3_up2_bwd_data_gated_f32_eligible", N, lh, lw, conv.cout, conv.cin))))
        fuse_last = bool(last and conv.act is not None)
        proj_grad = bool(keep and fuse_last and ctx.fuse_bwd_proj and resize == "virtual" and form == "projected" and f == 2
                         and conv.act in ("leaky_relu", "relu") and conv_out.k == 1 and conv_out.stride == 1 and conv_out.act is None
                         and conv_out.cin == conv.cout and L.query("ladder_up2proj_bwd_combine_proj_eligible", N, lh, lw, conv.cout, conv_out.cout))
        rs_bwd = bool(behind in ("materialise", "keep_both") and not above_lowres)
        gated = bool(rs_bwd and norm is None and conv.act is not None and not fuse_last and fb == 2)
        plan[i] = PairPlan(resize, f, form, one_launch, proj, norm_out, behind, lowres_dx, lgate, above_lgate, gated, rs_bwd, fuse_last, proj_grad)
        above_lowres, above_lgate = lowres_dx, lgate
    cache[key] = plan
    return plan


class Dense:

    def __init__(self, ctx, ps, name, cin, cout, act=None):
        self.ctx, self.ps, self.name, self.cin, self.cout, self.act = ctx, ps, name, cin, cout, act

    _plan = staticmethod(functools.lru_cache(maxsize=None)(_igemm_plan))

    def _igemm(self, name, M, K, Cout, *args):
        nb, kid = self._plan(M, K, Cout, K)
        _timed(kid, 2.0 * M * K * Cout, name, args + self.ctx.ws(nb) + (self.ctx.stream,))

    def _small(self, M):
        return bool(L.query("ladder_dense_small_eligible", M, self.cin, self.cout))

    def forward(self, x):
        M = x.shape[0]
        y = self.ctx.empty(M, self.cout)
        if self._small(M):
            L.call("ladder_dense_fwd_small" + self.ctx.sfx, _p(x), _p(self.ps.w[self.name + "/kernel"]), _p(self.ps.w[self.name + "/bias"]), _p(y),
                   M, self.cin, self.cout, L.ACT[self.act], self.ctx.stream)
        else:
            self._igemm("ladder_dense_fwd", M, self.cin, self.cout, _p(x), _p(self.ps.w[self.name + "/kernel"]), _p(self.ps.w[self.name + "/bias"]), _p(y),
                        M, self.cin, self.cout, L.ACT[self.act])
        self.x, self.y = x, y
        return y

    def backward(self, dy, need_dx=True, wgrad=True, act_done=False, gate_prev=None):
        x, y, st = self.x, self.y, self.ctx.stream
        M = x.shape[0]
        if self.act is not None and not act_done:
            L.call("ladder_act_bwd", _p(dy), _p(y), _p(dy), dy.numel(), L.ACT[self.act], st)
        if self._small(M):
            if wgrad and need_dx:
                dx = self.ctx.empty(M, self.cin)
                L.call("ladder_dense_bwd_small" + self.ctx.sfx, _p(x), _p(dy), _p(self.ps.w[self.name + "/kernel"]), _p(dx),
                       _p(self.ps.g[self.name + "/kernel"]), _p(self.ps.g[self.name + "/bias"]), M, self.cin, self.cout,
                       _p(x) if gate_prev else None, L.ACT[gate_prev] if gate_prev else 0, st)
                self.x = self.y = None
                return dx
            if wgrad:
                L.call("ladder_dense_bwd_weight_small" + self.ctx.sfx, _p(x), _p(dy), _p(self.ps.g[self.name + "/kernel"]),
                       _p(self.ps.g[self.name + "/bias"]), M, self.cin, self.cout, st)
            dx = None
            if need_dx:
                dx = self.ctx.empty(M, self.cin)
                L.call("ladder_dense_bwd_data_small" + self.ctx.sfx, _p(dy), _p(self.ps.w[self.name + "/kernel"]), _p(dx), M, self.cin, self.cout,
                       _p(x) if gate_prev else None, L.ACT[gate_prev] if gate_prev else 0, st)
            self.x = self.y = None
            return dx
        if wgrad:
            nb = L.query("ladder_dense_bwd_weight_workspace_bytes", M, self.cin, self.cout)
            wsp, wsn = self.ctx.ws(nb)
            L.call("ladder_dense_bwd_weight", _p(x), _p(dy), _p(self.ps.g[self.name + "/kernel"]),
                   _p(self.ps.g[self.name + "/bias"]), M, self.cin, self.cout, wsp, wsn, st)
        dx = None
        if need_dx:
            w = self.ps.w[self.name + "/kernel"]
            wT = self.ctx.empty(w.numel())
            L.call("ladder_filter_flip_transpose", _p(w), _p(wT), 1, 1, self.cin, self.cout, st)
            dx = self.ctx.empty(M, self.cin)
            self._igemm("ladder_dense_bwd_data", M, self.cout, self.cin, _p(dy), _p(wT), _p(dx), M, self.cin, self.cout,
                        _p(x) if gate_prev else None, L.ACT[gate_prev] if gate_prev else 0)
        self.x = self.y = None
        return dx


class BatchNormAct:

    def __init__(self, ctx, ps, name, C, act):
        self.ctx, self.ps, self.name, self.C, self.act = ctx, ps, name, C, act

    def forward(self, x, sums=None, planes=(False, True)):
        C, ctx = self.C, self.ctx
        rows = x.numel() // C
        want_planes, need_fp32 = planes
        want_planes = bool(want_planes and ctx.ns == 4 and C % 4 == 0 and x.numel() % 8 == 0)
        if sums is None:
            nb = L.query("ladder_bn_workspace_bytes", rows, C)
            if want_planes:
                wsp, wsn = ctx.ws(2 * nb)
                sums = ctx.empty(6 * C)
                L.call("ladder_bn_fwd_stats_minmax", _p(x), _p(sums), rows, C, wsp, wsn, ctx.stream)
            else:
                wsp, wsn = ctx.ws(nb)
                sums = ctx.empty(4 * C)
                L.call("ladder_bn_fwd_stats", _p(x), _p(sums), rows, C, wsp, wsn, ctx.stream)
        want_planes = want_planes and sums.numel() == 6 * C
        ctx.comm.allreduce_(sums[:4 * C].view(torch.float64), "C2 fwd " + self.name.split("/")[-1])
        self.count = float(rows) * ctx.comm.world
        self.mean_rstd = ctx.empty(2 * C)
        gam, bet = self.ps.w[self.name + "/gamma"], self.ps.w[self.name + "/beta"]
        if want_planes:
            y = torch.empty_like(x) if need_fp32 else None
            out = y if need_fp32 else PlanesOnly(x.shape)
            buf = torch.empty(L.query("ladder_presplit_bytes", x.numel(), ctx.ns), dtype=torch.uint8, device=ctx.device)
            y_amax = ctx.new_amax()
            L.call("ladder_bn_fwd_apply_planes", _p(x), _p(sums), self.count, _p(gam), _p(bet), _p(y), _p(buf), _p(self.mean_rstd), rows, C,
                   BN_EPS, L.ACT[self.act], _p(y_amax), ctx.stream)
            ctx.set_amax(out, y_amax)
            ctx.set_planes(out, buf)
            self.x = x
            return out
        y = torch.empty_like(x)
        y_amax = ctx.new_amax() if (ctx.ns == 4 and C % 4 == 0) else None
        L.call("ladder_bn_fwd_apply_absmax", _p(x), _p(sums), self.count, _p(gam), _p(bet), _p(y), _p(self.mean_rstd), rows, C, BN_EPS,
               L.ACT[self.act], _p(y_amax), ctx.stream)
        ctx.set_amax(y, y_amax)
        self.x = x
        return y

    def backward(self, dy, need_dx=True, wgrad=True):
        C, ctx, x = self.C, self.ctx, self.x
        rows = x.numel() // C
        gam, bet = self.ps.w[self.name + "/gamma"], self.ps.w[self.name + "/beta"]
        nb = L.query("ladder_bn_workspace_bytes", rows, C)
        wsp, wsn = ctx.ws(nb)
        dsums = ctx.empty(2 * C)
        L.call("ladder_bn_bwd_stats", _p(dy), _p(x), _p(self.mean_rstd), _p(gam), _p(bet), _p(dsums), rows, C,
               L.ACT[self.act], wsp, wsn, ctx.stream)
        ctx.comm.allreduce_(dsums, "C2 bwd " + self.name.split("/")[-1])
        dx = torch.empty_like(x) if need_dx else None
        dx_amax = ctx.new_amax() if (need_dx and ctx.ns == 4 and C % 4 == 0) else None
        L.call("ladder_bn_bwd_apply_absmax", _p(dy), _p(x), _p(self.mean_rstd), _p(gam), _p(bet), _p(dsums), self.count, _p(dx),
               _p(self.ps.g[self.name + "/gamma"]) if wgrad else None, _p(self.ps.g[self.name + "/beta"]) if wgrad else None,
               rows, C, L.ACT[self.act], _p(dx_amax), ctx.stream)
        if dx is not None:
            ctx.set_amax(dx, dx_amax)
        if wgrad and ctx.comm.world > 1:
            for t in (self.ps.g[self.name + "/gamma"], self.ps.g[self.name + "/beta"]):
                L.call("ladder_axpy", _p(t), _p(t), t.numel(), 1.0 / ctx.comm.world, 0, ctx.stream)
        self.x = None
        return dx


class InstanceNormStyleAct:

    def __init__(self, ctx, C, act):
        self.ctx, self.C, self.act = ctx, C, act

    def forward(self, x, style):
        N, H, W, C = x.shape
        y = torch.empty_like(x)
        self.mean_rstd = self.ctx.empty(N, 2 * C)
        wsp, wsn = self.ctx.ws(L.query("ladder_in_style_workspace_bytes", N, H * W, C))
        y_amax = self.ctx.new_amax() if (self.ctx.ns == 4 and C % 4 == 0) else None
        L.call("ladder_in_style_fwd_absmax", _p(x), _p(style), _p(y), _p(self.mean_rstd), N, H * W, C, IN_EPS, L.ACT[self.act],
               wsp, wsn, _p(y_amax), self.ctx.stream)
        self.ctx.set_amax(y, y_amax)
        self.x, self.style = x, style
        return y

    def forward_resized(self, x, style, rs, keep_lowres=False):
        N, H, W, C = x.shape
        up, y_lo = self.ctx.empty(N, 2 * H, 2 * W, C), None
        self.mean_rstd = self.ctx.empty(N, 2 * C)
        wsp, wsn = self.ctx.ws(L.query("ladder_in_style_workspace_bytes", N, H * W, C))
        up_amax = self.ctx.new_amax() if self.ctx.ns == 4 else None
        if keep_lowres:
            y_lo = self.ctx.empty(N, H, W, C)
            L.call("ladder_in_style_fwd_resize2x_keep", _p(x), _p(style), _p(up), _p(y_lo), _p(self.mean_rstd), N, H, W, C, IN_EPS,
                   L.ACT[self.act], wsp, wsn, _p(up_amax), self.ctx.stream)
            self.ctx.set_amax(y_lo, up_amax)
        else:
            L.call("ladder_in_style_fwd_resize2x", _p(x), _p(style), _p(up), _p(self.mean_rstd), N, H, W, C, IN_EPS, L.ACT[self.act], wsp, wsn,
                   _p(up_amax), self.ctx.stream)
        self.ctx.set_amax(up, up_amax)
        self.x, self.style = x, style
        rs.in_shape = (N, H, W, C)
        return up, y_lo

    def backward(self, dy):
        x = self.x
        N, H, W, C = x.shape
        dx = torch.empty_like(x)
        dstyle = self.ctx.empty(N, 2 * C)
        wsp, wsn = self.ctx.ws(L.query("ladder_in_style_workspace_bytes", N, H * W, C))
        dx_amax = self.ctx.new_amax() if (self.ctx.ns == 4 and C % 4 == 0) else None
        L.call("ladder_in_style_bwd_absmax", _p(dy), _p(x), _p(self.style), _p(self.mean_rstd), _p(dx), _p(dstyle), N, H * W, C,
               L.ACT[self.act], wsp, wsn, _p(dx_amax), self.ctx.stream)
        self.ctx.set_amax(dx, dx_amax)
        self.x = self.style = None
        return dx, dstyle


class Resize:

    def __init__(self, ctx, oh, ow):
        self.ctx, self.oh, self.ow = ctx, oh, ow

    def forward(self, x):
        N, H, W, C = x.shape
        self.in_shape = (N, H, W, C)
        if (H, W) == (self.oh, self.ow):
            return x
        y = self.ctx.empty(N, self.oh, self.ow, C)
        L.call("ladder_resize_bilinear_fwd", _p(x), _p(y), N, H, W, C, self.oh, self.ow, self.ctx.stream)
        self.ctx.set_amax(y, self.ctx.known_amax(x))
        return y

    def backward(self, dy, gate=None):
        N, H, W, C = self.in_shape
        if (H, W) == (self.oh, self.ow):
            return (dy, False) if gate is not None else dy
        dx = self.ctx.empty(N, H, W, C)
        if gate is not None and (self.oh, self.ow) == (2 * H, 2 * W) and gate[1] is not None:
            L.call("ladder_resize_bilinear_bwd_gated", _p(dy), _p(dx), N, H, W, C, self.oh, self.ow, _p(gate[0]), L.ACT[gate[1]],
                   self.ctx.stream)
            return dx, True
        L.call("ladder_resize_bilinear_bwd", _p(dy), _p(dx), N, H, W, C, self.oh, self.ow, self.ctx.stream)
        rec = self.ctx.known_amax(dy)
        if rec is not None:
            self.ctx.set_amax(dx, rec * float(arch.resize_transpose_gain(H, self.oh) * arch.resize_transpose_gain(W, self.ow)))
        return (dx, False) if gate is not None else dx


class DepthToSpace:
    def __init__(self, ctx, r):
        self.ctx, self.r = ctx, r

    def forward(self, x):
        N, H, W, C = x.shape
        r = self.r
        y = self.ctx.empty(N, H * r, W * r, C // (r * r))
        L.call("ladder_depth_to_space", _p(x), _p(y), N, H, W, C, r, 0, self.ctx.stream)
        return y

    def backward(self, dy):
        N, HR, WR, Cp = dy.shape
        r = self.r
        dx = self.ctx.empty(N, HR // r, WR // r, Cp * r * r)
        L.call("ladder_depth_to_space", _p(dy), _p(dx), N, HR // r, WR // r, Cp * r * r, r, 1, self.ctx.stream)
        return dx


def pad_symmetric(ctx, x, p):
    N, H, W, C = x.shape
    y = ctx.empty(N, H + 2 * p, W + 2 * p, C)
    L.call("ladder_pad_symmetric", _p(x), _p(y), N, H, W, C, p, ctx.stream)
    return y


def add_(ctx, out, inp):
    L.call("ladder_axpy", _p(inp), _p(out), out.numel(), 1.0, 1, ctx.stream)
    ctx.drop_amax(out)
    return out
```

Baseline: 6964 images/sec.

## Fold first-layer BN backward into RGB conv wgrad and add one-pass instance norm

For the first encoder conv, where no input gradient is needed, the batch-norm dx computation is folded into the RGB stride-2 weight-gradient kernel. The kernel recomputes the BN-adjusted gradient on the fly from the BN input, mean/rstd and dsums, so the full-size dx tensor is never written and read back. Separately, new one-pass instance-norm forward and backward kernels keep each slab in registers, replacing the multi-kernel stats, finalize and apply paths. The costs are extra register pressure (launch bounds drop to 3 blocks for the BN variant), extra loads of the BN input inside wgrad, and a cap on HW for the one-pass path.

```diff
diff --git a/include/ladder_hip.h b/include/ladder_hip.h
--- a/include/ladder_hip.h
+++ b/include/ladder_hip.h
@@ -207,6 +207,9 @@
                                        float* sums, void* ws, size_t ws_bytes, ladder_stream_t stream);
 int ladder_conv_rgb_s2_bwd_filter_f32(const float* x, const float* dy, float* dw, float* db, int N, int H, int W, int Cout, void* ws,
                                       size_t ws_bytes, ladder_stream_t stream);
+int ladder_conv_rgb_s2_bn_bwd_filter_f32(const float* x, const float* dy, const float* bn_x, const float* mean_rstd, const float* gamma,
+                                         const float* beta, const float* dsums, double count, int act, float* dw, float* db, int N, int H, int W,
+                                         int Cout, void* ws, size_t ws_bytes, ladder_stream_t stream);
 size_t ladder_conv_rgb_s2_bwd_filter_workspace_bytes(int N, int H, int W, int Cout);
 int ladder_conv_rgb_s2_bwd_filter(const float* x, const float* x_absmax, const float* dy, const float* dy_absmax, float* dw, float* db,
                                   int N, int H, int W, int Cout, void* ws, size_t ws_bytes, ladder_stream_t stream);
@@ -238,6 +241,7 @@
                                float* dx_absmax, ladder_stream_t stream);
 
 size_t ladder_in_style_workspace_bytes(int N, int HW, int C);
+int ladder_in_style_one_pass_kernel_id(int N, int HW, int C, int backward);
 int ladder_in_style_fwd(const float* x, const float* style, float* y, float* mean_rstd ,
                         int N, int HW, int C, float eps, int act, void* ws, size_t ws_bytes, ladder_stream_t stream);
 int ladder_in_style_bwd(const float* dy, const float* x, const float* style, const float* mean_rstd,
diff --git a/ladder_latent_data_distribution_modelling_amd/_lib.py b/ladder_latent_data_distribution_modelling_amd/_lib.py
--- a/ladder_latent_data_distribution_modelling_amd/_lib.py
+++ b/ladder_latent_data_distribution_modelling_amd/_lib.py
@@ -57,6 +57,7 @@
     "ladder_bn_bwd_stats": (_i, [_p, _p, _p, _p, _p, _p, _z, _i, _i, _p, _z, _p]),
     "ladder_bn_bwd_apply": (_i, [_p, _p, _p, _p, _p, _p, _d, _p, _p, _p, _z, _i, _i, _p]),
     "ladder_in_style_workspace_bytes": (_z, [_i, _i, _i]),
+    "ladder_in_style_one_pass_kernel_id": (_i, [_i, _i, _i, _i]),
     "ladder_in_style_fwd": (_i, [_p, _p, _p, _p, _i, _i, _i, _f, _i, _p, _z, _p]),
     "ladder_in_style_bwd": (_i, [_p, _p, _p, _p, _p, _p, _i, _i, _i, _i, _p, _z, _p]),
     "ladder_resize_bilinear_fwd": (_i, [_p, _p] + [_i] * 6 + [_p]),
@@ -186,6 +187,7 @@
     "ladder_conv_rgb_s2_bwd_filter_workspace_bytes": (_z, [_i] * 4),
     "ladder_conv_rgb_s2_bwd_filter": (_i, [_p] * 6 + [_i] * 4 + [_p, _z, _p]),
     "ladder_conv_rgb_s2_bwd_filter_f32": (_i, [_p] * 4 + [_i] * 4 + [_p, _z, _p]),
+    "ladder_conv_rgb_s2_bn_bwd_filter_f32": (_i, [_p] * 7 + [_d, _i, _p, _p] + [_i] * 4 + [_p, _z, _p]),
     "ladder_bn_fwd_apply_absmax": (_i, [_p, _p, _d, _p, _p, _p, _p, _z, _i, _f, _i, _p, _p]),
     "ladder_bn_bwd_apply_absmax": (_i, [_p, _p, _p, _p, _p, _p, _d, _p, _p, _p, _z, _i, _i, _p, _p]),
     "ladder_in_style_fwd_absmax": (_i, [_p, _p, _p, _p, _i, _i, _i, _f, _i, _p, _z, _p, _p]),
diff --git a/ladder_latent_data_distribution_modelling_amd/csrc/convrgb.hip b/ladder_latent_data_distribution_modelling_amd/csrc/convrgb.hip
--- a/ladder_latent_data_distribution_modelling_amd/csrc/convrgb.hip
+++ b/ladder_latent_data_distribution_modelling_amd/csrc/convrgb.hip
@@ -338,11 +338,13 @@
   if (bias_part != nullptr && lh == 0 && n < Cout) bias_part[(size_t)split * Cout + n] = bsum * (1.f / cd);
 }
 
+struct RgbBnArgs { const float* bx; const float* mean_rstd; const float* gamma; const float* beta; const float* dsums; float inv_count; int act; };
 constexpr int RW_LDA32 = 33;
-__global__ __launch_bounds__(RW_THREADS, 4) void conv_rgb_s2_wgrad_f32_kernel(const float* __restrict__ x, const float* __restrict__ dy,
-                                                                             float* __restrict__ part, float* __restrict__ bias_part,
-                                                                             const int N, const int H, const int W, const int Cout,
-                                                                             const int tiles_co, const int patches_per_split) {
+template <bool BN>
+__global__ __launch_bounds__(RW_THREADS, BN ? 3 : 4) void conv_rgb_s2_wgrad_f32_kernel(const float* __restrict__ x, const float* __restrict__ dy,
+                                                                                      float* __restrict__ part, float* __restrict__ bias_part,
+                                                                                      const int N, const int H, const int W, const int Cout,
+                                                                                      const int tiles_co, const int patches_per_split, const RgbBnArgs bn) {
   __shared__ float A32[RW_PIX * RW_LDA32];
   __shared__ float patch[RW_PATCH + 1];
   const int tid = threadIdx.x, lane = tid & 63, wv = tid >> 6;
@@ -353,6 +355,11 @@
   const int q0 = split * patches_per_split, q1 = min(q_total, q0 + patches_per_split);
   const int co = co0 + wv * 32 + l31;
   const bool co_ok = co < Cout;
+  float bn_mu = 0.f, bn_rs = 0.f, bn_g = 0.f, bn_be = 0.f, bn_s1 = 0.f, bn_s2 = 0.f;
+  if (BN && co_ok) {
+    bn_mu = bn.mean_rstd[co]; bn_rs = bn.mean_rstd[Cout + co]; bn_g = bn.gamma[co]; bn_be = bn.beta[co];
+    bn_s1 = bn.dsums[co] * bn.inv_count; bn_s2 = bn.dsums[Cout + co] * bn.inv_count;
+  }
 
   f32x16 acc;
 #pragma unroll
@@ -379,16 +386,18 @@
 
   if (q0 < q1) load_x(q0);
   for (int q = q0; q < q1; ++q) {
-    float b[RW_PIX / 2];
+    float b[RW_PIX / 2], bxv[BN ? RW_PIX / 2 : 1];
     {
       int img, h0, w0;
       decode(q, img, h0, w0);
-      const float* du = dy + (((long)img * Ho + h0) * Wo + w0) * Cout;
+      const long pix0 = (((long)img * Ho + h0) * Wo + w0) * Cout;
+      const float* du = dy + pix0;
       const unsigned loff = (unsigned)(co + lh * Cout);
 #pragma unroll
       for (int ks = 0; ks < RW_PIX / 2; ++ks) {
-        const float* pk = du + ((long)(ks >> 4) * Wo + 2 * (ks & 15)) * Cout;
-        b[ks] = co_ok ? pk[loff] : 0.f;
+        const long po = ((long)(ks >> 4) * Wo + 2 * (ks & 15)) * Cout;
+        b[ks] = co_ok ? (du + po)[loff] : 0.f;
+        if (BN) bxv[ks] = co_ok ? (bn.bx + pix0 + po)[loff] : 0.f;
       }
     }
 #pragma unroll
@@ -406,6 +415,14 @@
       }
     }
     __syncthreads();
+    if (BN) {
+#pragma unroll
+      for (int ks = 0; ks < RW_PIX / 2; ++ks) {
+        const float xh = (bxv[ks] - bn_mu) * bn_rs;
+        const float dp = b[ks] * ladder_act_grad_from_out(bn_g * xh + bn_be, bn.act);
+        b[ks] = co_ok ? bn_g * bn_rs * (dp - bn_s1 - xh * bn_s2) : 0.f;
+      }
+    }
 #pragma unroll
     for (int ks = 0; ks < RW_PIX / 2; ++ks) {
       const float a = A32[(2 * ks + lh) * RW_LDA32 + l31];
@@ -505,21 +522,39 @@
   return ladder_bn_stats_minmax_from_partials((const float*)ws, N * (H / 2 / RGB_TH) * (W / 2 / RGB_TW), sums, Cout, stream);
 }
 
-int ladder_conv_rgb_s2_bwd_filter_f32(const float* x, const float* dy, float* dw, float* db, int N, int H, int W, int Cout, void* ws,
-                                      size_t ws_bytes, ladder_stream_t stream) {
+static int rgb_wgrad_f32_launch(const float* x, const float* dy, float* dw, float* db, int N, int H, int W, int Cout, void* ws, size_t ws_bytes,
+                                const RgbBnArgs* bn, ladder_stream_t stream) {
   if (!rgb_s2_ok(N, H, W, 3, Cout, 3, 3, 2, 0, 0)) return LADDER_E_SHAPE;
   if (!ladder_aligned16(dw)) return LADDER_E_ALIGN;
   const RgbWgradPlan p = plan_rgb_wgrad(N, H, W, Cout);
   if (ws == nullptr || ws_bytes < (size_t)p.splits * (27 * (size_t)Cout + Cout) * sizeof(float)) return LADDER_E_WORKSPACE;
   float* part = (float*)ws;
   float* bias_part = db != nullptr ? part + (size_t)p.splits * 27 * Cout : nullptr;
-  hipLaunchKernelGGL(conv_rgb_s2_wgrad_f32_kernel, dim3(p.tiles_co * p.splits), dim3(RW_THREADS), 0, stream, x, dy, part, bias_part, N, H, W, Cout,
-                     p.tiles_co, p.pps);
+  if (bn != nullptr)
+    hipLaunchKernelGGL(conv_rgb_s2_wgrad_f32_kernel<true>, dim3(p.tiles_co * p.splits), dim3(RW_THREADS), 0, stream, x, dy, part, bias_part, N, H, W,
+                       Cout, p.tiles_co, p.pps, *bn);
+  else
+    hipLaunchKernelGGL(conv_rgb_s2_wgrad_f32_kernel<false>, dim3(p.tiles_co * p.splits), dim3(RW_THREADS), 0, stream, x, dy, part, bias_part, N, H, W,
+                       Cout, p.tiles_co, p.pps, RgbBnArgs{});
   LADDER_CHECK_LAUNCH();
   int rc = ladder_reduce_splits(part, dw, p.splits, (size_t)27 * Cout, stream);
   if (rc != LADDER_OK) return rc;
   if (db != nullptr) rc = ladder_reduce_splits(bias_part, db, p.splits, (size_t)Cout, stream);
   return rc;
+}
+
+int ladder_conv_rgb_s2_bwd_filter_f32(const float* x, const float* dy, float* dw, float* db, int N, int H, int W, int Cout, void* ws,
+                                      size_t ws_bytes, ladder_stream_t stream) {
+  return rgb_wgrad_f32_launch(x, dy, dw, db, N, H, W, Cout, ws, ws_bytes, nullptr, stream);
+}
+
+int ladder_conv_rgb_s2_bn_bwd_filter_f32(const float* x, const float* dy, const float* bn_x, const float* mean_rstd, const float* gamma,
+                                         const float* beta, const float* dsums, double count, int act, float* dw, float* db, int N, int H, int W,
+                                         int Cout, void* ws, size_t ws_bytes, ladder_stream_t stream) {
+  if (dy == nullptr || bn_x == nullptr || mean_rstd == nullptr || gamma == nullptr || beta == nullptr || dsums == nullptr || count <= 0)
+    return LADDER_E_SHAPE;
+  const RgbBnArgs bn{bn_x, mean_rstd, gamma, beta, dsums, (float)(1.0 / count), act};
+  return rgb_wgrad_f32_launch(x, dy, dw, db, N, H, W, Cout, ws, ws_bytes, &bn, stream);
 }
 
 size_t ladder_conv_rgb_s2_bwd_filter_workspace_bytes(int N, int H, int W, int Cout) {
diff --git a/ladder_latent_data_distribution_modelling_amd/csrc/norm.hip b/ladder_latent_data_distribution_modelling_amd/csrc/norm.hip
--- a/ladder_latent_data_distribution_modelling_amd/csrc/norm.hip
+++ b/ladder_latent_data_distribution_modelling_amd/csrc/norm.hip
@@ -769,6 +769,210 @@
   if (dxamax != nullptr) amax_commit_block_sample(omax, dxamax, n);
 }
 
+constexpr int IN1_MAX_HW = 4096;
+__device__ __forceinline__ int in1_slab(const int b, const int total, const int G) {
+  const int full = total / (8 * G) * (8 * G);
+  if (b >= full) return b;
+  const int xcd = b & 7, wi = b >> 3;
+  return ((wi / G) * 8 + xcd) * G + wi % G;
+}
+template <int NV> __device__ __forceinline__ int in1_src_lane(const int v) {
+  int off = 0;
+  for (int h = NV / 2, bit = 16 / NV; h >= 1; h >>= 1, bit <<= 1) off |= (v & h) ? bit : 0;
+  return off;
+}
+template <int NV, int T> __device__ __forceinline__ void in1_wg_sum(double (&a)[NV], double (*sm)[16]) {
+  const int lane = threadIdx.x & 63, wave = threadIdx.x >> 6;
+#pragma unroll
+  for (int h = NV / 2, bit = 16 / NV; h >= 1; h >>= 1, bit <<= 1) {
+    const bool hi = (lane & bit) != 0;
+#pragma unroll
+    for (int i = 0; i < h; ++i) {
+      const double send = hi ? a[i] : a[i + h], keep = hi ? a[i + h] : a[i];
+      a[i] = keep + __shfl_xor(send, bit, 64);
+    }
+  }
+  double t = a[0];
+  t += __shfl_xor(t, 16, 64);
+  t += __shfl_xor(t, 32, 64);
+  if (lane < 16) sm[wave][lane] = t;
+  __syncthreads();
+  constexpr int NW = T / 64;
+  t = 0.0;
+  for (int w = lane >> 4; w < NW; w += 4) t += sm[w][lane & 15];
+  t += __shfl_xor(t, 16, 64);
+  t += __shfl_xor(t, 32, 64);
+  const int quad = lane & (16 / NV - 1);
+#pragma unroll
+  for (int v = 0; v < NV; ++v) a[v] = __shfl(t, quad + in1_src_lane<NV>(v), 64);
+}
+__device__ __forceinline__ float4 in_style_act4(const float4 v, const float4 mu, const float4 rs, const float4 s0, const float4 s1, const int act) {
+  float4 o;
+  o.x = ladder_act_fn((v.x - mu.x) * rs.x * s0.x + s1.x, act);
+  o.y = ladder_act_fn((v.y - mu.y) * rs.y * s0.y + s1.y, act);
+  o.z = ladder_act_fn((v.z - mu.z) * rs.z * s0.z + s1.z, act);
+  o.w = ladder_act_fn((v.w - mu.w) * rs.w * s0.w + s1.w, act);
+  return o;
+}
+
+template <int R, int T>
+__global__ __launch_bounds__(T) void in_fwd_onepass_kernel(const float* __restrict__ x, const float* __restrict__ style, float* __restrict__ y,
+                                                           float* __restrict__ mean_rstd, const int HW, const int C, const int ng,
+                                                           const double inv_hw, const float eps, const int act, const int apply,
+                                                           float* __restrict__ rec) {
+  constexpr int L = T / 4;
+  const int slab = in1_slab(blockIdx.x, gridDim.x, 2);
+  const int n = slab / ng, g = slab - n * ng;
+  const int cq = threadIdx.x & 3, rl = threadIdx.x >> 2;
+  const int c = g * 16 + cq * 4;
+  const bool live = c < C;
+  const size_t base = (size_t)n * HW * C + c;
+  __shared__ double sm[2][T / 64][16];
+  float4 v[R];
+#pragma unroll
+  for (int k = 0; k < R; ++k) {
+    const int r = rl + k * L;
+    v[k] = (live && r < HW) ? *reinterpret_cast<const float4*>(x + base + (size_t)r * C) : make_float4(0.f, 0.f, 0.f, 0.f);
+  }
+  double s[4] = {0.0, 0.0, 0.0, 0.0};
+#pragma unroll
+  for (int k = 0; k < R; ++k) {
+    s[0] += (double)v[k].x; s[1] += (double)v[k].y; s[2] += (double)v[k].z; s[3] += (double)v[k].w;
+  }
+  in1_wg_sum<4, T>(s, sm[0]);
+  float mus[4], off[4];
+#pragma unroll
+  for (int j = 0; j < 4; ++j) {
+    const double mean = s[j] * inv_hw;
+    mus[j] = (float)mean;
+    off[j] = (float)(mean - (double)mus[j]);
+  }
+  const float4 mu = make_float4(mus[0], mus[1], mus[2], mus[3]);
+  float4 q = make_float4(0.f, 0.f, 0.f, 0.f);
+#pragma unroll
+  for (int k = 0; k < R; ++k)
+    if (rl + k * L < HW) {
+      const float dx = v[k].x - mu.x, dy = v[k].y - mu.y, dz = v[k].z - mu.z, dw = v[k].w - mu.w;
+      q.x += dx * dx; q.y += dy * dy; q.z += dz * dz; q.w += dw * dw;
+    }
+  double s2[4] = {(double)q.x, (double)q.y, (double)q.z, (double)q.w};
+  in1_wg_sum<4, T>(s2, sm[1]);
+  float rsv[4];
+#pragma unroll
+  for (int j = 0; j < 4; ++j) {
+    double var = s2[j] * inv_hw - (double)off[j] * (double)off[j];
+    if (var < 0.0) var = 0.0;
+    rsv[j] = (float)(1.0 / sqrt(var + (double)eps));
+  }
+  const float4 rs = make_float4(rsv[0], rsv[1], rsv[2], rsv[3]);
+  if (live && rl == 0) {
+    *reinterpret_cast<float4*>(mean_rstd + (size_t)n * 2 * C + c) = mu;
+    *reinterpret_cast<float4*>(mean_rstd + (size_t)n * 2 * C + C + c) = rs;
+  }
+  float ymax = 0.f;
+  if (live && apply) {
+    float4 s0 = *reinterpret_cast<const float4*>(style + (size_t)n * 2 * C + c);
+    const float4 s1 = *reinterpret_cast<const float4*>(style + (size_t)n * 2 * C + C + c);
+    s0.x += 1.f; s0.y += 1.f; s0.z += 1.f; s0.w += 1.f;
+    int rl2 = rl;
+    asm volatile("" : "+v"(rl2));
+#pragma unroll
+    for (int k = 0; k < R; ++k) {
+      const int r = rl2 + k * L;
+      if (r < HW) {
+        const float4 o = in_style_act4(v[k], mu, rs, s0, s1, act);
+        *reinterpret_cast<float4*>(y + base + (size_t)r * C) = o;
+        ymax = fmaxf(fmaxf(ymax, fmaxf(fabsf(o.x), fabsf(o.y))), fmaxf(fabsf(o.z), fabsf(o.w)));
+      }
+    }
+  }
+  if (rec != nullptr) amax_commit_block_sample(ymax, rec, n);
+}
+
+template <int R, int T>
+__global__ __launch_bounds__(T) void in_bwd_onepass_kernel(const float* __restrict__ dy, const float* __restrict__ x, const float* __restrict__ style,
+                                                           const float* __restrict__ mean_rstd, float* __restrict__ dx, float* __restrict__ dstyle,
+                                                           const int HW, const int C, const int ng, const int act, float* __restrict__ rec) {
+  constexpr int L = T / 2;
+  const int slab = in1_slab(blockIdx.x, gridDim.x, 4);
+  const int n = slab / ng, g = slab - n * ng;
+  const int cq = threadIdx.x & 1, rl = threadIdx.x >> 1;
+  const int c = g * 8 + cq * 4;
+  const bool live = c < C;
+  const size_t base = (size_t)n * HW * C + c;
+  __shared__ double sm[T / 64][16];
+  float4 xv[R], dv[R];
+#pragma unroll
+  for (int k = 0; k < R; ++k) {
+    const int r = rl + k * L;
+    const bool on = live && r < HW;
+    xv[k] = on ? *reinterpret_cast<const float4*>(x + base + (size_t)r * C) : make_float4(0.f, 0.f, 0.f, 0.f);
+    dv[k] = on ? *reinterpret_cast<const float4*>(dy + base + (size_t)r * C) : make_float4(0.f, 0.f, 0.f, 0.f);
+  }
+  float mu[4], rs[4], s0[4], s1[4];
+#pragma unroll
+  for (int j = 0; j < 4; ++j) {
+    const size_t i = (size_t)n * 2 * C + (live ? c + j : 0);
+    mu[j] = mean_rstd[i];
+    rs[j] = mean_rstd[i + C];
+    s0[j] = style[i] + 1.f;
+    s1[j] = style[i + C];
+  }
+  float a0[4] = {0.f, 0.f, 0.f, 0.f}, a1[4] = {0.f, 0.f, 0.f, 0.f};
+#pragma unroll
+  for (int k = 0; k < R; ++k) {
+    const bool on = live && rl + k * L < HW;
+    float xs[4] = {xv[k].x, xv[k].y, xv[k].z, xv[k].w}, ds[4] = {dv[k].x, dv[k].y, dv[k].z, dv[k].w};
+#pragma unroll
+    for (int j = 0; j < 4; ++j) {
+      const float xh = on ? (xs[j] - mu[j]) * rs[j] : 0.f;
+      const float dp = on ? ds[j] * ladder_act_grad_from_out(xh * s0[j] + s1[j], act) : 0.f;
+      a0[j] += dp * xh;
+      a1[j] += dp;
+      xs[j] = xh;
+      ds[j] = dp;
+    }
+    xv[k] = make_float4(xs[0], xs[1], xs[2], xs[3]);
+    dv[k] = make_float4(ds[0], ds[1], ds[2], ds[3]);
+  }
+  double a[8] = {(double)a0[0], (double)a0[1], (double)a0[2], (double)a0[3], (double)a1[0], (double)a1[1], (double)a1[2], (double)a1[3]};
+  in1_wg_sum<8, T>(a, sm);
+  float omax = 0.f;
+  float d0[4], d1[4];
+#pragma unroll
+  for (int j = 0; j < 4; ++j) {
+    d0[j] = (float)a[j];
+    d1[j] = (float)a[4 + j];
+  }
+  if (live && rl == 0) {
+    *reinterpret_cast<float4*>(dstyle + (size_t)n * 2 * C + c) = make_float4(d0[0], d0[1], d0[2], d0[3]);
+    *reinterpret_cast<float4*>(dstyle + (size_t)n * 2 * C + C + c) = make_float4(d1[0], d1[1], d1[2], d1[3]);
+  }
+  if (live) {
+    const float inv = 1.f / (float)HW;
+#pragma unroll
+    for (int j = 0; j < 4; ++j) {
+      d0[j] *= inv;
+      d1[j] *= inv;
+    }
+    int rl2 = rl;
+    asm volatile("" : "+v"(rl2));
+#pragma unroll
+    for (int k = 0; k < R; ++k) {
+      const int r = rl2 + k * L;
+      if (r < HW) {
+        const float xs[4] = {xv[k].x, xv[k].y, xv[k].z, xv[k].w}, ds[4] = {dv[k].x, dv[k].y, dv[k].z, dv[k].w};
+        float o[4];
+#pragma unroll
+        for (int j = 0; j < 4; ++j) o[j] = rs[j] * s0[j] * (ds[j] - d1[j] - xs[j] * d0[j]);
+        *reinterpret_cast<float4*>(dx + base + (size_t)r * C) = make_float4(o[0], o[1], o[2], o[3]);
+        omax = fmaxf(fmaxf(omax, fmaxf(fabsf(o[0]), fabsf(o[1]))), fmaxf(fabsf(o[2]), fabsf(o[3])));
+      }
+    }
+  }
+  if (rec != nullptr) amax_commit_block_sample(omax, rec, n);
+}
+
 inline int in_split(int N, int HW, int C) {
   const long groups = (long)N * ((C + 63) / 64);
   int sp = (int)((2048 + groups - 1) / groups);
@@ -776,6 +980,39 @@
   if (sp > max_sp) sp = max_sp;
   if (sp < 1) sp = 1;
   return sp;
+}
+
+static int in1_config(int N, int HW, int C, bool bwd) {
+  const char* e = getenv("LADDER_IN_ONE_PASS");
+  if (e != nullptr && atoi(e) == 0) return 0;
+  if (N <= 0 || HW <= 0 || C <= 0 || C % 4 != 0 || HW > IN1_MAX_HW || (long)N * ((C + 7) / 8) >= (1L << 30)) return 0;
+  if (bwd) return HW <= 32 ? 10064 : (HW <= 512 ? 40256 : 81024);
+  return HW <= 16 ? 10064 : (HW <= 256 ? 40256 : 161024);
+}
+static int in1_fwd_launch(const float* x, const float* style, float* y, float* mean_rstd, int N, int HW, int C, float eps, int act, int apply, float* rec,
+                          float* clear_rec, hipStream_t stream) {
+  if (clear_rec != nullptr && hipMemsetAsync(clear_rec, 0, LADDER_ABSMAX_FLOATS * sizeof(float), stream) != hipSuccess) return LADDER_E_LAUNCH;
+  const int ng = (C + 15) / 16;
+  const dim3 grid((unsigned)(N * ng));
+  const double inv_hw = 1.0 / (double)HW;
+  switch (in1_config(N, HW, C, false)) {
+    case 10064: hipLaunchKernelGGL((in_fwd_onepass_kernel<1, 64>), grid, dim3(64), 0, stream, x, style, y, mean_rstd, HW, C, ng, inv_hw, eps, act, apply, rec); break;
+    case 40256: hipLaunchKernelGGL((in_fwd_onepass_kernel<4, 256>), grid, dim3(256), 0, stream, x, style, y, mean_rstd, HW, C, ng, inv_hw, eps, act, apply, rec); break;
+    default: hipLaunchKernelGGL((in_fwd_onepass_kernel<16, 1024>), grid, dim3(1024), 0, stream, x, style, y, mean_rstd, HW, C, ng, inv_hw, eps, act, apply, rec);
+  }
+  return LADDER_OK;
+}
+static int in1_bwd_launch(const float* dy, const float* x, const float* style, const float* mean_rstd, float* dx, float* dstyle, int N, int HW, int C,
+                          int act, float* rec, hipStream_t stream) {
+  if (rec != nullptr && hipMemsetAsync(rec, 0, LADDER_ABSMAX_FLOATS * sizeof(float), stream) != hipSuccess) return LADDER_E_LAUNCH;
+  const int ng = (C + 7) / 8;
+  const dim3 grid((unsigned)(N * ng));
+  switch (in1_config(N, HW, C, true)) {
+    case 10064: hipLaunchKernelGGL((in_bwd_onepass_kernel<1, 64>), grid, dim3(64), 0, stream, dy, x, style, mean_rstd, dx, dstyle, HW, C, ng, act, rec); break;
+    case 40256: hipLaunchKernelGGL((in_bwd_onepass_kernel<4, 256>), grid, dim3(256), 0, stream, dy, x, style, mean_rstd, dx, dstyle, HW, C, ng, act, rec); break;
+    default: hipLaunchKernelGGL((in_bwd_onepass_kernel<8, 1024>), grid, dim3(1024), 0, stream, dy, x, style, mean_rstd, dx, dstyle, HW, C, ng, act, rec);
+  }
+  return LADDER_OK;
 }
 
 template <int V> struct ResizeVec;
@@ -1187,6 +1424,8 @@
 
 size_t ladder_in_style_workspace_bytes(int N, int HW, int C) { return (size_t)N * in_split(N, HW, C) * 2 * C * sizeof(float); }
 
+int ladder_in_style_one_pass_kernel_id(int N, int HW, int C, int backward) { return in1_config(N, HW, C, backward != 0); }
+
 int ladder_in_style_fwd(const float* x, const float* style, float* y, float* mean_rstd, int N, int HW, int C, float eps, int act,
                         void* ws, size_t ws_bytes, ladder_stream_t stream) {
   return ladder_in_style_fwd_absmax(x, style, y, mean_rstd, N, HW, C, eps, act, ws, ws_bytes, nullptr, stream);
@@ -1198,6 +1437,11 @@
   if (y_absmax != nullptr) {
     if (!(C % 4 == 0 && ws != nullptr && ws_bytes >= ladder_in_style_workspace_bytes(N, HW, C) && ladder_aligned16(x) && ladder_aligned16(y)))
       return LADDER_E_SHAPE;
+  }
+  if (in1_config(N, HW, C, false) != 0 && ladder_aligned16(x) && ladder_aligned16(y)) {
+    if (in1_fwd_launch(x, style, y, mean_rstd, N, HW, C, eps, act, 1, y_absmax, y_absmax, stream) != LADDER_OK) return LADDER_E_LAUNCH;
+    LADDER_CHECK_LAUNCH();
+    return LADDER_OK;
   }
   if (C % 4 == 0 && ws != nullptr && ws_bytes >= ladder_in_style_workspace_bytes(N, HW, C) && ladder_aligned16(x) && ladder_aligned16(y)) {
     const int sp = in_split(N, HW, C);
@@ -1225,10 +1469,14 @@
   const int HW = H * W;
   if (!(C % 4 == 0 && ws != nullptr && ws_bytes >= ladder_in_style_workspace_bytes(N, HW, C) && ladder_aligned16(x) && ladder_aligned16(up)))
     return LADDER_E_SHAPE;
-  const int sp = in_split(N, HW, C);
-  dim3 grid((C + 63) / 64, N, sp);
-  hipLaunchKernelGGL(in_stats_kernel, grid, dim3(256), 0, stream, x, (float*)ws, HW, C, sp);
-  hipLaunchKernelGGL(in_finalize_kernel, dim3((N * C + 255) / 256), dim3(256), 0, stream, x, (const float*)ws, mean_rstd, N, HW, C, sp, eps, up_absmax);
+  if (in1_config(N, HW, C, false) != 0) {
+    if (in1_fwd_launch(x, style, nullptr, mean_rstd, N, HW, C, eps, act, 0, nullptr, up_absmax, stream) != LADDER_OK) return LADDER_E_LAUNCH;
+  } else {
+    const int sp = in_split(N, HW, C);
+    dim3 grid((C + 63) / 64, N, sp);
+    hipLaunchKernelGGL(in_stats_kernel, grid, dim3(256), 0, stream, x, (float*)ws, HW, C, sp);
+    hipLaunchKernelGGL(in_finalize_kernel, dim3((N * C + 255) / 256), dim3(256), 0, stream, x, (const float*)ws, mean_rstd, N, HW, C, sp, eps, up_absmax);
+  }
   const long units = (long)HW * (C / 4);
   hipLaunchKernelGGL(in_apply_resize2x_kernel, dim3((unsigned)((units + 255) / 256), N), dim3(256), 0, stream, x, style,
                      (const float*)mean_rstd, up, H, W, C, act, up_absmax, y);
@@ -1248,6 +1496,11 @@
     if (!(C % 4 == 0 && ws != nullptr && ws_bytes >= ladder_in_style_workspace_bytes(N, HW, C) && ladder_aligned16(x) && ladder_aligned16(dy) &&
           ladder_aligned16(dx)))
       return LADDER_E_SHAPE;
+  }
+  if (in1_config(N, HW, C, true) != 0 && ladder_aligned16(x) && ladder_aligned16(dy) && ladder_aligned16(dx)) {
+    if (in1_bwd_launch(dy, x, style, mean_rstd, dx, dstyle, N, HW, C, act, dx_absmax, stream) != LADDER_OK) return LADDER_E_LAUNCH;
+    LADDER_CHECK_LAUNCH();
+    return LADDER_OK;
   }
   if (C % 4 == 0 && ws != nullptr && ws_bytes >= ladder_in_style_workspace_bytes(N, HW, C) && ladder_aligned16(x) && ladder_aligned16(dy) &&
       ladder_aligned16(dx)) {
diff --git a/ladder_latent_data_distribution_modelling_amd/engine.py b/ladder_latent_data_distribution_modelling_amd/engine.py
--- a/ladder_latent_data_distribution_modelling_amd/engine.py
+++ b/ladder_latent_data_distribution_modelling_amd/engine.py
@@ -52,9 +52,14 @@
             dh = self.hidden.backward(dh, wgrad=wgrad)
         dh = dh.reshape(self.conv_shape)
         for i in range(len(self.convs) - 1, -1, -1):
+            need_dx = i > 0 or need_input_dx
+            if self.bns[i] is not None and wgrad and not need_dx and self.convs[i].takes_bn_fold():
+                self.convs[i].backward_bn_folded(self.bns[i].backward(dh, wgrad=wgrad, fold=True))
+                dh = None
+                continue
             if self.bns[i] is not None:
                 dh = self.bns[i].backward(dh, wgrad=wgrad)
-            dh = self.convs[i].backward(dh, need_dx=(i > 0 or need_input_dx), wgrad=wgrad)
+            dh = self.convs[i].backward(dh, need_dx=need_dx, wgrad=wgrad)
         if need_input_dx and self.exp != "celeba":
             N, Hp, Wp, C = dh.shape
             dx = self.ctx.empty(N, Hp - 4, Wp - 4, C)
@@ -282,6 +287,7 @@
         self.ctx.up2 = int(cfg.get("upsample_fused_convs", 4 if prec == "f32" else 2))
         self.ctx.fuse_fwd = int(cfg.get("fused_projected_forward", 2))
         self.ctx.fuse_bwd_proj = int(cfg.get("fused_projection_backward", 1))
+        self.ctx.fold_bn_rgb = int(cfg.get("fold_bn_into_rgb_wgrad", 1))
         self.precision = prec
         if self.ctx.comm.rank == 0:
             print("Contraction precision (config key matmul_precision): {} -- {}".format(prec, PRECISION_NOTES[prec]))
diff --git a/ladder_latent_data_distribution_modelling_amd/layers.py b/ladder_latent_data_distribution_modelling_amd/layers.py
--- a/ladder_latent_data_distribution_modelling_amd/layers.py
+++ b/ladder_latent_data_distribution_modelling_amd/layers.py
@@ -87,6 +87,7 @@
         self.ns = 0
         self.up2_used = {}
         self.up2_skipped = {}
+        self.fold_bn_rgb = 1
         self.fuse_bwd_proj = 1
         self.fuse_fwd = 2
         self.up2 = True
@@ -730,6 +731,22 @@
             wsp, wsn = ctx.ws(r.wgrad.ws)
             ops = (_p(x), _p(xa), _p(dy), _p(da)) if ctx.ns else (_p(x), _p(dy))
             L.call(r.wgrad.fn, *ops, *self._grads(), r.N, r.H, r.W, self.cout, wsp, wsn, ctx.stream)
+
+    def takes_bn_fold(self):
+        k = self.kept
+        return bool(k is not None and self.act is None and self.ctx.ns == 0 and k.route.fused_bwd is None and k.route.wgrad is not None
+                    and k.route.wgrad.fn == "ladder_conv_rgb_s2_bwd_filter_f32" and self.ctx.fold_bn_rgb)
+
+    def backward_bn_folded(self, fold):
+        try:
+            k, ctx = self.kept, self.ctx
+            r = k.route
+            with ctx.side_or_main(k.x, fold.dy, fold.x, fold.mean_rstd, fold.gamma, fold.beta, fold.dsums):
+                wsp, wsn = ctx.ws(r.wgrad.ws)
+                L.call("ladder_conv_rgb_s2_bn_bwd_filter_f32", _p(k.x), _p(fold.dy), _p(fold.x), _p(fold.mean_rstd), _p(fold.gamma), _p(fold.beta),
+                       _p(fold.dsums), fold.count, L.ACT[fold.act], *self._grads(), r.N, r.H, r.W, self.cout, wsp, wsn, ctx.stream)
+        finally:
+            self.kept = None
 
     def _wg_halo_split(self, r, x, dy, x_amax, dy_amax, lo):
         ctx = self.ctx
@@ -958,6 +975,12 @@
         return dx
 
 
+class BnFold:
+
+    def __init__(self, dy, x, mean_rstd, gamma, beta, dsums, count, act):
+        self.dy, self.x, self.mean_rstd, self.gamma, self.beta, self.dsums, self.count, self.act = dy, x, mean_rstd, gamma, beta, dsums, count, act
+
+
 class BatchNormAct:
 
     def __init__(self, ctx, ps, name, C, act):
@@ -1002,7 +1025,8 @@
         self.x = x
         return y
 
-    def backward(self, dy, need_dx=True, wgrad=True):
+    def backward(self, dy, need_dx=True, wgrad=True, fold=False):
+        need_dx = need_dx and not fold
         C, ctx, x = self.C, self.ctx, self.x
         rows = x.numel() // C
         gam, bet = self.ps.w[self.name + "/gamma"], self.ps.w[self.name + "/beta"]
@@ -1023,6 +1047,8 @@
             for t in (self.ps.g[self.name + "/gamma"], self.ps.g[self.name + "/beta"]):
                 L.call("ladder_axpy", _p(t), _p(t), t.numel(), 1.0 / ctx.comm.world, 0, ctx.stream)
         self.x = None
+        if fold:
+            return BnFold(dy, x, self.mean_rstd, gam, bet, dsums, self.count, self.act)
         return dx
 
 
```

After: 7021 images/sec, median of 6. Within noise of the previous version (+0.8%).
